# logan-pearce/olpefit

Measured on AMD Instinct MI355X. Metric: walker-steps/sec (= model evals/sec) on 64×64 2-source cutout, 1/2/4/8 GPU, higher is better.
Workload: dtype f64

## Files before the change

### include/olpe.h

```cpp
#ifndef OLPE_H
#define OLPE_H

#include <stddef.h>
#include <stdint.h>

#ifdef __cplusplus
extern "C" {
#endif

#define OLPE_OK 0
#define OLPE_EINVAL (-1)
#define OLPE_EHIP (-2)
#define OLPE_ENOMEM (-3)
#define OLPE_ESTATE (-4)
#define OLPE_ECOMM (-5)
#define OLPE_EIO (-6)

#define OLPE_DTYPE_F32 0
#define OLPE_DTYPE_F64 1

#define OLPE_EVAL_EXACT 0
#define OLPE_EVAL_FAST 1

typedef struct olpe_ctx olpe_ctx;

int olpe_version(void);
int olpe_device_count(int *count);
int olpe_device_mem(int device, long long *free_bytes, long long *total_bytes);
int olpe_device_pci_id(int device, char *buf, int len);
const char *olpe_last_error(void);

int olpe_create(const void *image, int image_dtype, const void *pois2, double readnoise2,
                const uint8_t *mask, int ny, int nx, int nsrc, int bkgd_mode, int device,
                olpe_ctx **out);
void olpe_destroy(olpe_ctx *ctx);
int olpe_set_eval_mode(olpe_ctx *ctx, int mode);

int olpe_model(olpe_ctx *ctx, const double *params, double *model_out);
int olpe_chi2_batch(olpe_ctx *ctx, const double *params, int W, double *chi2_out);
int olpe_normal_batch(olpe_ctx *ctx, const double *params , int W,
                      double *chi2 , double *grad ,
                      double *jtj );

int olpe_seed(olpe_ctx *ctx, const uint32_t *seeds, int W);
int olpe_state_set(olpe_ctx *ctx, const double *state, const double *tries,
                   const double *accepts);
int olpe_state_get(olpe_ctx *ctx, double *state, double *tries, double *accepts);
int olpe_run(olpe_ctx *ctx, long long n_iters, long long burn_in, int record_stride,
             long long accept_min, long long *nrec_out);
int olpe_chain_read(olpe_ctx *ctx, double *chain_out);
int olpe_count(olpe_ctx *ctx, long long *count);
int olpe_count_reset(olpe_ctx *ctx, long long count);
int olpe_done_at(olpe_ctx *ctx, long long *done_at);
int olpe_run_gibbs(olpe_ctx *ctx, double *state, double *tries, double *accepts, int W,
                   long long n_iters, long long burn_in, int record_stride,
                   double *chain_out);

int olpe_rng_get(olpe_ctx *ctx, uint32_t *mt_state, double *gauss_cache);
int olpe_rng_set(olpe_ctx *ctx, const uint32_t *mt_state, const double *gauss_cache);
int olpe_rng_stream(olpe_ctx *ctx, int kind, int n, void *out);

int olpe_trace_enable(olpe_ctx *ctx, int on);
int olpe_trace_read(olpe_ctx *ctx, double *out);

int olpe_sync(olpe_ctx *ctx);
int olpe_last_kernel_ms(olpe_ctx *ctx, double *ms);
int olpe_kernel_times(olpe_ctx *ctx, int n, double *ms_out);
int olpe_last_units(olpe_ctx *ctx, int *units);
int olpe_unit_stats(olpe_ctx *ctx, long long *out);

#define OLPE_LOG_WIDTH_MAX 25.0
int olpe_widths_set(olpe_ctx *ctx, const double *w);
int olpe_widths_get(olpe_ctx *ctx, double *out);

#define OLPE_TUNE_LOG 256
int olpe_tune_begin(olpe_ctx *ctx, double target, double gain);
int olpe_tune_step(olpe_ctx *ctx);
int olpe_tune_get(olpe_ctx *ctx, int *steps, long long *dT, long long *dA, double *widths);
int olpe_tune_end(olpe_ctx *ctx);

int olpe_csv_format(const double *rows, long long nrows, int ncols, int nan_row, char *out,
                    size_t cap, size_t *len_out);
int olpe_csv_write_chains(const char *const *paths, const double *chains, int nfiles,
                          long long nrows, int ncols, int nan_row, int threads);

int olpe_csv_append_chains(const char *const *paths, const double *chains, int nfiles,
                           long long rows_per_file, long long nrows, int ncols, int threads,
                           long long *sizes_out);

int olpe_csv_shape(const char *path, long long *rows, int *cols);
int olpe_csv_read_chains(const char *const *paths, int nfiles, long long nrows, int ncols,
                         long long skip, double *out, int threads);

int olpe_acceptance_format(const double *x, int n, char *out, size_t cap, size_t *len_out);
int olpe_acceptance_write(const char *const *paths, const double *accepts, const double *tries,
                          int nfiles, int np, int threads, unsigned char *done);

int olpe_comm_unique_id(uint8_t *id128);
int olpe_comm_init(olpe_ctx *ctx, const uint8_t *id128, int nranks, int rank);
int olpe_comm_timeout(olpe_ctx *ctx, double seconds);
int olpe_comm_info(olpe_ctx *ctx, int *nranks, int *rank);
int olpe_comm_allgather_state(olpe_ctx *ctx, double *out);
int olpe_comm_allgather_chain(olpe_ctx *ctx, long long w0, long long wn, double *out,
                              long long *nrec_out);
int olpe_comm_gather_limit(olpe_ctx *ctx, long long bytes);
int olpe_comm_allreduce_moments(olpe_ctx *ctx, double *out);

int olpe_moments_accumulate(olpe_ctx *ctx);
int olpe_moments_reset(olpe_ctx *ctx);
int olpe_moments_get(olpe_ctx *ctx, long long *n, double *mean, double *m2);
int olpe_moments_set(olpe_ctx *ctx, long long n, const double *mean, const double *m2);
#define OLPE_MOMENTS_LEN(ps, np) (2 + 3 * (ps) + 2 * (np))
int olpe_moments_summary(olpe_ctx *ctx, const double *centre, double *out);

typedef struct olpe_astrom olpe_astrom;
#define OLPE_ASTROM_LEN 16
#define OLPE_ASTROM_BELOW_180 0
#define OLPE_ASTROM_BELOW_0 1
#define OLPE_ASTROM_ABOVE_360 2
#define OLPE_ASTROM_ABOVE_180 3
#define OLPE_ASTROM_ABOVE_0 4
#define OLPE_ASTROM_BELOW_PER_SAMPLE 5
int olpe_astrom_create(int device, int variant, int ps, const int *pair_cols, int npairs,
                       const double *x_dist, const double *y_dist, int tab_ny, int tab_nx,
                       int xdiff, int ydiff, double pixscale, double rotation_angle,
                       double rotcorr, int use_rotcorr, long long walkers, long long row_cap,
                       olpe_astrom **out);
void olpe_astrom_destroy(olpe_astrom *a);
int olpe_astrom_fold_ctx(olpe_astrom *a, olpe_ctx *ctx);
int olpe_astrom_fold_rows(olpe_astrom *a, const double *rows, long long nrows);
int olpe_astrom_rows(olpe_astrom *a, long long *rows);
int olpe_astrom_finalize(olpe_astrom *a, double delta_r, double parantel, double *out);
int olpe_astrom_samples(olpe_astrom *a, int pair, double *out);

typedef struct olpe_corner olpe_corner;
int olpe_corner_create(int device, int ncols, const double *edges1, int nb1,
                       const double *edges2, int nb2, olpe_corner **out);
void olpe_corner_destroy(olpe_corner *h);
int olpe_corner_fold_ctx(olpe_corner *h, olpe_ctx *ctx);
int olpe_corner_fold_rows(olpe_corner *h, const double *rows, long long nsamples);
int olpe_corner_get(olpe_corner *h, unsigned long long *n, unsigned long long *h1,
                    unsigned long long *h2);
int olpe_corner_add(olpe_corner *h, unsigned long long n, const unsigned long long *h1,
                    const unsigned long long *h2);
int olpe_corner_reset(olpe_corner *h);

// ... 109 lines not shown
```

### olpefit_amd/_lib.py

```python
from __future__ import annotations

import ctypes as C
import os

HERE = os.path.dirname(os.path.abspath(__file__))
LIB_PATH = os.environ.get("OLPE_LIB", os.path.join(HERE, "libolpe.so"))

OK, EINVAL, EHIP, ENOMEM, ESTATE, ECOMM, EIO = 0, -1, -2, -3, -4, -5, -6
DTYPE_F32, DTYPE_F64 = 0, 1
EVAL_EXACT, EVAL_FAST = 0, 1
LOG_WIDTH_MAX = 25.0
TUNE_LOG = 256


class OlpeError(RuntimeError):
    def __init__(self, code: int, msg: str):
        super().__init__(f"olpe error {code}: {msg}")
        self.code = code


_P = C.c_void_p
_i = C.c_int
_ll = C.c_longlong
_d = C.c_double
# ... 41 lines not shown
    "olpe_tune_get": (_i, [_P, C.POINTER(_i), _pll, _pll, _pd]),
    "olpe_tune_end": (_i, [_P]),
    "olpe_csv_format": (_i, [_pd, _ll, _i, _i, C.c_char_p, C.c_size_t,
                             C.POINTER(C.c_size_t)]),
    "olpe_csv_write_chains": (_i, [C.POINTER(C.c_char_p), _pd, _i, _ll, _i, _i, _i]),
    "olpe_csv_append_chains": (_i, [C.POINTER(C.c_char_p), _pd, _i, _ll, _ll, _i, _i, _pll]),
    "olpe_csv_shape": (_i, [C.c_char_p, _pll, C.POINTER(_i)]),
    "olpe_csv_read_chains": (_i, [C.POINTER(C.c_char_p), _i, _ll, _i, _ll, _pd, _i]),
    "olpe_acceptance_format": (_i, [_pd, _i, C.c_char_p, C.c_size_t, C.POINTER(C.c_size_t)]),
    "olpe_acceptance_write": (_i, [C.POINTER(C.c_char_p), _pd, _pd, _i, _i, _i, _pu8]),
    "olpe_moments_accumulate": (_i, [_P]),
    "olpe_moments_reset": (_i, [_P]),
    "olpe_moments_get": (_i, [_P, _pll, _pd, _pd]),
    "olpe_moments_set": (_i, [_P, _ll, _pd, _pd]),
    "olpe_moments_summary": (_i, [_P, _pd, _pd]),
    "olpe_comm_unique_id": (_i, [_pu8]),
    "olpe_comm_init": (_i, [_P, _pu8, _i, _i]),
    "olpe_comm_timeout": (_i, [_P, _d]),
    "olpe_comm_info": (_i, [_P, C.POINTER(_i), C.POINTER(_i)]),
    "olpe_comm_allgather_state": (_i, [_P, _pd]),
    "olpe_comm_allgather_chain": (_i, [_P, _ll, _ll, _pd, _pll]),
    "olpe_comm_gather_limit": (_i, [_P, _ll]),
    "olpe_comm_allreduce_moments": (_i, [_P, _pd]),
    "olpe_astrom_create": (_i, [_i, _i, _i, C.POINTER(_i), _i, _pd, _pd, _i, _i, _i, _i,
                                _d, _d, _d, _i, _ll, _ll, C.POINTER(_P)]),
    "olpe_astrom_destroy": (None, [_P]),
    "olpe_astrom_fold_ctx": (_i, [_P, _P]),
    "olpe_astrom_fold_rows": (_i, [_P, _pd, _ll]),
    "olpe_astrom_rows": (_i, [_P, _pll]),
    "olpe_astrom_finalize": (_i, [_P, _d, _d, _pd]),
    "olpe_astrom_samples": (_i, [_P, _i, _pd]),
    "olpe_corner_create": (_i, [_i, _i, _pd, _i, _pd, _i, C.POINTER(_P)]),
    "olpe_corner_destroy": (None, [_P]),
    "olpe_corner_fold_ctx": (_i, [_P, _P]),
    "olpe_corner_fold_rows": (_i, [_P, _pd, _ll]),
    "olpe_corner_get": (_i, [_P, _pu64, _pu64, _pu64]),
    "olpe_corner_add": (_i, [_P, C.c_ulonglong, _pu64, _pu64]),
    "olpe_corner_reset": (_i, [_P]),
    "olpe_resid_create": (_i, [_P, _pd, C.POINTER(_P)]),
    "olpe_resid_destroy": (None, [_P]),
    "olpe_resid_fold_ctx": (_i, [_P, _P, _i, _i]),
    "olpe_resid_fold_rows": (_i, [_P, _pd, _ll]),
    "olpe_resid_get": (_i, [_P, _pll, _pll, _pd, _pd, _pd, _pd]),
    "olpe_resid_add": (_i, [_P, _ll, _ll, _pd, _pd, _pd, _pd]),
    "olpe_resid_reset": (_i, [_P]),
    "olpe_resid_finalize": (_i, [_P, _pd, _pd]),
    "olpe_lik_create": (_i, [_P, _pd, C.POINTER(_P)]),
    "olpe_lik_destroy": (None, [_P]),
    "olpe_lik_fold_ctx": (_i, [_P, _P, _i, _i]),
    "olpe_lik_fold_rows": (_i, [_P, _pd, _ll]),
    "olpe_lik_get": (_i, [_P, _pll, _pll, _pd, _pd, _pd, _pd, _pd, _pd]),
    "olpe_lik_add": (_i, [_P, _ll, _ll, _pd, _pd, _pd, _pd, _pd, _pd]),
    "olpe_lik_reset": (_i, [_P]),
    "olpe_lik_point": (_i, [_P, _pd, _pd]),
    "olpe_lik_finalize": (_i, [_P, _pd, _pd, _pd]),
    "olpe_acf_create": (_i, [_i, _i, _i, C.POINTER(_P)]),
    "olpe_acf_destroy": (None, [_P]),
    "olpe_acf_fold_ctx": (_i, [_P, _P]),
    "olpe_acf_fold_rows": (_i, [_P, _pd, _ll, _ll, _i]),
    "olpe_acf_get": (_i, [_P, _pu64, _pu64, _pu64, _pd]),
    "olpe_acf_add": (_i, [_P, _i, _i, C.c_ulonglong, C.c_ulonglong, C.c_ulonglong, _pd]),
    "olpe_acf_reset": (_i, [_P]),
    "olpe_phot_create": (_i, [_i, _i, _i, _d, _ll, _ll, C.POINTER(_P)]),
    "olpe_phot_destroy": (None, [_P]),
    "olpe_phot_fold_ctx": (_i, [_P, _P, _i]),
    "olpe_phot_fold_rows": (_i, [_P, _pd, _ll]),
    "olpe_phot_rows": (_i, [_P, _pll]),
    "olpe_phot_unusable": (_i, [_P, _pll]),
    "olpe_phot_finalize": (_i, [_P, _pd, _i, _pd]),
    "olpe_phot_samples": (_i, [_P, _i, _pd]),
    "olpe_phot_reset": (_i, [_P]),
    "olpe_cov_create": (_i, [_i, _i, _ll, _pd, C.POINTER(_P)]),
    "olpe_cov_destroy": (None, [_P]),
    "olpe_cov_fold_ctx": (_i, [_P, _P, _i]),
    "olpe_cov_fold_rows": (_i, [_P, _pd, _ll, _ll, _i]),
    "olpe_cov_get": (_i, [_P, _pu64, _pu64, C.POINTER(_i), _pd, _pd, _pd]),
    "olpe_cov_walkers_get": (_i, [_P, _pu64, _pd]),
    "olpe_cov_between": (_i, [_P, _pd, _pu64, _pu64, _pu64]),
    "olpe_cov_add": (_i, [_P, _i, _ll, C.c_ulonglong, C.c_ulonglong, _pd, _pd, _pd, _pu64,
                          _pd]),
    "olpe_cov_reset": (_i, [_P]),
    "olpe_moments_fault": (_i, [_P, _i]),
    "olpe_test_hold_handoff": (_i, [_P, _i]),
    "olpe_test_chain_set": (_i, [_P, _pd, _ll]),
    "olpe_test_jacobian": (_i, [_P, _pd, _pd]),
}

_lib = None


def load(path: str = LIB_PATH):
    global _lib
    if _lib is not None:
        return _lib
    if not os.path.exists(path):
        raise OSError(f"libolpe.so not found at {path}: build it with "
                      "`python -m olpefit_amd.build` (hipcc, gfx950)")
    lib = C.CDLL(path)
    for name, (res, args) in SIGNATURES.items():
        f = getattr(lib, name)
        f.restype = res
        f.argtypes = args
    _lib = lib
    return lib


def check(rc: int) -> None:
    if rc != OK:
        msg = load().olpe_last_error().decode(errors="replace")
        raise OlpeError(rc, msg)
```

### olpefit_amd/core.py

```python
from __future__ import annotations

import ctypes as C

import numpy as np

from . import _lib
from ._lib import OlpeError, check

__all__ = ["OlpeError", "Sampler", "noise_model", "param_count", "SIGMA0"]

SIGMA0 = (50 / 9.95) / 2.35


def param_count(nsrc: int) -> int:
    if nsrc not in (2, 3):
        raise ValueError("nsrc must be 2 or 3")
    return 16 if nsrc == 2 else 19


def _dptr(a):
    return a.ctypes.data_as(_lib._pd) if a is not None else None


def noise_model(image, itime, coadds, multisam, sampmode):
# ... 220 lines not shown
            if w.shape != (self.np_,):
                raise ValueError(f"widths must have {self.np_} entries")
        check(self._lib.olpe_widths_set(self._ctx, _dptr(w)))

    def get_widths(self):
        out = np.empty(self.np_)
        check(self._lib.olpe_widths_get(self._ctx, _dptr(out)))
        return out

    def tune_begin(self, target=0.44, gain=2.0):
        check(self._lib.olpe_tune_begin(self._ctx, float(target), float(gain)))

    def tune_step(self):
        check(self._lib.olpe_tune_step(self._ctx))

    def tune_history(self):
        k = C.c_int(0)
        dT = np.zeros((_lib.TUNE_LOG, self.np_), dtype=np.int64)
        dA = np.zeros((_lib.TUNE_LOG, self.np_), dtype=np.int64)
        w = np.zeros((_lib.TUNE_LOG, self.np_))
        check(self._lib.olpe_tune_get(self._ctx, C.byref(k), dT.ctypes.data_as(_lib._pll),
                                      dA.ctypes.data_as(_lib._pll), _dptr(w)))
        k = k.value
        return dT[:k].copy(), dA[:k].copy(), w[:k].copy()

    def tune_end(self):
        check(self._lib.olpe_tune_end(self._ctx))

    @staticmethod
    def device_count() -> int:
        n = C.c_int(0)
        check(_lib.load().olpe_device_count(C.byref(n)))
        return n.value

    @staticmethod
    def device_pci_id(device: int) -> str:
        buf = C.create_string_buffer(64)
        check(_lib.load().olpe_device_pci_id(int(device), buf, 64))
        return buf.value.decode()

    @staticmethod
    def comm_unique_id() -> bytes:
        buf = (C.c_uint8 * 128)()
        check(_lib.load().olpe_comm_unique_id(buf))
        return bytes(buf)

    def comm_init(self, uid: bytes, nranks: int, rank: int):
        buf = (C.c_uint8 * 128).from_buffer_copy(uid)
        check(self._lib.olpe_comm_init(self._ctx, buf, nranks, rank))
        self.nranks = nranks

    def comm_timeout(self, seconds: float):
        check(self._lib.olpe_comm_timeout(self._ctx, float(seconds)))

    def comm_info(self) -> tuple[int, int]:
        n, r = C.c_int(-1), C.c_int(-1)
        check(self._lib.olpe_comm_info(self._ctx, C.byref(n), C.byref(r)))
        return n.value, r.value

    def allgather_state(self):
        out = np.empty((self.nranks * self.W, self.ps))
        check(self._lib.olpe_comm_allgather_state(self._ctx, _dptr(out)))
        return out

    def allgather_chain(self, w0: int = 0, wn: int | None = None, out: bool = True):
        wn = self.W - w0 if wn is None else wn
        nrec = C.c_longlong(0)
        buf = np.empty((self.nranks, wn, self._nrec, self.ps)) if out else None
        check(self._lib.olpe_comm_allgather_chain(self._ctx, int(w0), int(wn), _dptr(buf),
                                                  C.byref(nrec)))
        return buf

    def gather_limit(self, nbytes: int):
        check(self._lib.olpe_comm_gather_limit(self._ctx, int(nbytes)))

    def allreduce_moments(self):
        out = np.empty(self.moments_len)
        check(self._lib.olpe_comm_allreduce_moments(self._ctx, _dptr(out)))
        return out

    def hold_handoff(self, on: bool = True):
        check(self._lib.olpe_test_hold_handoff(self._ctx, 1 if on else 0))

    def test_chain_set(self, chain):
        ch = np.ascontiguousarray(chain, dtype=np.float64)
        if ch.ndim != 3 or ch.shape[2] != self.ps or (self.W and ch.shape[0] != self.W):
            raise ValueError(f"chain must be [{self.W}, nrec, {self.ps}]")
        check(self._lib.olpe_test_chain_set(self._ctx, _dptr(ch), ch.shape[1]))
        self._nrec = int(ch.shape[1])
        self._record_stride = 1

    def moments_fault(self, where: int):
        check(self._lib.olpe_moments_fault(self._ctx, int(where)))

    @property
    def moments_len(self) -> int:
        return 2 + 3 * self.ps + 2 * self.np_

    def moments_accumulate(self):
        check(self._lib.olpe_moments_accumulate(self._ctx))

    def moments_reset(self):
        check(self._lib.olpe_moments_reset(self._ctx))

    def moments(self):
        n = C.c_longlong(0)
        mean = np.empty((self.W, self.ps))
        m2 = np.empty((self.W, self.ps))
        check(self._lib.olpe_moments_get(self._ctx, C.byref(n), _dptr(mean), _dptr(m2)))
        return int(n.value), mean, m2

    def set_moments(self, n, mean=None, m2=None):
        mean = None if mean is None else np.ascontiguousarray(mean, dtype=np.float64)
        m2 = None if m2 is None else np.ascontiguousarray(m2, dtype=np.float64)
        check(self._lib.olpe_moments_set(self._ctx, int(n), _dptr(mean), _dptr(m2)))

    def moments_summary(self, centre=None):
        out = np.empty(self.moments_len)
        c = None if centre is None else np.ascontiguousarray(centre, dtype=np.float64)
        check(self._lib.olpe_moments_summary(self._ctx, _dptr(c), _dptr(out)))
        return out
```

### olpefit_amd/csrc/olpe.hip

```cpp
#include <hip/hip_runtime.h>

#include <limits.h>
#include <math.h>
#include <stdarg.h>
#include <stdint.h>
#include <stdio.h>
#include <stdlib.h>
#include <string.h>

#include <algorithm>
#include <cmath>
#include <atomic>
#include <vector>

#include "../../include/olpe.h"
#include "../../include/olpe_test.h"
#include "olpe_device.h"
#include "olpe_internal.h"

using namespace olpe;

namespace {

__constant__ double c_widths2[16] = {0.01, 0.01, 0.3,   0.3,    0.08,  0.09,
                                     0.0025, 0.02, 0.001, 0.0008, 0.002, 0.002,
                                     0.001, 0.001, 0.008, 0.01};
__constant__ double c_widths3[19] = {0.01,  0.01,  0.3,   0.3,  0.3,   0.3,   0.08,
                                     0.09,  0.0025, 0.02, 0.02, 0.001, 0.0008, 0.002,
                                     0.002, 0.001, 0.001, 0.008, 0.01};

__device__ __forceinline__ double width_of(const double *widths, int r) {
  return ((const __attribute__((address_space(4))) double *)widths)[r];
}

__global__ void widths_default_kernel(int nsrc, double *w, double *wdef) {
  const int j = threadIdx.x;
  if (j >= (nsrc == 2 ? 16 : 19)) return;
  const double v = nsrc == 2 ? c_widths2[j] : c_widths3[j];
  w[j] = v;
  if (wdef) wdef[j] = v;
}

struct GibbsArgs {
  const double2 *DE;
  int n;
  int bkgd_mode;
  long long W;
  double *state;
  uint32_t *tries;
  uint32_t *accepts;
  uint32_t *mt;
  int *mt_pos;
  double *gauss;
  int *has_gauss;
  long long *done_at;
  long long n_iters;
  long long count0;
  long long burn_in;
  long long stride;
  long long row0;
  long long nrows;
  double *chain;
  long long accept_min;
  double *trace;
  const double *widths;
  unsigned long long *queue;
  unsigned long long qbase;
  int units;
  unsigned *uflag;
  unsigned utag;
  unsigned *uerr;
  unsigned long long wait_ticks;
  int balance;
  int stagger;
  unsigned *hold;
};

constexpr int kTraceF = 6;
constexpr int kSampHdr = kEtabBytes + 64;


template <int NP> struct WaveSlice {
  static constexpr int U32 = 2 * NP;
  static constexpr int PS = NP + 1;
  static constexpr int NSRC = NP == 16 ? 2 : 3;
  static constexpr int OT1 = PS, OT2 = PS + 5, OC1 = PS + 10, OC2 = PS + 13;
  static constexpr int OPT = PS + 16, OPC = PS + 21;
  static constexpr int OWD = PS + 24;
  static constexpr int F64 = 2 * PS + 24;
  static constexpr int OMD = ((U32 * 4 + F64 * 8 + 15) & ~15);
  static constexpr int OCC = (OMD + (int)sizeof(ModelDesc<NSRC>) + 15) & ~15;
  static constexpr int OPE = (OCC + 2 * NSRC * 4 * 8 + 15) & ~15;
  static constexpr int BYTES = OPE + NSRC * 2 * 64 * 8;
};
constexpr int kDrawTabBytes = (kDrawTab * 8 + 15) & ~15;
constexpr int kDrawTabExactBytes = (kThr * 8 + 15) & ~15;
__host__ __device__ constexpr int drawtab_extra(int nt, bool fast = true) {
  return (nt != 0 && nt <= 64) ? (fast ? kDrawTabBytes : kDrawTabExactBytes) : 0;
}
__host__ __device__ inline int vtab_bytes(int n, int nsrc) { return (n * 2 * nsrc * 8 + 15) & ~15; }
__host__ __device__ constexpr bool single_h(int nsrc, int nt, int wpb, bool fast) {
  return nsrc == 2 && nt == 64 && wpb == 16 && fast;
}
__host__ __device__ constexpr int sampler_vtab_bytes(int n, int nsrc, int nt, int wpb = 12,
                                                     bool fast = false) {
  return single_h(nsrc, nt, wpb, fast) ? 64 * 16
       : (nsrc == 3 && nt == 64) ? 2 * 64 * 16 : ((n * 2 * nsrc * 8 + 15) & ~15);
}
template <int NP> __host__ __device__ constexpr int ring_wave_bytes(int n) {
  return WaveSlice<NP>::OPE + kDrawTabBytes + 2 * n * 16;
}
__host__ __device__ constexpr bool ring_wpb(int nt, int wpb) {
  return nt == 128 && (wpb == 12 || wpb == 8);
}
static_assert((WaveSlice<16>::U32 * 4) % 8 == 0 && (WaveSlice<19>::U32 * 4) % 8 == 0, "align");
template <int NP> constexpr int parking_bytes() { return WaveSlice<NP>::BYTES - WaveSlice<NP>::OPE; }
static_assert(parking_bytes<16>() >= 64 * 4 * 8 && sampler_vtab_bytes(64, 2, 64) >= 64 * 4 * 8 &&
              parking_bytes<19>() >= 64 * 6 * 8 && parking_bytes<16>() >= 2 * 32 * 4 * 8 &&
              parking_bytes<19>() >= 2 * 32 * 6 * 8 && sampler_vtab_bytes(128, 2, 128) >= 128 * 4 * 8 &&
              sampler_vtab_bytes(128, 3, 128) >= 128 * 6 * 8 && drawtab_extra(32) && drawtab_extra(64),
              "sweep_exact_rows tables");

__device__ __forceinline__ Trig ld_trig(const double *s) { return Trig{s[0], s[1], s[2]}; }
__device__ __forceinline__ Coef ld_coef(const double *s) { return Coef{s[0], s[1], s[2]}; }
__device__ __forceinline__ void st_trig(double *s, const Trig &t) {
  s[0] = t.cost2; s[1] = t.sint2; s[2] = t.sin2t;
}
__device__ __forceinline__ void st_shape(double *s, const Trig &t, double ix, double iy) {
  st_trig(s, t);
  s[3] = ix; s[4] = iy;
}
__device__ __forceinline__ void st_coef(double *s, const Coef &k) {
  s[0] = k.a; s[1] = k.b; s[2] = k.c;
}

__device__ __forceinline__ void lds_inc(uint32_t *p) {
  const unsigned a = (unsigned)(size_t)(__attribute__((address_space(3))) uint32_t *)p;
  asm volatile("ds_add_u32 %0, %1" : : "v"(a), "v"(1u) : "memory");
}
__device__ __forceinline__ uint32_t lds_inc_rtn(uint32_t *p) {
  const unsigned a = (unsigned)(size_t)(__attribute__((address_space(3))) uint32_t *)p;
  uint32_t old;
  asm volatile("ds_add_rtn_u32 %0, %1, %2\n\ts_waitcnt lgkmcnt(0)"
               : "=v"(old) : "v"(a), "v"(1u) : "memory");
  return old;
}

typedef __attribute__((address_space(1))) unsigned gu32;
typedef __attribute__((address_space(1))) unsigned long long gu64;
__device__ __forceinline__ void st_wt(double *p, double v) {
  __hip_atomic_store((gu64 *)p, (unsigned long long)__double_as_longlong(v), __ATOMIC_RELAXED,
                     __HIP_MEMORY_SCOPE_AGENT);
}
__device__ __forceinline__ void st_wt(long long *p, long long v) {
  __hip_atomic_store((gu64 *)p, (unsigned long long)v, __ATOMIC_RELAXED, __HIP_MEMORY_SCOPE_AGENT);
}
template <class T> __device__ __forceinline__ void st_wt(T *p, T v) {
  static_assert(sizeof(T) == 4, "32-bit word");
  unsigned u;
  __builtin_memcpy(&u, &v, 4);
  __hip_atomic_store((gu32 *)p, u, __ATOMIC_RELAXED, __HIP_MEMORY_SCOPE_AGENT);
}
template <class T> __device__ __forceinline__ T ld_uniform(const T *p) {
  static_assert(sizeof(T) == 4, "32-bit word");
  const unsigned u = (unsigned)__builtin_amdgcn_readfirstlane(
      (int)__hip_atomic_load((gu32 *)p, __ATOMIC_RELAXED, __HIP_MEMORY_SCOPE_AGENT));
  T v;
  __builtin_memcpy(&v, &u, 4);
  return v;
}
__device__ __forceinline__ void unit_publish(unsigned *flag, unsigned v, int lane) {
  asm volatile("s_waitcnt vmcnt(0)" ::: "memory");
  if (lane == 0) __hip_atomic_store((gu32 *)flag, v, __ATOMIC_RELAXED, __HIP_MEMORY_SCOPE_AGENT);
}
__device__ __forceinline__ void unit_wait(unsigned *flag, unsigned want, unsigned *err,
                                          unsigned long long *stats, int lane,
                                          unsigned long long limit, unsigned *hold) {
  const unsigned long long t0 = __builtin_amdgcn_s_memrealtime();
  bool waited = false;
  for (;;) {
    const unsigned v = (unsigned)__builtin_amdgcn_readfirstlane(
        (int)__hip_atomic_load((gu32 *)flag, __ATOMIC_RELAXED, __HIP_MEMORY_SCOPE_AGENT));
    if (v == want) break;
    if (!waited && hold && lane == 0)
      __hip_atomic_store((gu32 *)hold, 1u, __ATOMIC_RELAXED, __HIP_MEMORY_SCOPE_AGENT);
    waited = true;
    if (__builtin_amdgcn_s_memrealtime() - t0 > limit) {
      __hip_atomic_store((gu32 *)err, 1u, __ATOMIC_RELAXED, __HIP_MEMORY_SCOPE_AGENT);
      break;
    }
    __builtin_amdgcn_s_sleep(4);
  }
  if (waited && lane == 0) {
    atomicAdd(stats, 1ull);
    atomicAdd(stats + 1, __builtin_amdgcn_s_memrealtime() - t0);
  }
  __builtin_amdgcn_fence(__ATOMIC_ACQUIRE, "agent");
  asm volatile("s_waitcnt vmcnt(0)" ::: "memory");
}

__device__ __forceinline__ void hold_handoff(unsigned *hold, unsigned *err, unsigned long long limit) {
  const unsigned long long t0 = __builtin_amdgcn_s_memrealtime();
  while (__builtin_amdgcn_readfirstlane((int)__hip_atomic_load((gu32 *)hold, __ATOMIC_RELAXED,
                                                               __HIP_MEMORY_SCOPE_AGENT)) == 0) {
    if (__builtin_amdgcn_s_memrealtime() - t0 > limit) {
      __hip_atomic_store((gu32 *)err, 1u, __ATOMIC_RELAXED, __HIP_MEMORY_SCOPE_AGENT);
      break;
    }
    __builtin_amdgcn_s_sleep(4);
  }
}

constexpr int kCtrlPrio = 2;
constexpr int kGlobalWavesPerEU = 3;
template <int NSRC, int NT, bool LDS_IMG, int WPB, bool FAST>
__global__ __launch_bounds__(WPB * 64, (LDS_IMG || (NT == 128 && WPB == 12)) ? 1 : kGlobalWavesPerEU)
void olpe_gibbs_kernel(GibbsArgs A) {
  using L = Layout<NSRC>;
  using WS = WaveSlice<L::NP>;
  constexpr int NP = L::NP, PS = L::PS;
  constexpr bool RING = !LDS_IMG && FAST && ring_wpb(NT, WPB);
  using Ring = LdsRing<WPB>;
  extern __shared__ __align__(16) unsigned char smem[];
  const int n = NT ? NT : A.n;
  const int npix = n * n;
  const int lane = threadIdx.x & 63;
  const int wave = __builtin_amdgcn_readfirstlane(threadIdx.x >> 6);

  double *etab = reinterpret_cast<double *>(smem);
  unsigned *s_prog = reinterpret_cast<unsigned *>(smem + kEtabBytes);
  double2 *sDE = reinterpret_cast<double2 *>(smem + kSampHdr);
  constexpr int TABX = drawtab_extra(NT, FAST);
  const int wstride = RING ? ring_wave_bytes<NP>(n)
                           : WS::BYTES + TABX + sampler_vtab_bytes(n, NSRC, NT, WPB, FAST);
  unsigned char *wb = reinterpret_cast<unsigned char *>(sDE + (LDS_IMG ? npix : 0)) +
                      (RING ? Ring::BYTES : 0) + (size_t)wave * wstride;
  uint32_t *s_tries = reinterpret_cast<uint32_t *>(wb);
  uint32_t *s_acc = s_tries + NP;
  double *st = reinterpret_cast<double *>(wb + WS::U32 * 4);
  double *vtab = reinterpret_cast<double *>(wb + (RING ? WS::OPE + kDrawTabBytes : WS::BYTES + TABX));
  double *drawtab = reinterpret_cast<double *>(wb + (TABX ? WS::BYTES : WS::OPE));
  ModelDesc<NSRC> *mdl = reinterpret_cast<ModelDesc<NSRC> *>(wb + WS::OMD);
  double *colc = reinterpret_cast<double *>(wb + WS::OCC);

  if constexpr (LDS_IMG) {
    for (int k = threadIdx.x; k < npix; k += blockDim.x) sDE[k] = A.DE[k];
  }
  if (threadIdx.x < 64) etab[threadIdx.x] = c_exp2_64[threadIdx.x];
  if (threadIdx.x == 0) s_prog[0] = 0u;
  __syncthreads();
  const double2 *DE = LDS_IMG ? sDE : A.DE;
  [[maybe_unused]] Ring ring;
  if constexpr (RING) ring.prologue(smem + kSampHdr, A.DE, wave, lane);
  unsigned my_steps = 0;
  for (int i = 0, n = (wave >> 2) * A.stagger; i < n; ++i) __builtin_amdgcn_s_sleep(8);

  auto K = []() {
    const __attribute__((address_space(4))) GibbsArgs *p =
        (const __attribute__((address_space(4))) GibbsArgs *)__builtin_amdgcn_kernarg_segment_ptr();
    asm volatile("" : "+s"(p));
    return p;
  };

  auto take = [&]() -> int {
    unsigned long long v = 0;
    if (lane == 0) v = atomicAdd(K()->queue, 1ull) - K()->qbase;
    const unsigned d = v > 0x7fffffffull ? 0x7fffffffu : (unsigned)v;
    return __builtin_amdgcn_readfirstlane((int)d);
  };

  const int niter = (int)A.n_iters;
  const int rstride = (int)A.stride;
  const int nrows = (int)A.nrows;
  int rec_it0 = -1, rec_row0 = 0;
  if (A.stride > 0) {
    const long long c1 = A.count0 + 1;
    const long long k = c1 > A.burn_in ? (c1 - A.burn_in + A.stride - 1) / A.stride : 0;
    const long long first = A.burn_in + k * A.stride - c1;
    rec_it0 = first < niter ? (int)first : -1;
    rec_row0 = (int)(k - A.row0);
  }
  auto take_batch = [&]() -> int {
    asm volatile("s_waitcnt lgkmcnt(0)\n\ts_barrier" ::: "memory");
    if (wave == 0 && lane == 0) {
      const unsigned long long v = atomicAdd(K()->queue, 1ull) - K()->qbase;
      s_prog[1] = v > 0x7fffffffull ? 0x7fffffffu : (unsigned)v;
    }
    asm volatile("s_waitcnt lgkmcnt(0)\n\ts_barrier" ::: "memory");
    return __builtin_amdgcn_readfirstlane((int)s_prog[1]);
  };
  const int total = (int)K()->W * K()->units;
  int u = RING ? 0 : A.queue ? take() : (int)blockIdx.x * WPB + wave;
  for (;;) {
    bool active = true;
    if constexpr (RING) {
      const int bt = take_batch();
      if (bt >= (total + WPB - 1) / WPB) break;
      u = bt * WPB + wave;
      active = u < total;
      if (!active) u = 0;
    } else {
      if (u >= total) break;
    }
    const int units = K()->units;
    const int Wn = (int)K()->W;
    int w = u, k = 0, it_s = 0, it_e = niter;
    if (units > 1) {
      k = u / Wn;
      w = u - k * Wn;
      const int q = niter / units, r = niter - q * units;
      it_s = q * k + (r * k) / units;
      it_e = q * (k + 1) + (r * (k + 1)) / units;
      if (k > 0 && active)
        unit_wait(K()->uflag + w, K()->utag + (unsigned)k, K()->uerr, K()->queue + 2, lane,
                  K()->wait_ticks, K()->hold);
    }
    int it_end = it_e;
    if constexpr (RING) {
      if (lane == 0) s_prog[2 + wave] = active ? (unsigned)(it_e - it_s) : 0u;
      asm volatile("s_waitcnt lgkmcnt(0)\n\ts_barrier" ::: "memory");
      unsigned mx = 0;
      for (int j = 0; j < WPB; ++j) mx = max(mx, s_prog[2 + j]);
      it_end = it_s + (int)__builtin_amdgcn_readfirstlane((int)mx);
      if (!active) it_e = it_s;
    }
    if (lane < NP) {
      s_tries[lane] = K()->tries[(size_t)w * NP + lane];
      s_acc[lane] = K()->accepts[(size_t)w * NP + lane];
    }
    if (lane < PS) st[lane] = K()->state[(size_t)w * PS + lane];
    if constexpr (FAST) {
      if (lane < NP) st[WS::OWD + lane] = K()->widths[lane];
    }
    wave_sync();
    if (lane == 0) {
      const Trig t1 = make_trig<FAST>(st[L::T1]), t2 = make_trig<FAST>(st[L::T2]);
      const double i1x = inv_var(st[L::S1X]), i1y = inv_var(st[L::S1Y]);
      const double i2x = inv_var(st[L::S2X]), i2y = inv_var(st[L::S2Y]);
      st_shape(st + WS::OT1, t1, i1x, i1y);
      st_shape(st + WS::OT2, t2, i2x, i2y);
      if constexpr (FAST) {
        st_coef(st + WS::OC1, coef_inv(t1, i1x, i1y));
        st_coef(st + WS::OC2, coef_inv(t2, i2x, i2y));
      } else {
        st_coef(st + WS::OC1, make_coef<FAST>(st[L::S1X], st[L::S1Y], t1));
        st_coef(st + WS::OC2, make_coef<FAST>(st[L::S2X], st[L::S2Y], t2));
      }
    }
    wave_sync();
    const int bg_idx = A.bkgd_mode == 0 ? L::BG_QUIRK : L::BG_FIXED;
    build_desc<NSRC, NT, FAST>(mdl, colc, [&](int k) -> double { return st[k]; },
                               ld_coef(st + WS::OC1), ld_coef(st + WS::OC2), bg_idx, lane, etab);
    wave_sync();

    MTWave mt;
    mt.key = K()->mt + (size_t)w * MT_N;
    mt.pos = ld_uniform(K()->mt_pos + w);
    mt.bstart = mt.pos;
    mt.bsize = 0;
    mt.batch = 0;
    mt.has_gauss = ld_uniform(K()->has_gauss + w);
    mt.gauss = uniform_f64(K()->gauss[w]);
    mt.tab = drawtab;
    mt.thr = FAST;

    int ndone = 0;
    long long done_at = K()->done_at[w];
    if (A.accept_min > 0) {
      for (int k = 0; k < NP; ++k) ndone += (s_tries[k] >= (uint32_t)A.accept_min);
      ndone = __builtin_amdgcn_readfirstlane(ndone);
      if (ndone == NP && done_at < 0 && it_s < it_e) done_at = A.count0 + it_s + 1;
    }

    int rec_it = rec_it0, rec_row = rec_row0;
    if (rec_it0 >= 0 && it_s > rec_it0) {
      const int j = (it_s - rec_it0 + rstride - 1) / rstride;
      rec_it += j * rstride;
      rec_row += j;
    }
    double *chain_w = K()->chain + (size_t)w * nrows * PS;

    HCache hcache;
    hcache.single = single_h(NSRC, NT, WPB, FAST);
    GuardCache gcache;
    ColCache<2 * NSRC> ccache;
    ccache.pbuf = reinterpret_cast<double *>(wb + WS::OPE);
    ccache.colc = colc;
    __builtin_amdgcn_s_setprio(kCtrlPrio);
    for (int it = it_s; it < it_end; ++it) {
      if constexpr (RING) {
        if (it >= it_e) {
          ring.idle_step();
          continue;
        }
      }
      int r0 = 0, dice_idx = 0;
      double g = 0.0;
      mt.template draw<NP>(lane, 0, 2, r0, g, dice_idx);
      const int r = __builtin_amdgcn_readfirstlane(r0);
// ... 112 lines not shown

      const double dchi = chi - st[PS - 1];
      const double la = -dchi / 2.;
      double dice = 0.0;
      if constexpr (!FAST) dice = drawtab[dice_idx];
      bool acc;
      uint32_t acc_bit;
      if constexpr (FAST) {
        const double thr = drawtab[kThr + (dice_idx == 128 ? 64 : dice_idx)];
        acc_bit = (uint32_t)(__builtin_amdgcn_ballot_w64(dchi < thr) >> 32) >> 31;
      } else {
        acc_bit = (uint32_t)(__builtin_amdgcn_ballot_w64(dice < exp(la)) >> 32) >> 31;
      }
      asm volatile("" : "+s"(acc_bit));
      acc = acc_bit != 0;
      if (acc && lane == 63) st[PS - 1] = chi;
      double chi_u = 0.0, la_u = 0.0;
      if (A.trace) {
        chi_u = lane63_f64(chi);
        la_u = lane63_f64(la);
      }
      hcache.after(acc);
      gcache.after(acc);
      if constexpr (FAST && NT != 0 && NT <= 64) {
        if (acc && gmask) colcache_accept<NSRC, NT>(ccache, *mdl, gmask, lane, etab);
        ccache.pend = 0;
      }
      if (!acc && !nan_prop) {
        Coef Cs{0.0, 0.0, 0.0};
        if (grp) Cs = ld_coef(st + (grp == 1 ? WS::OC1 : WS::OC2));
        int pl = lane;
        asm volatile("" : "+v"(pl));
        patch_desc<NSRC, NT, FAST>(mdl, colc, st, r, st[r], Cs, grp,
                                   A.bkgd_mode == 0 ? L::BG_QUIRK : L::BG_FIXED, pl, etab);
      }
      wave_sync();
      if (acc && lane == 0) {
        if constexpr (FAST) lds_inc(s_acc + r);
        else s_acc[r] = s_acc[r] + 1u;
        st[r] = nv;
        if (grp) {
          double *dt = st + (grp == 1 ? WS::OT1 : WS::OT2);
          double *dc = st + (grp == 1 ? WS::OC1 : WS::OC2);
          for (int k = 0; k < 5; ++k) dt[k] = st[WS::OPT + k];
          for (int k = 0; k < 3; ++k) dc[k] = st[WS::OPC + k];
        }
      }
      wave_sync();

      if (A.trace) {
       if (lane == 0) {
        double *t = A.trace + ((size_t)w * A.n_iters + it) * kTraceF;
        t[0] = (double)r;
        t[1] = nv;
        t[2] = chi_u;
        t[3] = FAST ? drawtab[dice_idx] : dice;
        t[4] = FAST ? (la_u == la_u ? ExpTab{etab}(la_u) : la_u) : exp(la_u);
        t[5] = acc ? 1.0 : 0.0;
       }
      }
      if (it == rec_it) {
        if (rec_row >= 0 && rec_row < nrows && lane < PS) chain_w[rec_row * PS + lane] = st[lane];
        rec_it += rstride;
        ++rec_row;
      }
    }

    wave_sync();
    if (RING && !active) continue;
    asm volatile("" : "+s"(u));
    k = K()->units > 1 ? u / (int)K()->W : 0;
    w = u - k * (int)K()->W;
    if (lane < PS) st_wt(K()->state + (size_t)w * PS + lane, st[lane]);
    if (lane < NP) {
      st_wt(K()->tries + (size_t)w * NP + lane, s_tries[lane]);
      st_wt(K()->accepts + (size_t)w * NP + lane, s_acc[lane]);
    }
    if (lane == 0) {
      st_wt(K()->mt_pos + w, mt.pos);
      st_wt(K()->has_gauss + w, mt.has_gauss);
      st_wt(K()->gauss + w, mt.gauss);
      st_wt(K()->done_at + w, done_at);
    }
    if (k < K()->units - 1) {
      if (k == 0 && K()->hold) hold_handoff(K()->hold, K()->uerr, K()->wait_ticks);
      unit_publish(K()->uflag + w, K()->utag + (unsigned)(k + 1), lane);
    }
    wave_sync();
    if constexpr (!RING) u = K()->queue ? take() : INT_MAX;
  }
  if constexpr (RING) asm volatile("s_waitcnt vmcnt(0) lgkmcnt(0)\n\ts_barrier" ::: "memory");
}

template <int NSRC, bool WRITE>
__global__ __launch_bounds__(256) void olpe_eval_kernel(const double2 *DE, int n, int bkgd_mode,
                                                        int fast, const double *params, int W,
                                                        double *out) {
  using L = Layout<NSRC>;
  constexpr int PS = L::PS;
  extern __shared__ __align__(16) unsigned char smem[];
  const int lane = threadIdx.x & 63;
  const int wave = threadIdx.x >> 6;
  double *etab = reinterpret_cast<double *>(smem);
  double *vtab =
      reinterpret_cast<double *>(smem + kEtabBytes + (size_t)wave * vtab_bytes(n, NSRC));
  if (threadIdx.x < 64) etab[threadIdx.x] = c_exp2_64[threadIdx.x];
  __syncthreads();
  const long long w = (long long)blockIdx.x * (blockDim.x / 64) + wave;
  if (w >= W) return;
  double p[PS];
#pragma unroll
  for (int k = 0; k < PS; ++k) p[k] = uniform_f64(params[w * PS + k]);
  auto q = [&](int k) -> double { return p[k]; };
  double *o = WRITE ? out + (size_t)w * n * n : nullptr;
  double part;
  if (fast) {
    const Trig T1 = make_trig<true>(p[L::T1]), T2 = make_trig<true>(p[L::T2]);
    const ModelDesc<NSRC> md = make_model<NSRC>(
        q, make_coef<true>(p[L::S1X], p[L::S1Y], T1), make_coef<true>(p[L::S2X], p[L::S2Y], T2),
        bkgd_mode);
    part = sweep<NSRC, 0, WRITE, true>(md, DE, vtab, o, n, lane, etab);
  } else {
    const Trig T1 = make_trig<false>(p[L::T1]), T2 = make_trig<false>(p[L::T2]);
    const ModelDesc<NSRC> md = make_model<NSRC>(
        q, make_coef<false>(p[L::S1X], p[L::S1Y], T1),
        make_coef<false>(p[L::S2X], p[L::S2Y], T2), bkgd_mode);
    part = sweep<NSRC, 0, WRITE, false>(md, DE, vtab, o, n, lane, etab);
  }
  if constexpr (!WRITE) {
    const double chi = wave_sum(part);
    if (lane == 0) out[w] = chi;
  }
}

__global__ void olpe_seed_kernel(const uint32_t *seeds, int W, uint32_t *mt, int *pos,
                                 int *has_gauss, double *gauss) {
  const int w = blockIdx.x * blockDim.x + threadIdx.x;
  if (w >= W) return;
  mt_seed_serial(mt + (size_t)w * MT_N, seeds[w]);
  pos[w] = MT_N;
  has_gauss[w] = 0;
  gauss[w] = 0.0;
}

template <int NP>
__global__ __launch_bounds__(64) void olpe_stream_kernel(uint32_t *mtg, int *posg,
                                                         int *hasg, double *gg, int W,
                                                         int kind, int nd, void *out) {
  const int lane = threadIdx.x;
  const int w = blockIdx.x;
  if (w >= W) return;
  __shared__ double drawtab[kDrawTab];
  MTWave mt;
  mt.tab = drawtab;
  mt.key = mtg + (size_t)w * MT_N;
  mt.pos = __builtin_amdgcn_readfirstlane(posg[w]);
  mt.bstart = mt.pos;
  mt.bsize = 0;
  mt.batch = 0;
  mt.has_gauss = __builtin_amdgcn_readfirstlane(hasg[w]);
  mt.gauss = uniform_f64(gg[w]);
  for (int i = 0; i < nd; ++i) {
    if (kind == 0) {
      const uint32_t v = mt.next(lane);
      if (lane == 0) reinterpret_cast<uint32_t *>(out)[(size_t)w * nd + i] = v;
    } else {
      int r = 0, di = 0;
      double v = 0.0;
// ... 8 lines not shown
    posg[w] = mt.pos;
    hasg[w] = mt.has_gauss;
    gg[w] = mt.gauss;
  }
}

}

namespace olpe {

thread_local char g_err[512] = "";

int set_err(int code, const char *fmt, ...) {
  va_list ap;
  va_start(ap, fmt);
  vsnprintf(g_err, sizeof(g_err), fmt, ap);
  va_end(ap);
  return code;
}

}

namespace {

template <class T> int dev_alloc(T **p, size_t count) {
  if (*p) {
    (void)hipFree(*p);
    *p = nullptr;
  }
  if (count == 0) return OLPE_OK;
  hipError_t e = hipMalloc((void **)p, count * sizeof(T));
  if (e != hipSuccess) {
    *p = nullptr;
    return set_err(OLPE_ENOMEM, "hipMalloc(%zu bytes): %s", count * sizeof(T),
                   hipGetErrorString(e));
  }
  return OLPE_OK;
}

size_t wave_lds(int n, int np, bool lds_img, bool ring = false, int wpb = 12,
                bool fast = false) {
  if (ring) return (size_t)(np == 16 ? ring_wave_bytes<16>(n) : ring_wave_bytes<19>(n));
  const int nt = lds_img && (n == 32 || n == 64) ? n : 0;
  return (size_t)(np == 16 ? WaveSlice<16>::BYTES : WaveSlice<19>::BYTES) +
         drawtab_extra(nt, fast) + sampler_vtab_bytes(n, np == 16 ? 2 : 3, nt, wpb, fast);
}

int choose_units(long long W, long long slots, long long n_iters, int override_p) {
  const int pmax = 15;
  auto ok = [&](int p) { return p <= pmax && p <= n_iters && W * p < 0x7fffffffLL; };
  if (override_p > 0) {
    int p = override_p;
    while (p > 1 && !ok(p)) --p;
    return p;
  }
  if (n_iters < 16 || slots <= 0 || W <= 0) return 1;
  const double s0 = 2.0;
  auto T = [&](int p) {
    const double rounds = (double)((W * p + slots - 1) / slots);
    return std::max(rounds * ((double)n_iters / p + s0), (double)n_iters + p * s0);
  };
  int best = 1;
  double tb = T(1);
  for (int p = 2; p <= 8; ++p) {
    if (!ok(p) || n_iters / p < 8) break;
    const double t = T(p);
    if (t < tb) {
      tb = t;
      best = p;
    }
  }
  return tb < 0.97 * T(1) ? best : 1;
}

size_t lds_bytes(const olpe_ctx *c, int wpb, bool ring = false) {
  size_t b = (size_t)wpb * wave_lds(c->n, c->np, c->lds_img, ring, wpb,
                                    c->eval_mode == OLPE_EVAL_FAST) + kSampHdr;
  if (c->lds_img) b += (size_t)c->n * c->n * sizeof(double2);
  if (ring) b += wpb >= 12 ? LdsRing<12>::BYTES : LdsRing<8>::BYTES;
  return b;
}


template <int NSRC, int NT, bool LDS, int WPB, bool FAST>
int launch_gibbs_t(olpe_ctx *c, const GibbsArgs &a) {
  constexpr bool RING = !LDS && FAST && ring_wpb(NT, WPB);
  const size_t shm = lds_bytes(c, WPB, RING);
  auto k = olpe_gibbs_kernel<NSRC, NT, LDS, WPB, FAST>;
  static std::atomic<uint64_t> attr_set{0};
  const uint64_t bit = 1ull << (c->device & 63);
  if (!(attr_set.load(std::memory_order_acquire) & bit)) {
    HIPCHK(hipFuncSetAttribute((const void *)k, hipFuncAttributeMaxDynamicSharedMemorySize,
                               160 * 1024));
    attr_set.fetch_or(bit, std::memory_order_release);
  }
  unsigned blocks = (unsigned)((a.W + WPB - 1) / WPB);
  GibbsArgs q = a;
  q.queue = nullptr;
  q.qbase = 0;
  q.units = 1;
  q.uflag = c->d_uflag;
  q.utag = 0;
  q.uerr = reinterpret_cast<unsigned *>(c->d_queue + 1);
  q.stagger = c->stagger;
  q.hold = nullptr;
  int per_cu = 0;
  HIPCHK(hipOccupancyMaxActiveBlocksPerMultiprocessor(&per_cu, k, WPB * 64, shm));
  const unsigned resident = (unsigned)std::max(1, per_cu) * (unsigned)c->n_cu;
  const int units = c->queue_on && c->d_queue && c->d_uflag && !(RING && a.W < WPB)
                        ? choose_units(a.W, (long long)resident * WPB, a.n_iters, c->units_override)
                        : 1;
  if (c->queue_on && c->d_queue && (LDS || RING || units > 1)) {
    if (blocks > resident) blocks = resident;
    q.queue = c->d_queue;
    q.qbase = c->qbase;
    q.units = units;
    c->utag += 16;
    q.utag = c->utag;
    if (c->hold_handoff && units > 1) {
      const unsigned need = (unsigned)((a.W + WPB - 1) / WPB) + 1;
      if (need > resident)
        return set_err(OLPE_EINVAL, "olpe_test_hold_handoff: %lld walkers need %u resident "
                       "workgroups, the device holds %u", a.W, need, resident);
      blocks = need;
      HIPCHK(hipMemsetAsync(c->d_queue + 4, 0, sizeof(unsigned long long), c->stream));
      q.hold = reinterpret_cast<unsigned *>(c->d_queue + 4);
    }
  }
  q.balance = c->balance >= 0 ? c->balance
            : (LDS && FAST && NSRC == 2 && WPB == 16 && q.units == 1 &&
               a.W <= (long long)resident * WPB) ? 1 : 0;
  c->last_units = q.units;
  if (q.units > 1) c->units_used = true;
  {
    const double chunk = (double)((a.n_iters + q.units - 1) / q.units);
    const double ticks = chunk * (double)a.n * (double)a.n * (2.0 * NSRC) * 0.8;
    q.wait_ticks = c->wait_ticks_override > 0
                       ? (unsigned long long)c->wait_ticks_override
                       : (unsigned long long)std::min(std::max(ticks, 3e9), 1e15);
    c->wait_limit_s = (double)q.wait_ticks * 1e-8;
  }
  hipLaunchKernelGGL(k, dim3(blocks), dim3(WPB * 64), shm, c->stream, q);
  HIPCHK(hipGetLastError());
  if (q.queue) {
    const unsigned long long tot = (unsigned long long)a.W * (unsigned long long)q.units;
    c->qbase += RING ? (tot + WPB - 1) / WPB + blocks : tot + (unsigned long long)blocks * WPB;
  }
  return OLPE_OK;
}

template <int NSRC, bool FAST> int launch_gibbs_m(olpe_ctx *c, const GibbsArgs &a) {
  if (c->lds_img) {
    switch (c->n) {
      case 32: return launch_gibbs_t<NSRC, 32, true, 12, FAST>(c, a);
      case 64: {
        const long long r16 = 16LL * c->n_cu, r12 = 12LL * c->n_cu;
        int wpb = c->wpb ? c->wpb
                : (NSRC == 2 && (!FAST || a.W >= 8 * r16 || (a.W > r12 && a.W <= r16)))
                      ? 16 : 12;
        if (wpb == 16 && lds_bytes(c, 16) > 160 * 1024) wpb = 12;
        if (wpb == 8) return launch_gibbs_t<NSRC, 64, true, 8, FAST>(c, a);
        if (wpb == 12) return launch_gibbs_t<NSRC, 64, true, 12, FAST>(c, a);
        return launch_gibbs_t<NSRC, 64, true, 16, FAST>(c, a);
      }
      default: return launch_gibbs_t<NSRC, 0, true, 16, FAST>(c, a);
    }
  }
  if (c->n == 128) {
    if constexpr (FAST) {
      if (c->ring_wpb && c->queue_on && c->d_queue && c->d_uflag) {
        return launch_gibbs_t<NSRC, 128, false, 12, FAST>(c, a);
      }
    }
    return launch_gibbs_t<NSRC, 128, false, 4, FAST>(c, a);
  }
  if (lds_bytes(c, 4) > 160 * 1024) return launch_gibbs_t<NSRC, 0, false, 1, FAST>(c, a);
  return launch_gibbs_t<NSRC, 0, false, 4, FAST>(c, a);
}

int launch_gibbs(olpe_ctx *c, const GibbsArgs &a) {
  const bool fast = c->eval_mode == OLPE_EVAL_FAST;
  if (c->nsrc == 2) return fast ? launch_gibbs_m<2, true>(c, a) : launch_gibbs_m<2, false>(c, a);
  return fast ? launch_gibbs_m<3, true>(c, a) : launch_gibbs_m<3, false>(c, a);
}

int ensure_ensemble(olpe_ctx *c, int W) {
  if (W <= 0) return set_err(OLPE_EINVAL, "W must be > 0 (got %d)", W);
  if (c->W == W && c->d_state) return OLPE_OK;
  int rc;
  if ((rc = dev_alloc(&c->d_state, (size_t)W * c->ps))) return rc;
  if ((rc = dev_alloc(&c->d_tries, (size_t)W * c->np))) return rc;
  if ((rc = dev_alloc(&c->d_acc, (size_t)W * c->np))) return rc;
  if ((rc = dev_alloc(&c->d_mt, (size_t)W * MT_N))) return rc;
  if ((rc = dev_alloc(&c->d_mtpos, (size_t)W))) return rc;
  if ((rc = dev_alloc(&c->d_gauss, (size_t)W))) return rc;
  if ((rc = dev_alloc(&c->d_hasg, (size_t)W))) return rc;
  if ((rc = dev_alloc(&c->d_done, (size_t)W))) return rc;
  if ((rc = dev_alloc(&c->d_uflag, (size_t)W))) return rc;
  HIPCHK(hipMemsetAsync(c->d_uflag, 0, (size_t)W * sizeof(unsigned), c->stream));
  HIPCHK(hipMemsetAsync(c->d_state, 0, (size_t)W * c->ps * sizeof(double), c->stream));
  HIPCHK(hipMemsetAsync(c->d_tries, 0, (size_t)W * c->np * sizeof(uint32_t), c->stream));
  HIPCHK(hipMemsetAsync(c->d_acc, 0, (size_t)W * c->np * sizeof(uint32_t), c->stream));
  HIPCHK(hipMemsetAsync(c->d_done, 0xff, (size_t)W * sizeof(long long), c->stream));
  c->W = W;
  c->seeded = false;
  c->count = 0;
  c->chain_rows = 0;
  c->mom_n = 0;
  return OLPE_OK;
}

}

int olpe_widths_defaults(olpe_ctx *c, bool with_base) {
  hipLaunchKernelGGL(widths_default_kernel, dim3(1), dim3(64), 0, c->stream, c->nsrc, c->d_widths,
                     with_base ? c->d_wdef : nullptr);
  HIPCHK(hipGetLastError());
  return OLPE_OK;
}

extern "C" {

int olpe_version(void) { return 101; }


const char *olpe_last_error(void) { return g_err; }

int olpe_device_count(int *count) {
  if (!count) return set_err(OLPE_EINVAL, "count is NULL");
  int n = 0;
  hipError_t e = hipGetDeviceCount(&n);
  *count = (e == hipSuccess) ? n : 0;
  return OLPE_OK;
}

int olpe_device_pci_id(int device, char *buf, int len) {
  if (!buf || len < 16) return set_err(OLPE_EINVAL, "buffer of at least 16 bytes needed");
  int ndev = 0;
  if (hipGetDeviceCount(&ndev) != hipSuccess || ndev == 0)
    return set_err(OLPE_EHIP, "no HIP device visible");
  if (device < 0 || device >= ndev) return set_err(OLPE_EINVAL, "bad device %d", device);
  HIPCHK(hipDeviceGetPCIBusId(buf, len, device));
  return OLPE_OK;
}

int olpe_device_mem(int device, long long *free_bytes, long long *total_bytes) {
  if (!free_bytes || !total_bytes) return set_err(OLPE_EINVAL, "NULL argument");
  int ndev = 0;
  if (hipGetDeviceCount(&ndev) != hipSuccess || ndev == 0)
    return set_err(OLPE_EHIP, "no HIP device visible");
  if (device < 0 || device >= ndev) return set_err(OLPE_EINVAL, "bad device %d", device);
  HIPCHK(hipSetDevice(device));
  size_t f = 0, t = 0;
  HIPCHK(hipMemGetInfo(&f, &t));
  *free_bytes = (long long)f;
  *total_bytes = (long long)t;
  return OLPE_OK;
}

int olpe_create(const void *image, int image_dtype, const void *pois2, double readnoise2,
                const uint8_t *mask, int ny, int nx, int nsrc, int bkgd_mode, int device,
                olpe_ctx **out) {
  if (!out) return set_err(OLPE_EINVAL, "out is NULL");
  *out = nullptr;
  if (!image || !pois2) return set_err(OLPE_EINVAL, "image/pois2 is NULL");
  if (ny <= 0 || nx <= 0) return set_err(OLPE_EINVAL, "bad shape %dx%d", ny, nx);
  if (ny != nx)
    return set_err(OLPE_EINVAL,
                   "non-square image %dx%d: the reference model is square-only "
                   "(apf_step2.py:237, :119-123)", ny, nx);
  if (nx > 4096) return set_err(OLPE_EINVAL, "image too large (%d)", nx);
  if (nsrc != 2 && nsrc != 3) return set_err(OLPE_EINVAL, "nsrc must be 2 or 3");
  {
    const size_t one = wave_lds(nx, nsrc == 2 ? 16 : 19, false) + kSampHdr;
    if (one > 160 * 1024)
      return set_err(OLPE_EINVAL, "%dx%d cutout: its row tables need %zu bytes of LDS per "
                     "wave, more than the 163840 a workgroup has (cut the frame to the stars)",
                     nx, nx, one);
  }
  if (image_dtype != OLPE_DTYPE_F32 && image_dtype != OLPE_DTYPE_F64)
    return set_err(OLPE_EINVAL, "image_dtype must be OLPE_DTYPE_F32/F64");
  if (bkgd_mode != 0 && bkgd_mode != 1) return set_err(OLPE_EINVAL, "bkgd_mode must be 0/1");
  if (device < 0) return set_err(OLPE_EINVAL, "device must be a HIP ordinal (no CPU path)");
  const int np_ = nsrc == 2 ? 16 : 19;
  const size_t npix_ = (size_t)nx * nx;
  const bool lds_img = npix_ * sizeof(double2) +
                           ((nx == 64 || nx == 32) ? 12 : 16) * wave_lds(nx, np_, true) +
                           kSampHdr <= 160 * 1024;
  int wpb = 0;
  if (const char *e = getenv("OLPE_WPB")) {
    wpb = atoi(e);
    if (wpb != 8 && wpb != 12 && wpb != 16)
      return set_err(OLPE_EINVAL, "OLPE_WPB=%s: must be 8, 12 or 16", e);
    const size_t b = (size_t)wpb * wave_lds(nx, np_, true, false, wpb, true) + kSampHdr +
                     npix_ * sizeof(double2);
    if (lds_img && nx == 64 && b > 160 * 1024)
      return set_err(OLPE_EINVAL, "OLPE_WPB=%d needs %zu bytes of LDS at %dx%d (%d sources) > 163840",
                     wpb, b, nx, nx, nsrc);
    if (!(lds_img && nx == 64)) wpb = 0;
  }
  int ndev = 0;
  if (hipGetDeviceCount(&ndev) != hipSuccess || ndev == 0)
    return set_err(OLPE_EHIP, "no HIP device visible");
  if (device >= ndev) return set_err(OLPE_EINVAL, "device %d >= device count %d", device, ndev);
  HIPCHK(hipSetDevice(device));

  olpe_ctx *c = new olpe_ctx();
  c->device = device;
  c->n = nx;
  c->nsrc = nsrc;
  c->bkgd_mode = bkgd_mode;
  c->np = nsrc == 2 ? 16 : 19;
  c->ps = c->np + 1;
  const size_t npix = (size_t)nx * nx;
  c->lds_img = lds_img;
  c->wpb = wpb;
  std::vector<double2> hDE(npix), hDW(npix);
  for (size_t i = 0; i < npix; ++i) {
    const double d = image_dtype == OLPE_DTYPE_F32 ? (double)((const float *)image)[i]
                                                   : ((const double *)image)[i];
    const double p2 = image_dtype == OLPE_DTYPE_F32 ? (double)((const float *)pois2)[i]
                                                    : ((const double *)pois2)[i];
    const double e = sqrt(readnoise2 + p2);
    if ((mask && mask[i]) || !std::isfinite(d) || !(e > 0.0)) {
      hDE[i] = make_double2(0.0, 0.0);
      hDW[i] = make_double2(0.0, 0.0);
    } else {
      hDE[i] = make_double2(d, 1.0 / e);
      hDW[i] = make_double2(d * (1.0 / e), 1.0 / e);
    }
  }
  bool any_pixel = false;
  for (size_t i = 0; i < npix && !any_pixel; ++i) any_pixel = hDE[i].y != 0.0;
  if (!any_pixel) {
    hDE[0] = make_double2(NAN, NAN);
    hDW[0] = make_double2(NAN, NAN);
  }
  int rc;
  hipError_t e1 = hipStreamCreateWithFlags(&c->stream, hipStreamNonBlocking);
  if (e1 != hipSuccess) {
    delete c;
    return set_err(OLPE_EHIP, "hipStreamCreate: %s", hipGetErrorString(e1));
  }
  for (auto &pair : c->ev)
    for (auto &ev : pair)
      if (hipEventCreate(&ev) != hipSuccess) ev = nullptr;
  if ((rc = dev_alloc(&c->d_DE, npix)) || (rc = dev_alloc(&c->d_DW, npix)) ||
      (rc = dev_alloc(&c->d_queue, 5)) || (rc = olpe_comm_setup(c))) {
    olpe_destroy(c);
    return rc;
  }
  if (hipMemset(c->d_queue, 0, 5 * sizeof(unsigned long long)) != hipSuccess ||
      hipDeviceGetAttribute(&c->n_cu, hipDeviceAttributeMultiprocessorCount, device) !=
          hipSuccess || c->n_cu <= 0) {
    olpe_destroy(c);
    return set_err(OLPE_EHIP, "walker queue setup failed");
  }
  if (const char *e = getenv("OLPE_NO_QUEUE")) c->queue_on = atoi(e) == 0;
  if (const char *e = getenv("OLPE_UNITS")) {
    const int p = atoi(e);
    if (p < 0 || p > 15) {
      olpe_destroy(c);
      return set_err(OLPE_EINVAL, "OLPE_UNITS=%s: must be 0 (automatic) .. 15", e);
    }
    c->units_override = p;
  }
  if (const char *e = getenv("OLPE_RING")) {
    const int v = atoi(e);
    if (v != 0 && v != 12) {
      olpe_destroy(c);
      return set_err(OLPE_EINVAL, "OLPE_RING=%s: must be 0 (off) or 12 (waves per workgroup)", e);
    }
    c->ring_wpb = v;
  }
  if (const char *e = getenv("OLPE_WAIT_TICKS")) c->wait_ticks_override = std::max(0.0, atof(e));
  hipError_t e2 = hipMemcpy(c->d_DE, hDE.data(), npix * sizeof(double2), hipMemcpyHostToDevice);
  if (e2 == hipSuccess)
    e2 = hipMemcpy(c->d_DW, hDW.data(), npix * sizeof(double2), hipMemcpyHostToDevice);
  if (e2 != hipSuccess) {
    olpe_destroy(c);
    return set_err(OLPE_EHIP, "hipMemcpy image: %s", hipGetErrorString(e2));
  }
  c->logmask = nsrc == 2 ? Layout<2>::LOGMASK : Layout<3>::LOGMASK;
  if ((rc = dev_alloc(&c->d_widths, (size_t)c->np)) || (rc = dev_alloc(&c->d_wdef, (size_t)c->np)) ||
      (rc = olpe_widths_defaults(c, true))) {
    olpe_destroy(c);
    return rc;
  }
  if (hipStreamSynchronize(c->stream) != hipSuccess) {
    olpe_destroy(c);
    return set_err(OLPE_EHIP, "filling in the default jump widths failed");
  }
  *out = c;
  return OLPE_OK;
}

void olpe_destroy(olpe_ctx *c) {
  if (!c) return;
  (void)hipSetDevice(c->device);
  if (c->stream) (void)hipStreamSynchronize(c->stream);
  olpe_comm_release(c);
  void *ptrs[] = {c->d_DE, c->d_DW, c->d_state, c->d_tries, c->d_acc,
                  c->d_mt, c->d_mtpos, c->d_gauss, c->d_hasg,  c->d_done,
                  c->d_chain, c->d_trace, c->d_scratch, c->d_scratch2, c->d_queue,
                  c->d_gather, c->d_uflag, c->d_mmean, c->d_mm2, c->d_mpart, c->d_check,
                  c->d_widths, c->d_wdef, c->d_tune};
  for (void *p : ptrs)
    if (p) (void)hipFree(p);
  for (auto &pair : c->ev)
    for (auto &ev : pair)
      if (ev) (void)hipEventDestroy(ev);
  if (c->stream) (void)hipStreamDestroy(c->stream);
  delete c;
}

int olpe_set_eval_mode(olpe_ctx *c, int mode) {
  if (!c) return set_err(OLPE_EINVAL, "ctx is NULL");
  if (mode != OLPE_EVAL_EXACT && mode != OLPE_EVAL_FAST)
    return set_err(OLPE_EINVAL, "unknown eval mode %d", mode);
  c->eval_mode = mode;
  return OLPE_OK;
}

static int eval_batch(olpe_ctx *c, const double *params, int W, double *out, bool write) {
  if (!c || !params || !out) return set_err(OLPE_EINVAL, "NULL argument");
  if (W <= 0) return set_err(OLPE_EINVAL, "W must be > 0");
  HIPCHK(hipSetDevice(c->device));
  const size_t pin = (size_t)W * c->ps;
  const size_t pout = write ? (size_t)W * c->n * c->n : (size_t)W;
  int rc;
  if (c->scratch_cap < pin && (rc = dev_alloc(&c->d_scratch, pin))) return rc;
  if (c->scratch_cap < pin) c->scratch_cap = pin;
  if (c->scratch2_cap < pout && (rc = dev_alloc(&c->d_scratch2, pout))) return rc;
  if (c->scratch2_cap < pout) c->scratch2_cap = pout;
  HIPCHK(hipMemcpyAsync(c->d_scratch, params, pin * 8, hipMemcpyHostToDevice, c->stream));
  int wpb = 4;
  while (wpb > 1 && (size_t)wpb * vtab_bytes(c->n, c->nsrc) + kEtabBytes > 160 * 1024) wpb /= 2;
  dim3 grid((W + wpb - 1) / wpb), block(wpb * 64);
  const size_t shm = (size_t)wpb * vtab_bytes(c->n, c->nsrc) + kEtabBytes;
  const int fast = c->eval_mode == OLPE_EVAL_FAST;
  if (shm > 160 * 1024) return set_err(OLPE_EINVAL, "image too large for the eval kernel");
  if (shm > 65536) {
    static std::atomic<uint64_t> eval_attr{0};
    const uint64_t bit = 1ull << (c->device & 63);
    if (!(eval_attr.load(std::memory_order_acquire) & bit)) {
      const void *ks[4] = {(const void *)olpe_eval_kernel<2, true>,
                           (const void *)olpe_eval_kernel<2, false>,
                           (const void *)olpe_eval_kernel<3, true>,
                           (const void *)olpe_eval_kernel<3, false>};
      for (const void *k : ks)
        HIPCHK(hipFuncSetAttribute(k, hipFuncAttributeMaxDynamicSharedMemorySize, 160 * 1024));
      eval_attr.fetch_or(bit, std::memory_order_release);
    }
  }
  if (c->nsrc == 2) {
    if (write)
      hipLaunchKernelGGL((olpe_eval_kernel<2, true>), grid, block, shm, c->stream, fast ? c->d_DW : c->d_DE,
                         c->n, c->bkgd_mode, fast, c->d_scratch, W, c->d_scratch2);
    else
      hipLaunchKernelGGL((olpe_eval_kernel<2, false>), grid, block, shm, c->stream, fast ? c->d_DW : c->d_DE,
                         c->n, c->bkgd_mode, fast, c->d_scratch, W, c->d_scratch2);
  } else {
    if (write)
      hipLaunchKernelGGL((olpe_eval_kernel<3, true>), grid, block, shm, c->stream, fast ? c->d_DW : c->d_DE,
                         c->n, c->bkgd_mode, fast, c->d_scratch, W, c->d_scratch2);
    else
      hipLaunchKernelGGL((olpe_eval_kernel<3, false>), grid, block, shm, c->stream, fast ? c->d_DW : c->d_DE,
                         c->n, c->bkgd_mode, fast, c->d_scratch, W, c->d_scratch2);
  }
  HIPCHK(hipGetLastError());
  HIPCHK(hipMemcpyAsync(out, c->d_scratch2, pout * 8, hipMemcpyDeviceToHost, c->stream));
  HIPCHK(hipStreamSynchronize(c->stream));
  return OLPE_OK;
}

int olpe_model(olpe_ctx *c, const double *params, double *model_out) {
  return eval_batch(c, params, 1, model_out, true);
}

int olpe_chi2_batch(olpe_ctx *c, const double *params, int W, double *chi2_out) {
  return eval_batch(c, params, W, chi2_out, false);
}

int olpe_seed(olpe_ctx *c, const uint32_t *seeds, int W) {
  if (!c || !seeds) return set_err(OLPE_EINVAL, "NULL argument");
  HIPCHK(hipSetDevice(c->device));
  int rc;
  if ((rc = ensure_ensemble(c, W))) return rc;
  uint32_t *ds = nullptr;
  if ((rc = dev_alloc(&ds, (size_t)W))) return rc;
  HIPCHK(hipMemcpyAsync(ds, seeds, (size_t)W * 4, hipMemcpyHostToDevice, c->stream));
  hipLaunchKernelGGL(olpe_seed_kernel, dim3((W + 255) / 256), dim3(256), 0, c->stream, ds, W,
                     c->d_mt, c->d_mtpos, c->d_hasg, c->d_gauss);
  HIPCHK(hipGetLastError());
  HIPCHK(hipStreamSynchronize(c->stream));
  (void)hipFree(ds);
  c->seeded = true;
  c->mom_n = 0;
  c->mom_folded = c->launches;
  return OLPE_OK;
}

static int check_units(olpe_ctx *c) {
  if (!c->d_queue || !c->units_used) return OLPE_OK;
  unsigned long long e = 0;
  HIPCHK(hipMemcpy(&e, c->d_queue + 1, sizeof(e), hipMemcpyDeviceToHost));
  if (e)
    return set_err(OLPE_EHIP, "sampler chunk hand-off timed out (%.0f s): results invalid",
                   c->wait_limit_s);
  return OLPE_OK;
}

static int counters_to_dev(olpe_ctx *c, const double *h, uint32_t *d) {
  const size_t m = (size_t)c->W * c->np;
  std::vector<uint32_t> t(m, 0u);
  if (h)
    for (size_t i = 0; i < m; ++i) {
      if (!(h[i] >= 0.0) || h[i] > 4294967295.0)
        return set_err(OLPE_EINVAL, "counter %zu out of range (%g)", i, h[i]);
      t[i] = (uint32_t)h[i];
    }
  HIPCHK(hipMemcpyAsync(d, t.data(), m * 4, hipMemcpyHostToDevice, c->stream));
  HIPCHK(hipStreamSynchronize(c->stream));
  return OLPE_OK;
}

static int counters_to_host(olpe_ctx *c, const uint32_t *d, double *h) {
  const size_t m = (size_t)c->W * c->np;
  std::vector<uint32_t> t(m);
  HIPCHK(hipMemcpy(t.data(), d, m * 4, hipMemcpyDeviceToHost));
  for (size_t i = 0; i < m; ++i) h[i] = (double)t[i];
  return OLPE_OK;
}

int olpe_state_set(olpe_ctx *c, const double *state, const double *tries,
                   const double *accepts) {
  if (!c || !state) return set_err(OLPE_EINVAL, "NULL argument");
  if (!c->d_state) return set_err(OLPE_ESTATE, "call olpe_seed first");
  HIPCHK(hipSetDevice(c->device));
  HIPCHK(hipStreamSynchronize(c->stream));
  HIPCHK(hipMemcpyAsync(c->d_state, state, (size_t)c->W * c->ps * 8, hipMemcpyHostToDevice,
                        c->stream));
  int rc;
  if ((rc = counters_to_dev(c, tries, c->d_tries))) return rc;
  if ((rc = counters_to_dev(c, accepts, c->d_acc))) return rc;
  HIPCHK(hipMemsetAsync(c->d_done, 0xff, (size_t)c->W * sizeof(long long), c->stream));
  HIPCHK(hipStreamSynchronize(c->stream));
  return OLPE_OK;
}

int olpe_state_get(olpe_ctx *c, double *state, double *tries, double *accepts) {
  if (!c) return set_err(OLPE_EINVAL, "NULL ctx");
  if (!c->d_state) return set_err(OLPE_ESTATE, "no ensemble");
  HIPCHK(hipSetDevice(c->device));
  HIPCHK(hipStreamSynchronize(c->stream));
  if (state)
    HIPCHK(hipMemcpy(state, c->d_state, (size_t)c->W * c->ps * 8, hipMemcpyDeviceToHost));
  int rc;
  if (tries && (rc = counters_to_host(c, c->d_tries, tries))) return rc;
  if (accepts && (rc = counters_to_host(c, c->d_acc, accepts))) return rc;
  return check_units(c);
}

int olpe_run(olpe_ctx *c, long long n_iters, long long burn_in, int record_stride,
             long long accept_min, long long *nrec_out) {
  if (!c) return set_err(OLPE_EINVAL, "NULL ctx");
  if (!c->d_state || !c->seeded) return set_err(OLPE_ESTATE, "call olpe_seed first");
  if (n_iters < 0 || burn_in < 0 || record_stride < 0 || accept_min < 0)
    return set_err(OLPE_EINVAL, "negative argument");
  if (n_iters > 0x7fffffffLL)
    return set_err(OLPE_EINVAL, "n_iters per launch must be < 2^31 (split the run)");
  HIPCHK(hipSetDevice(c->device));
  long long row0 = 0, nrows = 0;
  const long long c0 = c->count, c1 = c->count + n_iters;
  if (record_stride > 0 && c1 >= burn_in) {
    const long long s = record_stride;
    const long long lo = std::max(c0 + 1, burn_in);
    const long long first = (lo - burn_in + s - 1) / s;
    const long long last = (c1 - burn_in) / s;
    if (last >= first) {
      row0 = first;
      nrows = last - first + 1;
    }
  }
  int rc;
  const size_t chain_need = (size_t)c->W * nrows * c->ps;
  if (chain_need > c->chain_cap) {
    if ((rc = dev_alloc(&c->d_chain, chain_need))) return rc;
    c->chain_cap = chain_need;
  }
  c->chain_rows = nrows;
  const size_t trace_need = c->trace_on ? (size_t)c->W * n_iters * kTraceF : 0;
  if (trace_need > c->trace_cap) {
    if ((rc = dev_alloc(&c->d_trace, trace_need))) return rc;
    c->trace_cap = trace_need;
  }
  c->trace_iters = c->trace_on ? n_iters : 0;

  GibbsArgs a;
  a.DE = c->eval_mode == OLPE_EVAL_FAST ? c->d_DW : c->d_DE;
  a.n = c->n;
  a.bkgd_mode = c->bkgd_mode;
  a.W = c->W;
  a.state = c->d_state;
  a.tries = c->d_tries;
  a.accepts = c->d_acc;
  a.mt = c->d_mt;
  a.mt_pos = c->d_mtpos;
  a.gauss = c->d_gauss;
  a.has_gauss = c->d_hasg;
  a.done_at = c->d_done;
  a.n_iters = n_iters;
  a.count0 = c0;
  a.burn_in = burn_in;
  a.stride = nrows > 0 ? record_stride : 0;
  a.row0 = row0;
  a.nrows = nrows;
  a.chain = c->d_chain;
  a.accept_min = accept_min;
  a.trace = c->trace_on ? c->d_trace : nullptr;
  a.widths = c->d_widths;
  hipEvent_t *ev = c->ev[c->launches % olpe_ctx::kRing];
  if (!ev[0] || !ev[1]) return set_err(OLPE_EHIP, "launch events were not created");
  HIPCHK(hipEventRecord(ev[0], c->stream));
  if ((rc = launch_gibbs(c, a))) return rc;
  HIPCHK(hipEventRecord(ev[1], c->stream));
  ++c->launches;
  c->count = c1;
  if (nrec_out) *nrec_out = nrows;
  return OLPE_OK;
}

int olpe_chain_read(olpe_ctx *c, double *chain_out) {
  if (!c || !chain_out) return set_err(OLPE_EINVAL, "NULL argument");
  HIPCHK(hipSetDevice(c->device));
  HIPCHK(hipStreamSynchronize(c->stream));
  const size_t m = (size_t)c->W * c->chain_rows * c->ps;
  if (m) HIPCHK(hipMemcpy(chain_out, c->d_chain, m * 8, hipMemcpyDeviceToHost));
  return check_units(c);
}

int olpe_count(olpe_ctx *c, long long *count) {
  if (!c || !count) return set_err(OLPE_EINVAL, "NULL argument");
  *count = c->count;
  return OLPE_OK;
}

int olpe_count_reset(olpe_ctx *c, long long count) {
  if (!c || count < 0) return set_err(OLPE_EINVAL, "bad argument");
  c->count = count;
  return OLPE_OK;
}

int olpe_done_at(olpe_ctx *c, long long *done_at) {
  if (!c || !done_at) return set_err(OLPE_EINVAL, "NULL argument");
  if (!c->d_done) return set_err(OLPE_ESTATE, "no ensemble");
  HIPCHK(hipSetDevice(c->device));
  HIPCHK(hipStreamSynchronize(c->stream));
  HIPCHK(hipMemcpy(done_at, c->d_done, (size_t)c->W * 8, hipMemcpyDeviceToHost));
  return check_units(c);
}

int olpe_run_gibbs(olpe_ctx *c, double *state, double *tries, double *accepts, int W,
                   long long n_iters, long long burn_in, int record_stride,
                   double *chain_out) {
  if (!c || !state) return set_err(OLPE_EINVAL, "NULL argument");
  if (!c->seeded || c->W != W)
    return set_err(OLPE_ESTATE, "seed %d walkers with olpe_seed first", W);
  int rc;
  if ((rc = olpe_state_set(c, state, tries, accepts))) return rc;
  c->count = 0;
  if ((rc = olpe_run(c, n_iters, burn_in, record_stride, 0, nullptr))) return rc;
  if ((rc = olpe_state_get(c, state, tries, accepts))) return rc;
  if (chain_out && (rc = olpe_chain_read(c, chain_out))) return rc;
  return OLPE_OK;
}

int olpe_rng_get(olpe_ctx *c, uint32_t *mt_state, double *gauss_cache) {
  if (!c) return set_err(OLPE_EINVAL, "NULL ctx");
  if (!c->d_mt) return set_err(OLPE_ESTATE, "no ensemble");
  HIPCHK(hipSetDevice(c->device));
  HIPCHK(hipStreamSynchronize(c->stream));
  const int W = c->W;
  if (mt_state) {
    std::vector<uint32_t> key((size_t)W * MT_N);
    std::vector<int> pos(W);
    HIPCHK(hipMemcpy(key.data(), c->d_mt, key.size() * 4, hipMemcpyDeviceToHost));
    HIPCHK(hipMemcpy(pos.data(), c->d_mtpos, (size_t)W * 4, hipMemcpyDeviceToHost));
    for (int w = 0; w < W; ++w) {
      memcpy(mt_state + (size_t)w * (MT_N + 1), key.data() + (size_t)w * MT_N, MT_N * 4);
      mt_state[(size_t)w * (MT_N + 1) + MT_N] = (uint32_t)pos[w];
    }
  }
  if (gauss_cache) {
    std::vector<int> h(W);
    std::vector<double> g(W);
    HIPCHK(hipMemcpy(h.data(), c->d_hasg, (size_t)W * 4, hipMemcpyDeviceToHost));
    HIPCHK(hipMemcpy(g.data(), c->d_gauss, (size_t)W * 8, hipMemcpyDeviceToHost));
    for (int w = 0; w < W; ++w) {
      gauss_cache[2 * w] = h[w];
      gauss_cache[2 * w + 1] = g[w];
    }
  }
  return OLPE_OK;
}

int olpe_rng_set(olpe_ctx *c, const uint32_t *mt_state, const double *gauss_cache) {
  if (!c || !mt_state || !gauss_cache) return set_err(OLPE_EINVAL, "NULL argument");
  if (!c->d_mt) return set_err(OLPE_ESTATE, "no ensemble (call olpe_seed)");
  HIPCHK(hipSetDevice(c->device));
  HIPCHK(hipStreamSynchronize(c->stream));
  const int W = c->W;
  std::vector<uint32_t> key((size_t)W * MT_N);
  std::vector<int> pos(W), h(W);
  std::vector<double> g(W);
  for (int w = 0; w < W; ++w) {
    memcpy(key.data() + (size_t)w * MT_N, mt_state + (size_t)w * (MT_N + 1), MT_N * 4);
    pos[w] = (int)mt_state[(size_t)w * (MT_N + 1) + MT_N];
    if (pos[w] < 0 || pos[w] > MT_N) return set_err(OLPE_EINVAL, "bad MT position");
    h[w] = gauss_cache[2 * w] != 0.0;
    g[w] = gauss_cache[2 * w + 1];
  }
  HIPCHK(hipMemcpy(c->d_mt, key.data(), key.size() * 4, hipMemcpyHostToDevice));
  HIPCHK(hipMemcpy(c->d_mtpos, pos.data(), (size_t)W * 4, hipMemcpyHostToDevice));
  HIPCHK(hipMemcpy(c->d_hasg, h.data(), (size_t)W * 4, hipMemcpyHostToDevice));
  HIPCHK(hipMemcpy(c->d_gauss, g.data(), (size_t)W * 8, hipMemcpyHostToDevice));
  c->seeded = true;
  return OLPE_OK;
}

int olpe_rng_stream(olpe_ctx *c, int kind, int n, void *out) {
  if (!c || !out) return set_err(OLPE_EINVAL, "NULL argument");
  if (kind < 0 || kind > 3 || n <= 0) return set_err(OLPE_EINVAL, "bad kind/n");
  if (!c->seeded) return set_err(OLPE_ESTATE, "call olpe_seed first");
  HIPCHK(hipSetDevice(c->device));
  const size_t esz = kind == 0 ? 4 : 8;
  const size_t bytes = (size_t)c->W * n * esz;
  void *d = nullptr;
  HIPCHK(hipMalloc(&d, bytes));
  if (c->np == 16)
    hipLaunchKernelGGL(olpe_stream_kernel<16>, dim3(c->W), dim3(64), 0, c->stream, c->d_mt,
                       c->d_mtpos, c->d_hasg, c->d_gauss, c->W, kind, n, d);
  else
    hipLaunchKernelGGL(olpe_stream_kernel<19>, dim3(c->W), dim3(64), 0, c->stream, c->d_mt,
                       c->d_mtpos, c->d_hasg, c->d_gauss, c->W, kind, n, d);
  hipError_t e = hipGetLastError();
  if (e == hipSuccess) e = hipMemcpyAsync(out, d, bytes, hipMemcpyDeviceToHost, c->stream);
  if (e == hipSuccess) e = hipStreamSynchronize(c->stream);
  (void)hipFree(d);
  if (e != hipSuccess) return set_err(OLPE_EHIP, "rng stream: %s", hipGetErrorString(e));
  return OLPE_OK;
}

int olpe_test_hold_handoff(olpe_ctx *c, int on) {
  if (!c) return set_err(OLPE_EINVAL, "NULL ctx");
  c->hold_handoff = on != 0;
  return OLPE_OK;
}

int olpe_test_chain_set(olpe_ctx *c, const double *chain, long long nrec) {
  if (!c || nrec < 0 || (nrec > 0 && !chain)) return set_err(OLPE_EINVAL, "bad argument");
  if (!c->d_state || !c->seeded) return set_err(OLPE_ESTATE, "call olpe_seed first");
  HIPCHK(hipSetDevice(c->device));
  HIPCHK(hipStreamSynchronize(c->stream));
  int rc;
  const size_t chain_need = (size_t)c->W * nrec * c->ps;
  if (chain_need > c->chain_cap) {
    c->chain_cap = 0;
    if ((rc = dev_alloc(&c->d_chain, chain_need))) return rc;
    c->chain_cap = chain_need;
  }
  hipEvent_t *ev = c->ev[c->launches % olpe_ctx::kRing];
  if (!ev[0] || !ev[1]) return set_err(OLPE_EHIP, "launch events were not created");
  HIPCHK(hipEventRecord(ev[0], c->stream));
  if (chain_need)
    HIPCHK(hipMemcpyAsync(c->d_chain, chain, chain_need * 8, hipMemcpyHostToDevice, c->stream));
  HIPCHK(hipEventRecord(ev[1], c->stream));
  HIPCHK(hipStreamSynchronize(c->stream));
  c->chain_rows = nrec;
  ++c->launches;
  return OLPE_OK;
}

int olpe_trace_enable(olpe_ctx *c, int on) {
  if (!c) return set_err(OLPE_EINVAL, "NULL ctx");
  c->trace_on = on != 0;
  return OLPE_OK;
}

int olpe_trace_read(olpe_ctx *c, double *out) {
  if (!c || !out) return set_err(OLPE_EINVAL, "NULL argument");
  HIPCHK(hipSetDevice(c->device));
  HIPCHK(hipStreamSynchronize(c->stream));
  const size_t m = (size_t)c->W * c->trace_iters * kTraceF;
  if (m) HIPCHK(hipMemcpy(out, c->d_trace, m * 8, hipMemcpyDeviceToHost));
  return OLPE_OK;
}

int olpe_sync(olpe_ctx *c) {
  if (!c) return set_err(OLPE_EINVAL, "NULL ctx");
  HIPCHK(hipSetDevice(c->device));
  HIPCHK(hipStreamSynchronize(c->stream));
  return check_units(c);
}

int olpe_unit_stats(olpe_ctx *c, long long *out) {
  if (!c || !out) return set_err(OLPE_EINVAL, "NULL argument");
  HIPCHK(hipSetDevice(c->device));
  HIPCHK(hipStreamSynchronize(c->stream));
  unsigned long long v[2] = {0, 0};
  HIPCHK(hipMemcpy(v, c->d_queue + 2, sizeof(v), hipMemcpyDeviceToHost));
  out[0] = (long long)v[0];
  out[1] = (long long)(v[1] * 10);
  return OLPE_OK;
}

int olpe_last_units(olpe_ctx *c, int *units) {
  if (!c || !units) return set_err(OLPE_EINVAL, "NULL argument");
  *units = c->last_units;
  return OLPE_OK;
}

int olpe_kernel_times(olpe_ctx *c, int n, double *ms_out) {
  if (!c || !ms_out) return set_err(OLPE_EINVAL, "NULL argument");
  if (n < 1 || n > olpe_ctx::kRing || n > c->launches)
    return set_err(OLPE_EINVAL, "n = %d: 1..min(%d, launches so far = %lld)", n,
                   olpe_ctx::kRing, c->launches);
  HIPCHK(hipSetDevice(c->device));
  for (int i = 0; i < n; ++i) {
    hipEvent_t *ev = c->ev[(c->launches - n + i) % olpe_ctx::kRing];
    HIPCHK(hipEventSynchronize(ev[1]));
    float f = 0.f;
    HIPCHK(hipEventElapsedTime(&f, ev[0], ev[1]));
    ms_out[i] = f;
  }
  return OLPE_OK;
}

int olpe_last_kernel_ms(olpe_ctx *c, double *ms) {
  if (!c || !ms) return set_err(OLPE_EINVAL, "NULL argument");
  if (!c->launches) return set_err(OLPE_ESTATE, "no sampler launch yet");
  return olpe_kernel_times(c, 1, ms);
}

}
```

### olpefit_amd/csrc/olpe_comm.hip

```cpp
#include <hip/hip_runtime.h>
#include <rccl/rccl.h>

#include <stdarg.h>
#include <stdio.h>
#include <stdlib.h>
#include <string.h>

#include <chrono>
#include <thread>
#include <vector>

#include "../../include/olpe.h"
#include "../../include/olpe_test.h"
#include "olpe_comm_proto.h"
#include "olpe_internal.h"

using olpe::set_err;
namespace proto = olpe::proto;

namespace {

constexpr size_t kPoisonI64Off = 16, kPoisonF64Off = 32;
static_assert(proto::kCheckWords <= 16, "check words fit their slot");

double now_s() {
  return std::chrono::duration<double>(std::chrono::steady_clock::now().time_since_epoch())
      .count();
}

void dbg(const char *fmt, ...) {
  static const bool on = getenv("OLPE_COMM_DEBUG") != nullptr;
  if (!on) return;
  va_list ap;
  va_start(ap, fmt);
  fprintf(stderr, "[olpe comm %.3f] ", now_s());
  vfprintf(stderr, fmt, ap);
  fprintf(stderr, "\n");
  va_end(ap);
}

int abort_comm(olpe_ctx *c, const char *fmt, ...) {
  char msg[512];
  va_list ap;
  va_start(ap, fmt);
  vsnprintf(msg, sizeof(msg), fmt, ap);
  va_end(ap);
  dbg("abort: %s", msg);
  if (c->comm) (void)ncclCommAbort((ncclComm_t)c->comm);
  dbg("abort returned");
  c->comm = nullptr;
  c->comm_aborted = true;
  const double t0 = now_s();
  while (hipStreamQuery(c->stream) == hipErrorNotReady && now_s() - t0 < 10.0)
    std::this_thread::sleep_for(std::chrono::microseconds(200));
  (void)hipGetLastError();
  return set_err(OLPE_ECOMM, "%s", msg);
}

void poll_pause(int &spins) {
  if (++spins < 2000)
    std::this_thread::yield();
  else
    std::this_thread::sleep_for(std::chrono::microseconds(100));
}

int settle(olpe_ctx *c, ncclResult_t r, const char *what) {
  if (r == ncclSuccess) return OLPE_OK;
  if (r != ncclInProgress) {
    if (c->comm) return abort_comm(c, "%s: %s", what, ncclGetErrorString(r));
    return set_err(OLPE_ECOMM, "%s: %s", what, ncclGetErrorString(r));
  }
  const double t0 = now_s();
  int spins = 0;
  dbg("settle %s: in progress", what);
  for (;;) {
    ncclResult_t a = ncclInProgress;
    const ncclResult_t q = ncclCommGetAsyncError((ncclComm_t)c->comm, &a);
    if (spins == 0 || spins % 20000 == 0) dbg("settle %s: async state %d (%d)", what, (int)a, (int)q);
    if (q != ncclSuccess) return abort_comm(c, "%s: ncclCommGetAsyncError: %s", what,
                                            ncclGetErrorString(q));
    if (a == ncclSuccess) return OLPE_OK;
    if (a != ncclInProgress) return abort_comm(c, "%s: %s", what, ncclGetErrorString(a));
    if (c->comm_timeout_s > 0 && now_s() - t0 > c->comm_timeout_s)
      return abort_comm(c, "%s: the other ranks did not answer within %g s (olpe_comm_timeout): "
                        "communicator aborted", what, c->comm_timeout_s);
    poll_pause(spins);
  }
}

int comm_wait(olpe_ctx *c, const char *what) {
  if (!c->comm) {
    const hipError_t e = hipStreamSynchronize(c->stream);
    return e == hipSuccess ? OLPE_OK : set_err(OLPE_EHIP, "%s: %s", what, hipGetErrorString(e));
  }
  const double t0 = now_s();
  int spins = 0;
  for (;;) {
    const hipError_t e = hipStreamQuery(c->stream);
    if (e == hipSuccess) return OLPE_OK;
    if (e != hipErrorNotReady) return set_err(OLPE_EHIP, "%s: %s", what, hipGetErrorString(e));
    ncclResult_t a = ncclSuccess;
    if (ncclCommGetAsyncError((ncclComm_t)c->comm, &a) == ncclSuccess && a != ncclSuccess &&
        a != ncclInProgress)
      return abort_comm(c, "%s: RCCL reported %s", what, ncclGetErrorString(a));
    if (c->comm_timeout_s > 0 && now_s() - t0 > c->comm_timeout_s)
      return abort_comm(c, "%s: still waiting for the other ranks after %g s "
                        "(olpe_comm_timeout): communicator aborted", what, c->comm_timeout_s);
    poll_pause(spins);
  }
}

struct Rccl {
  olpe_ctx *c;
  bool has_comm() const { return c->comm != nullptr || c->comm_aborted; }
  int aborted(proto::Site s) const {
    return set_err(OLPE_ECOMM, "%s: the communicator was aborted earlier in this call",
                   proto::site_name(s));
  }
  bool forced(proto::Site s) const {
    return (c->mom_fault == 3 && s == proto::kCheckSend) ||
           (c->mom_fault == 4 && s == proto::kR1Back);
  }
  int fail(proto::Site s) const {
    return set_err(OLPE_EHIP, "%s: failure forced (olpe_moments_fault)", proto::site_name(s));
  }
  int copy(void *dst, const void *src, size_t n, hipMemcpyKind kind, proto::Site s) {
    if (forced(s)) return fail(s);
    const hipError_t e = hipMemcpyAsync(dst, src, n, kind, c->stream);
    return e == hipSuccess ? OLPE_OK
                           : set_err(OLPE_EHIP, "%s: %s", proto::site_name(s), hipGetErrorString(e));
  }
  int h2d(void *d, const void *h, size_t n, proto::Site s) {
    return copy(d, h, n, hipMemcpyHostToDevice, s);
  }
  int d2h(void *h, const void *d, size_t n, proto::Site s) {
    return copy(h, d, n, hipMemcpyDeviceToHost, s);
  }
  template <class T>
  int reduce(const T *send, T *recv, size_t n, ncclDataType_t t, ncclRedOp_t op, proto::Site s) {
    if (c->comm_aborted) return aborted(s);
    if (!c->comm) return send == recv ? OLPE_OK : copy(recv, send, n * sizeof(T),
                                                       hipMemcpyDeviceToDevice, s);
    return settle(c, ncclAllReduce(send, recv, n, t, op, (ncclComm_t)c->comm, c->stream),
                  proto::site_name(s));
  }
  int allreduce_max_i64(const long long *s, long long *r, size_t n, proto::Site site) {
    return reduce(s, r, n, ncclInt64, ncclMax, site);
  }
  int allreduce_sum_f64(const double *s, double *r, size_t n, proto::Site site) {
    return reduce(s, r, n, ncclDouble, ncclSum, site);
  }
  int allgather_f64(const double *s, double *r, size_t n, proto::Site site) {
    if (c->comm_aborted) return aborted(site);
    if (!c->comm) return copy(r, s, n * sizeof(double), hipMemcpyDeviceToDevice, site);
    return settle(c, ncclAllGather(s, r, n, ncclDouble, (ncclComm_t)c->comm, c->stream),
                  proto::site_name(site));
  }
  int wait(proto::Site s) { return comm_wait(c, proto::site_name(s)); }
  int local_summary(const double *dcen, double *d, proto::Site) {
    return olpe_moments_local(c, dcen, d);
  }
  long long *check_words() { return c->d_check; }
  const long long *poison_i64() { return c->d_check + kPoisonI64Off; }
  const double *poison_f64() { return reinterpret_cast<const double *>(c->d_check + kPoisonF64Off); }
};

}

int olpe_comm_setup(olpe_ctx *c) {
  constexpr size_t words = kPoisonF64Off + proto::kPoisonF64;
  if (hipMalloc((void **)&c->d_check, words * sizeof(long long)) != hipSuccess) {
    c->d_check = nullptr;
    (void)hipGetLastError();
    return set_err(OLPE_ENOMEM, "hipMalloc(%zu bytes) for the collectives' words", words * 8);
  }
  std::vector<long long> h(words, 0);
  h[kPoisonI64Off + proto::kLost] = 1;
  const double one = 1.0;
  memcpy(&h[kPoisonF64Off], &one, sizeof(one));
  HIPCHK(hipMemcpy(c->d_check, h.data(), words * sizeof(long long), hipMemcpyHostToDevice));
  return OLPE_OK;
}

void olpe_comm_release(olpe_ctx *c) {
  if (!c || !c->comm) return;
  ncclComm_t comm = (ncclComm_t)c->comm;
  const ncclResult_t r = ncclCommFinalize(comm);
  if (r == ncclSuccess || r == ncclInProgress) {
    const double t0 = now_s();
    ncclResult_t a = ncclInProgress;
    while (ncclCommGetAsyncError(comm, &a) == ncclSuccess && a == ncclInProgress &&
           now_s() - t0 < 30.0)
      std::this_thread::sleep_for(std::chrono::microseconds(200));
    if (a == ncclSuccess) {
      (void)ncclCommDestroy(comm);
      c->comm = nullptr;
      return;
    }
  }
  (void)ncclCommAbort(comm);
  c->comm = nullptr;
}

extern "C" {

int olpe_comm_unique_id(uint8_t *id128) {
  if (!id128) return set_err(OLPE_EINVAL, "NULL id buffer");
  static_assert(sizeof(ncclUniqueId) == 128, "ncclUniqueId must be 128 bytes");
  ncclUniqueId id;
  const ncclResult_t r = ncclGetUniqueId(&id);
  if (r != ncclSuccess) return set_err(OLPE_ECOMM, "ncclGetUniqueId: %s", ncclGetErrorString(r));
  memcpy(id128, &id, sizeof(id));
  return OLPE_OK;
}

int olpe_comm_timeout(olpe_ctx *c, double seconds) {
  if (!c || !(seconds >= 0)) return set_err(OLPE_EINVAL, "bad argument");
  c->comm_timeout_s = seconds;
  return OLPE_OK;
}

int olpe_comm_init(olpe_ctx *c, const uint8_t *id128, int nranks, int rank) {
  if (!c || !id128) return set_err(OLPE_EINVAL, "NULL argument");
  if (nranks < 1 || rank < 0 || rank >= nranks) return set_err(OLPE_EINVAL, "bad rank/nranks");
  HIPCHK(hipSetDevice(c->device));
  olpe_comm_release(c);
  c->comm_aborted = false;
  ncclUniqueId id;
  memcpy(&id, id128, sizeof(id));
  ncclConfig_t cfg = NCCL_CONFIG_INITIALIZER;
  cfg.blocking = 0;
  ncclComm_t comm = nullptr;
  dbg("ncclCommInitRankConfig %d/%d", rank, nranks);
  const ncclResult_t r = ncclCommInitRankConfig(&comm, nranks, id, rank, &cfg);
  dbg("ncclCommInitRankConfig returned %d", (int)r);
  if (r != ncclSuccess && r != ncclInProgress) {
    if (comm) (void)ncclCommAbort(comm);
    return set_err(OLPE_ECOMM, "ncclCommInitRankConfig: %s", ncclGetErrorString(r));
// ... 130 lines not shown
```

### olpefit_amd/csrc/olpe_fold.h

```cpp
#pragma once
#include <hip/hip_runtime.h>

#include <initializer_list>

#include "../../include/olpe.h"
#include "olpe_internal.h"

namespace olpe {

struct FoldBase {
  int device = 0;
  hipStream_t stream = nullptr;
  hipEvent_t ev = nullptr;
  bool ev_pending = false;
  const olpe_ctx *last_ctx = nullptr;
  long long last_launch = 0;
};

inline int open_device(int device) {
  if (device < 0) return set_err(OLPE_EINVAL, "device %d (there is no CPU path)", device);
  int ndev = 0;
  if (hipGetDeviceCount(&ndev) != hipSuccess || device >= ndev) {
    (void)hipGetLastError();
    return set_err(OLPE_EHIP, "no HIP device %d (%d visible)", device, ndev);
  }
  HIPCHK(hipSetDevice(device));
  return OLPE_OK;
}

inline int fold_open(FoldBase *b, int device) {
  b->device = device;
  if (hipStreamCreateWithFlags(&b->stream, hipStreamNonBlocking) != hipSuccess ||
      hipEventCreateWithFlags(&b->ev, hipEventDisableTiming) != hipSuccess)
    return set_err(OLPE_EHIP, "stream / event creation failed");
  return OLPE_OK;
}

inline void fold_close(FoldBase *b, std::initializer_list<void *> bufs) {
  (void)hipSetDevice(b->device);
  if (b->ev_pending) (void)hipEventSynchronize(b->ev);
  if (b->stream) (void)hipStreamSynchronize(b->stream);
  for (void *p : bufs)
    if (p) (void)hipFree(p);
  if (b->ev) (void)hipEventDestroy(b->ev);
  if (b->stream) (void)hipStreamDestroy(b->stream);
}

inline int alloc(void **p, size_t bytes, const char *what) {
  if (hipMalloc(p, bytes) != hipSuccess) {
    *p = nullptr;
    (void)hipGetLastError();
    return set_err(OLPE_ENOMEM, "hipMalloc(%zu bytes) for %s", bytes, what);
  }
  return OLPE_OK;
}

inline int grow(void **p, size_t *cap, size_t bytes, const char *what) {
  if (*cap >= bytes) return OLPE_OK;
  if (*p) (void)hipFree(*p);
  *p = nullptr;
  *cap = 0;
  int rc = alloc(p, bytes, what);
  if (!rc) *cap = bytes;
  return rc;
}

inline int wait_pending(FoldBase *b) {
  if (b->ev_pending) {
    HIPCHK(hipStreamWaitEvent(b->stream, b->ev, 0));
    b->ev_pending = false;
  }
  return OLPE_OK;
}

inline int drain(FoldBase *b) {
  if (b->ev_pending) {
    HIPCHK(hipEventSynchronize(b->ev));
    b->ev_pending = false;
  }
  HIPCHK(hipStreamSynchronize(b->stream));
  return OLPE_OK;
}

inline int fold_check(const FoldBase *b, const olpe_ctx *c) {
  if (!c->d_state || !c->launches) return set_err(OLPE_ESTATE, "no sampler launch yet");
  if (b->last_ctx == c && b->last_launch == c->launches)
    return set_err(OLPE_ESTATE, "the last launch's rows are already folded");
  return OLPE_OK;
}

inline void fold_mark(FoldBase *b, const olpe_ctx *c) {
  b->last_ctx = c;
  b->last_launch = c->launches;
}

inline int fold_enter(FoldBase *b, const olpe_ctx *c) {
  int rc;
  if ((rc = wait_pending(b))) return rc;
  HIPCHK(hipEventRecord(b->ev, b->stream));
  HIPCHK(hipStreamWaitEvent(c->stream, b->ev, 0));
  return OLPE_OK;
}

inline int fold_leave(FoldBase *b, const olpe_ctx *c) {
  HIPCHK(hipEventRecord(b->ev, c->stream));
  b->ev_pending = true;
  return OLPE_OK;
}

template <class Launch>
int fold_run(FoldBase *b, const olpe_ctx *c, bool any, Launch launch) {
  fold_mark(b, c);
  if (!any) return OLPE_OK;
  int rc;
  if ((rc = fold_enter(b, c))) return rc;
  if ((rc = launch(c->stream))) return rc;
  return fold_leave(b, c);
}

inline void fold_forget(FoldBase *b) {
  b->last_ctx = nullptr;
  b->last_launch = 0;
}

}
```

### olpefit_amd/csrc/olpe_internal.h

```cpp
#pragma once
#include <hip/hip_runtime.h>
#include <stddef.h>
#include <stdint.h>

struct olpe_ctx {
  int device = 0;
  int n = 0;
  int nsrc = 2;
  int bkgd_mode = 0;
  int np = 16, ps = 17;
  int eval_mode = 1;
  bool lds_img = true;
  int wpb = 0;
  hipStream_t stream = nullptr;
  static constexpr int kRing = 64;
  hipEvent_t ev[kRing][2] = {};
  long long launches = 0;
  double2 *d_DE = nullptr;
  double2 *d_DW = nullptr;
  int W = 0;
  bool seeded = false;
  long long count = 0;
  double *d_state = nullptr;
  uint32_t *d_tries = nullptr;
  uint32_t *d_acc = nullptr;
  uint32_t *d_mt = nullptr;
  int *d_mtpos = nullptr;
  double *d_gauss = nullptr;
  int *d_hasg = nullptr;
  long long *d_done = nullptr;
  double *d_chain = nullptr;
  size_t chain_cap = 0;
  long long chain_rows = 0;
  double *d_trace = nullptr;
  size_t trace_cap = 0;
  int trace_on = 0;
  long long trace_iters = 0;
  double *d_scratch = nullptr, *d_scratch2 = nullptr;
  size_t scratch_cap = 0, scratch2_cap = 0;
  unsigned long long *d_queue = nullptr;
  unsigned long long qbase = 0;
  bool queue_on = true;
  int n_cu = 0;
  unsigned *d_uflag = nullptr;
  unsigned utag = 0;
  int units_override = 0;
  bool hold_handoff = false;
  int last_units = 1;
  bool units_used = false;
  double wait_limit_s = 30;
  double wait_ticks_override = 0;
  int balance = -1;
  int ring_wpb = 12;
  int stagger = 0;
  double *d_widths = nullptr, *d_wdef = nullptr;
  uint32_t logmask = 0;
  void *d_tune = nullptr;
  bool tune_on = false;
  int tune_k = 0;
  double tune_target = 0, tune_gain = 0;
  double *d_mmean = nullptr, *d_mm2 = nullptr;
  size_t mom_cap = 0;
  long long mom_n = 0;
  long long mom_folded = 0;
  double *d_mpart = nullptr;
  size_t mpart_cap = 0;
  int mom_fault = 0;
  void *comm = nullptr;
  int nranks = 1, rank = 0;
  double *d_gather = nullptr;
  size_t gather_cap = 0;
  size_t gather_limit = 0;
  long long *d_check = nullptr;
  double comm_timeout_s = 600;
  bool comm_aborted = false;
};

namespace olpe {
int set_err(int code, const char *fmt, ...);
}
#define HIPCHK(expr)                                                                    \
  do {                                                                                  \
    hipError_t e_ = (expr);                                                             \
    if (e_ != hipSuccess)                                                               \
      return ::olpe::set_err(OLPE_EHIP, "%s failed: %s", #expr, hipGetErrorString(e_)); \
  } while (0)
void olpe_comm_release(olpe_ctx *c);
int olpe_widths_defaults(olpe_ctx *c, bool with_base);
int olpe_comm_setup(olpe_ctx *c);
int olpe_moments_prepare(olpe_ctx *c);
int olpe_moments_local(olpe_ctx *c, const double *d_centre, double *d_out);
```

### olpefit_amd/csrc/olpe_lik.hip

```cpp
#include <hip/hip_runtime.h>

#include <limits.h>
#include <math.h>
#include <stdint.h>
#include <stdlib.h>
#include <string.h>

#include <algorithm>
#include <type_traits>
#include <utility>
#include <vector>

#include "../../include/olpe.h"
#include "olpe_fold.h"
#include "olpe_internal.h"

namespace olpe_lik_dev {
#include "olpe_device.h"
}
namespace dev = olpe_lik_dev::olpe;

using namespace olpe;

#include "olpe_samples.h"
// ... 322 lines not shown
    hipLaunchKernelGGL((lik_pivot_kernel<2>), dim3(pixblocks), dim3(kThreads), 0, r->stream,
                       r->d_words, 1, r->d_pivot, r->d_DE, r->n, r->bkgd_mode, r->d_cimg);
  else
    hipLaunchKernelGGL((lik_pivot_kernel<3>), dim3(pixblocks), dim3(kThreads), 0, r->stream,
                       r->d_words, 1, r->d_pivot, r->d_DE, r->n, r->bkgd_mode, r->d_cimg);
  HIPCHK(hipGetLastError());
  unsigned long long one = 1;
  HIPCHK(hipMemcpyAsync(r->d_words + kWHavePivot, &one, 8, hipMemcpyHostToDevice, r->stream));
  HIPCHK(hipStreamSynchronize(r->stream));
  return OLPE_OK;
}

int read_words(olpe_lik *r, unsigned long long *w) {
  HIPCHK(hipMemcpy(w, r->d_words, kWords * 8, hipMemcpyDeviceToHost));
  return OLPE_OK;
}

int clear_sums(olpe_lik *r) {
  std::vector<double> z(4 * r->npix, 0.0);
  std::fill(z.begin() + 2 * r->npix, z.begin() + 3 * r->npix, (double)INFINITY);
  HIPCHK(hipMemcpy(r->d_sum, z.data(), 4 * r->npix * 8, hipMemcpyHostToDevice));
  return OLPE_OK;
}

int stage_vec(olpe_lik *r, const double *vec) {
  std::vector<double> v(vec, vec + r->np);
  v.push_back(0.0);
  HIPCHK(hipMemcpyAsync(r->d_vec, v.data(), (size_t)r->ps * 8, hipMemcpyHostToDevice, r->stream));
  HIPCHK(hipStreamSynchronize(r->stream));
  return OLPE_OK;
}

}

extern "C" {

int olpe_lik_create(olpe_ctx *c, const double *pivot, olpe_lik **out) {
  if (!out) return set_err(OLPE_EINVAL, "NULL out");
  *out = nullptr;
  if (!c) return set_err(OLPE_EINVAL, "NULL context");
  if (pivot && !finite_params(pivot, c->np))
    return set_err(OLPE_EINVAL, "the pivot vector has a non-finite parameter");
  int rows = 8;
  if (const char *e = getenv("OLPE_LIK_ROWS")) {
    rows = atoi(e);
    if (rows != 4 && rows != 8)
      return set_err(OLPE_EINVAL, "OLPE_LIK_ROWS=%s: 4 or 8 rows per tile", e);
  }
  const size_t npix = (size_t)c->n * c->n;
  const size_t per_block = npix * 32;
  if (per_block > kPartLimit)
    return set_err(OLPE_EINVAL, "a %dx%d frame needs %zu bytes of partial sums per block of %d "
                   "samples; the limit is %zu", c->n, c->n, per_block, kB, kPartLimit);
  const long long tiles = (long long)((c->n + 63) / 64) * ((c->n + rows - 1) / rows);
  if (tiles > 65535)
    return set_err(OLPE_EINVAL, "a %dx%d frame has %lld tiles of 64 x %d pixels; a grid "
                   "takes 65535", c->n, c->n, tiles, rows);
  HIPCHK(hipSetDevice(c->device));
  olpe_lik *r = new olpe_lik;
  r->n = c->n;
  r->nsrc = c->nsrc;
  r->np = c->np;
  r->bkgd_mode = c->bkgd_mode;
  r->ps = c->ps;
  r->rows = rows;
  r->npix = npix;
  r->piece_blocks = (int)std::min<size_t>(kMaxPieceBlocks, std::max<size_t>(1, kPartBudget / per_block));
  const size_t ks = 12 * (size_t)c->nsrc + 1, pb = (size_t)r->piece_blocks;
  const size_t finblocks = (npix + kThreads - 1) / kThreads;
  int rc = fold_open(r, c->device);
  if (!rc) rc = alloc((void **)&r->d_DE, npix * sizeof(double2), "the cutout");
  if (!rc) rc = alloc((void **)&r->d_sum, 4 * npix * 8, "the pixel state");
  if (!rc) rc = alloc((void **)&r->d_cimg, npix * 8, "the pivot's deviance");
  if (!rc) rc = alloc((void **)&r->d_pivot, (size_t)r->ps * 8, "the pivot vector");
  if (!rc) rc = alloc((void **)&r->d_best, (size_t)r->ps * 8, "the best row");
  if (!rc) rc = alloc((void **)&r->d_vec, (size_t)r->ps * 8, "the point vector");
  if (!rc) rc = alloc((void **)&r->d_words, kWords * 8, "the counters");
  if (!rc) rc = alloc(&r->d_info, pb * sizeof(BlkInfo), "the block table");
  if (!rc) rc = alloc((void **)&r->d_boff, pb * sizeof(int), "the block offsets");
  if (!rc) rc = alloc((void **)&r->d_desc, pb * kB * ks * 8, "the sample descriptors");
  if (!rc) rc = alloc((void **)&r->d_part, pb * per_block, "the partial sums");
  if (!rc) rc = alloc((void **)&r->d_planes, OLPE_LIK_PLANES * npix * 8, "the planes");
  if (!rc) rc = alloc(&r->d_fin, finblocks * sizeof(FinPart), "the finalize partials");
  if (!rc && (hipStreamSynchronize(c->stream) != hipSuccess ||
              hipMemcpy(r->d_DE, c->d_DE, npix * sizeof(double2), hipMemcpyDeviceToDevice) != hipSuccess ||
              hipMemset(r->d_cimg, 0, npix * 8) != hipSuccess ||
              hipMemset(r->d_pivot, 0, (size_t)r->ps * 8) != hipSuccess ||
              hipMemset(r->d_best, 0, (size_t)r->ps * 8) != hipSuccess ||
              hipMemset(r->d_vec, 0, (size_t)r->ps * 8) != hipSuccess ||
              hipMemset(r->d_words, 0, kWords * 8) != hipSuccess))
    rc = set_err(OLPE_EHIP, "cutout copy failed");
  if (!rc) rc = clear_sums(r);
  if (!rc && pivot) {
    std::vector<double> pv(pivot, pivot + c->np);
    pv.push_back(0.0);
    rc = set_pivot(r, pv.data());
    r->explicit_pivot = true;
  }
  if (rc) {
    olpe_lik_destroy(r);
    return rc;
  }
  *out = r;
  return OLPE_OK;
}

void olpe_lik_destroy(olpe_lik *r) {
  if (!r) return;
  fold_close(r, {r->d_DE, r->d_sum, r->d_cimg, r->d_pivot, r->d_best, r->d_vec, r->d_words,
                 r->d_info, r->d_boff, r->d_desc, r->d_part, r->d_planes, r->d_fin, r->d_stage});
  delete r;
}

int olpe_lik_fold_ctx(olpe_lik *r, olpe_ctx *c, int row_step, int walker_step) {
  if (!r || !c) return set_err(OLPE_EINVAL, "NULL argument");
  if (row_step <= 0 || walker_step <= 0)
    return set_err(OLPE_EINVAL, "row_step %d, walker_step %d: both must be > 0", row_step,
                   walker_step);
  if (c->device != r->device || c->n != r->n || c->nsrc != r->nsrc || c->bkgd_mode != r->bkgd_mode)
    return set_err(OLPE_EINVAL, "context of device %d, side %d, %d sources, bkgd_mode %d; this "
                   "object of device %d, side %d, %d sources, bkgd_mode %d", c->device, c->n,
                   c->nsrc, c->bkgd_mode, r->device, r->n, r->nsrc, r->bkgd_mode);
  int rc;
  if ((rc = fold_check(r, c))) return rc;
  HIPCHK(hipSetDevice(r->device));
  const long long nr = (c->chain_rows + row_step - 1) / row_step;
  const long long nw = ((long long)c->W + walker_step - 1) / walker_step;
  const RowMap m{c->d_chain, nr, (long long)walker_step * c->chain_rows * c->ps,
                 (long long)row_step * c->ps};
  return fold_run(r, c, nr > 0 && nw > 0,
                  [&](hipStream_t s) { return launch_fold(r, s, m, nr * nw); });
}

int olpe_lik_fold_rows(olpe_lik *r, const double *rows, long long nsamples) {
  if (!r) return set_err(OLPE_EINVAL, "NULL argument");
  if (nsamples < 0 || (nsamples > 0 && !rows))
    return set_err(OLPE_EINVAL, "%lld samples at %p", nsamples, (const void *)rows);
  if (nsamples == 0) return OLPE_OK;
  HIPCHK(hipSetDevice(r->device));
  const long long piece = (long long)r->piece_blocks * kB;
  int rc;
  if (!r->d_stage &&
      (rc = alloc((void **)&r->d_stage, (size_t)piece * r->ps * 8, "the row upload")))
    return rc;
  if ((rc = wait_pending(r))) return rc;
  for (long long s0 = 0; s0 < nsamples; s0 += piece) {
    const long long ns = std::min(piece, nsamples - s0);
    HIPCHK(hipMemcpyAsync(r->d_stage, rows + (size_t)s0 * r->ps, (size_t)ns * r->ps * 8,
                          hipMemcpyHostToDevice, r->stream));
    const RowMap m{r->d_stage, ns, 0, (long long)r->ps};
    if ((rc = launch_fold(r, r->stream, m, ns))) return rc;
    HIPCHK(hipStreamSynchronize(r->stream));
  }
  return OLPE_OK;
}

int olpe_lik_get(olpe_lik *r, long long *n, long long *n_bad, double *pivot, double *a1,
                 double *a2, double *m, double *l, double *best) {
  if (!r) return set_err(OLPE_EINVAL, "NULL argument");
  HIPCHK(hipSetDevice(r->device));
  int rc;
  if ((rc = drain(r))) return rc;
  unsigned long long w[kWords];
  if ((rc = read_words(r, w))) return rc;
  if (n) *n = (long long)w[kWUsed];
  if (n_bad) *n_bad = (long long)w[kWBad];
  if (pivot) {
// ... 170 lines not shown
```

### olpefit_amd/csrc/olpe_moments.hip

```cpp
#include <hip/hip_runtime.h>

#include <string.h>

#include <algorithm>
#include <vector>

#include "../../include/olpe.h"
#include "olpe_internal.h"
#include "olpe_reduce.h"

using olpe::block_sum;
using olpe::set_err;

namespace {

constexpr int kThreads = 256;
constexpr int kWalkersPerBlock = 256;

constexpr int kFoldRows = 8;
constexpr int kFoldWaves = 4;
constexpr int kWaveRows = 16;
constexpr long long kFoldRowsMin = 64;

__device__ __forceinline__ void chan_merge(double &m, double &q, double &n, double mb,
// ... 109 lines not shown
}

__global__ __launch_bounds__(kThreads) void summary_stage1(
    const double *__restrict__ mean, const double *__restrict__ m2,
    const double *__restrict__ centre, const uint32_t *__restrict__ tries,
    const uint32_t *__restrict__ acc, long long W, int ps, int np, int nblk,
    double *__restrict__ part) {
  __shared__ double red[kThreads];
  __shared__ unsigned long long cnt[2 * 32];
  const int b = blockIdx.x;
  const long long w0 = (long long)b * kWalkersPerBlock;
  const long long w1 = w0 + kWalkersPerBlock < W ? w0 + kWalkersPerBlock : W;
  for (int k = 0; k < ps; ++k) {
    const double *mk = mean + (size_t)k * W, *qk = m2 + (size_t)k * W;
    const double ck = centre ? centre[k] : 0.0;
    double a = 0.0, q = 0.0, d2 = 0.0;
    for (long long w = w0 + threadIdx.x; w < w1; w += kThreads) {
      const double m = mk[w];
      a += m;
      q += qk[w];
      const double d = m - ck;
      d2 = fma(d, d, d2);
    }
    a = block_sum<kThreads>(a, red);
    q = block_sum<kThreads>(q, red);
    d2 = block_sum<kThreads>(d2, red);
    if (threadIdx.x == 0) {
      part[((size_t)0 * ps + k) * nblk + b] = a;
      part[((size_t)1 * ps + k) * nblk + b] = q;
      part[((size_t)2 * ps + k) * nblk + b] = centre ? d2 : 0.0;
    }
  }
  for (int i = threadIdx.x; i < 2 * np; i += kThreads) cnt[i] = 0;
  __syncthreads();
  const size_t e0 = (size_t)w0 * np, e1 = (size_t)w1 * np;
  for (size_t e = e0 + threadIdx.x; e < e1; e += kThreads) {
    const int k = (int)(e % (size_t)np);
    atomicAdd(&cnt[k], (unsigned long long)tries[e]);
    atomicAdd(&cnt[np + k], (unsigned long long)acc[e]);
  }
  __syncthreads();
  double *pc = part + (size_t)3 * ps * nblk;
  for (int i = threadIdx.x; i < 2 * np; i += kThreads) pc[(size_t)i * nblk + b] = (double)cnt[i];
}

int ensure_moments(olpe_ctx *c) {
  const size_t need = (size_t)c->W * c->ps;
  if (c->d_mmean && c->mom_cap >= need) return OLPE_OK;
  if (c->d_mmean) (void)hipFree(c->d_mmean);
  if (c->d_mm2) (void)hipFree(c->d_mm2);
  c->d_mmean = c->d_mm2 = nullptr;
  c->mom_cap = 0;
  if (hipMalloc((void **)&c->d_mmean, need * sizeof(double)) != hipSuccess ||
      hipMalloc((void **)&c->d_mm2, need * sizeof(double)) != hipSuccess) {
    if (c->d_mmean) (void)hipFree(c->d_mmean);
    c->d_mmean = nullptr;
    return set_err(OLPE_ENOMEM, "hipMalloc(%zu bytes) for the walker moments", 2 * need * 8);
  }
  c->mom_cap = need;
  return OLPE_OK;
}

}

int olpe_moments_prepare(olpe_ctx *c) {
  if (c->mom_fault == 1)
    return set_err(OLPE_ENOMEM, "moment partials: allocation failure forced (olpe_moments_fault)");
  const int nblk = (int)((c->W + kWalkersPerBlock - 1) / kWalkersPerBlock);
  const size_t need = ((size_t)3 * c->ps + 2 * c->np) * nblk;
  if (need > c->mpart_cap) {
    if (c->d_mpart) (void)hipFree(c->d_mpart);
    c->d_mpart = nullptr;
    c->mpart_cap = 0;
    if (hipMalloc((void **)&c->d_mpart, need * sizeof(double)) != hipSuccess) {
      c->d_mpart = nullptr;
      (void)hipGetLastError();
      return set_err(OLPE_ENOMEM, "hipMalloc(%zu bytes) for the moment partials", need * 8);
    }
    c->mpart_cap = need;
  }
  int rc;
  if ((rc = ensure_moments(c))) return rc;
  if (c->mom_n == 0) {
    HIPCHK(hipMemsetAsync(c->d_mmean, 0, (size_t)c->W * c->ps * 8, c->stream));
    HIPCHK(hipMemsetAsync(c->d_mm2, 0, (size_t)c->W * c->ps * 8, c->stream));
  }
  return OLPE_OK;
}

int olpe_moments_local(olpe_ctx *c, const double *d_centre, double *d_out) {
  if (c->mom_fault == 2)
    return set_err(OLPE_EHIP, "moments summary launch: failure forced (olpe_moments_fault)");
  const int nblk = (int)((c->W + kWalkersPerBlock - 1) / kWalkersPerBlock);
  const size_t cols = (size_t)3 * c->ps + 2 * c->np;
  if (!c->d_mpart || c->mpart_cap < cols * nblk || !c->d_mmean)
    return set_err(OLPE_ESTATE, "moments summary before its buffers were prepared");
  hipLaunchKernelGGL(summary_stage1, dim3(nblk), dim3(kThreads), 0, c->stream, c->d_mmean,
                     c->d_mm2, d_centre, c->d_tries, c->d_acc, (long long)c->W, c->ps, c->np,
                     nblk, c->d_mpart);
  HIPCHK(hipGetLastError());
  hipLaunchKernelGGL(olpe::reduce_stage2_kernel<kThreads>, dim3((unsigned)cols), dim3(kThreads),
                     0, c->stream, c->d_mpart, nblk, d_out + 2);
  HIPCHK(hipGetLastError());
  return OLPE_OK;
}

extern "C" {

int olpe_moments_fault(olpe_ctx *c, int where) {
  if (!c || where < 0 || where > 4) return set_err(OLPE_EINVAL, "bad argument");
  c->mom_fault = where;
  return OLPE_OK;
}

int olpe_moments_accumulate(olpe_ctx *c) {
  if (!c) return set_err(OLPE_EINVAL, "NULL ctx");
  if (!c->d_state || !c->launches) return set_err(OLPE_ESTATE, "no sampler launch yet");
  if (c->mom_folded == c->launches)
    return set_err(OLPE_ESTATE, "the last launch's rows are already in the moments");
  HIPCHK(hipSetDevice(c->device));
  int rc;
  if ((rc = ensure_moments(c))) return rc;
  c->mom_folded = c->launches;
  const long long nrec = c->chain_rows;
  if (nrec == 0) return OLPE_OK;
  if (nrec >= kFoldRowsMin && c->ps <= 64) {
    hipLaunchKernelGGL(fold_rows_kernel, dim3((unsigned)((c->W + kFoldWaves - 1) / kFoldWaves)),
                       dim3(64 * kFoldWaves), 0, c->stream, c->d_chain, (long long)c->W, c->ps,
                       nrec, (double)c->mom_n, c->d_mmean, c->d_mm2);
  } else {
    const long long total = (long long)c->W * c->ps;
    hipLaunchKernelGGL(fold_cols_kernel, dim3((unsigned)((total + kThreads - 1) / kThreads)),
                       dim3(kThreads), 0, c->stream, c->d_chain, (long long)c->W, c->ps, nrec,
                       (double)c->mom_n, c->d_mmean, c->d_mm2);
  }
  HIPCHK(hipGetLastError());
  c->mom_n += nrec;
  return OLPE_OK;
}

int olpe_moments_reset(olpe_ctx *c) {
  if (!c) return set_err(OLPE_EINVAL, "NULL ctx");
  c->mom_n = 0;
  c->mom_folded = c->launches;
  return OLPE_OK;
}

int olpe_moments_get(olpe_ctx *c, long long *n, double *mean, double *m2) {
  if (!c || !n) return set_err(OLPE_EINVAL, "NULL argument");
  if (!c->d_state) return set_err(OLPE_ESTATE, "no ensemble");
  HIPCHK(hipSetDevice(c->device));
  HIPCHK(hipStreamSynchronize(c->stream));
  *n = c->mom_n;
  const size_t m = (size_t)c->W * c->ps;
  std::vector<double> t(m, 0.0);
  double *outs[2] = {mean, m2};
  double *devs[2] = {c->d_mmean, c->d_mm2};
  for (int i = 0; i < 2; ++i) {
    if (!outs[i]) continue;
    if (c->mom_n && devs[i]) {
      HIPCHK(hipMemcpy(t.data(), devs[i], m * 8, hipMemcpyDeviceToHost));
    } else {
      std::fill(t.begin(), t.end(), 0.0);
    }
    for (int w = 0; w < c->W; ++w)
      for (int k = 0; k < c->ps; ++k) outs[i][(size_t)w * c->ps + k] = t[(size_t)k * c->W + w];
  }
  return OLPE_OK;
}

int olpe_moments_set(olpe_ctx *c, long long n, const double *mean, const double *m2) {
  if (!c || n < 0 || (n > 0 && (!mean || !m2))) return set_err(OLPE_EINVAL, "bad argument");
  if (!c->d_state) return set_err(OLPE_ESTATE, "call olpe_seed first");
  HIPCHK(hipSetDevice(c->device));
  HIPCHK(hipStreamSynchronize(c->stream));
  int rc;
  if ((rc = ensure_moments(c))) return rc;
  const size_t m = (size_t)c->W * c->ps;
  if (n > 0) {
    std::vector<double> t(m);
    const double *ins[2] = {mean, m2};
    double *devs[2] = {c->d_mmean, c->d_mm2};
    for (int i = 0; i < 2; ++i) {
      for (int w = 0; w < c->W; ++w)
        for (int k = 0; k < c->ps; ++k) t[(size_t)k * c->W + w] = ins[i][(size_t)w * c->ps + k];
      HIPCHK(hipMemcpy(devs[i], t.data(), m * 8, hipMemcpyHostToDevice));
    }
  }
  c->mom_n = n;
  c->mom_folded = c->launches;
  return OLPE_OK;
}

int olpe_moments_summary(olpe_ctx *c, const double *centre, double *out) {
  if (!c || !out) return set_err(OLPE_EINVAL, "NULL argument");
  if (!c->d_state) return set_err(OLPE_ESTATE, "no ensemble");
  HIPCHK(hipSetDevice(c->device));
  const size_t len = (size_t)OLPE_MOMENTS_LEN(c->ps, c->np);
  double *d = nullptr;
  HIPCHK(hipMalloc((void **)&d, (len + c->ps) * sizeof(double)));
  double *dc = nullptr;
  hipError_t e = hipSuccess;
  if (centre) {
    dc = d + len;
    e = hipMemcpyAsync(dc, centre, c->ps * sizeof(double), hipMemcpyHostToDevice, c->stream);
  }
  int rc = e == hipSuccess ? olpe_moments_prepare(c) : OLPE_OK;
  if (e == hipSuccess && rc == OLPE_OK) rc = olpe_moments_local(c, dc, d);
  if (e == hipSuccess && rc == OLPE_OK)
    e = hipMemcpyAsync(out, d, len * sizeof(double), hipMemcpyDeviceToHost, c->stream);
  if (e == hipSuccess && rc == OLPE_OK) e = hipStreamSynchronize(c->stream);
  (void)hipFree(d);
  if (rc) return rc;
  if (e != hipSuccess) return set_err(OLPE_EHIP, "moments summary: %s", hipGetErrorString(e));
  out[0] = (double)c->mom_n;
  out[1] = (double)c->W;
  return OLPE_OK;
}

}
```

### olpefit_amd/csrc/olpe_normal.hip

```cpp
#include <hip/hip_runtime.h>

#include <math.h>
#include <stdint.h>
#include <stdlib.h>
#include <string.h>

#include "../../include/olpe.h"
#include "../../include/olpe_test.h"
#include "olpe_fold.h"
#include "olpe_internal.h"

namespace olpe_normal_dev {
#include "olpe_device.h"
}
namespace dev = olpe_normal_dev::olpe;

using namespace olpe;

#include "olpe_samples.h"

namespace {

constexpr int kWaves = 4;
typedef double v4d __attribute__((ext_vector_type(4)));
// ... 195 lines not shown
  }
  const int col = lane & 15;
#pragma unroll
  for (int q = 0; q < 4; ++q) {
    const int rowi = (lane >> 4) + 4 * q;
    const double v = nanout ? nanv : acc[q];
    if (rowi <= col) {
      oj[rowi * P + col] = v;
      oj[col * P + rowi] = v;
    }
    if constexpr (HI > 0) {
      const double vh = nanout ? nanv : acch[q];
      if (col < HI) {
        oj[rowi * P + 16 + col] = vh;
        oj[(16 + col) * P + rowi] = vh;
      }
      if constexpr (CM) {
        const double vc = nanout ? nanv : accc[q];
        if (rowi <= col && col < HI) {
          oj[(16 + rowi) * P + 16 + col] = vc;
          oj[(16 + col) * P + 16 + rowi] = vc;
        }
      }
    }
  }
}

template <int NSRC>
__global__ __launch_bounds__(kThreads) void jacobian_kernel(const double *__restrict__ vec, int n,
                                                            int bkgd_mode,
                                                            double *__restrict__ planes) {
  using L = dev::Layout<NSRC>;
  const int pix = blockIdx.x * kThreads + threadIdx.x;
  const int npix = n * n;
  if (pix >= npix) return;
  double p[L::NP], d[12 * NSRC + 1], J[L::NP];
#pragma unroll
  for (int k = 0; k < L::NP; ++k) p[k] = vec[k];
  make_desc<NSRC>(p, bkgd_mode, d);
  const Chain<NSRC> ch = make_chain<NSRC>(p);
  const int i = pix / n, j = pix - i * n;
  (void)pixel_jac<NSRC>(d, ch, bkgd_mode, (double)j, (double)i, J);
#pragma unroll
  for (int k = 0; k < L::NP; ++k) planes[(size_t)k * npix + pix] = J[k];
}

int reserve(olpe_ctx *c, size_t pin, size_t pout) {
  int rc;
  if (c->scratch_cap < pin) {
    if (c->d_scratch) (void)hipFree(c->d_scratch);
    c->d_scratch = nullptr;
    c->scratch_cap = 0;
    if ((rc = alloc((void **)&c->d_scratch, pin * 8, "the parameter vectors"))) return rc;
    c->scratch_cap = pin;
  }
  if (c->scratch2_cap < pout) {
    if (c->d_scratch2) (void)hipFree(c->d_scratch2);
    c->d_scratch2 = nullptr;
    c->scratch2_cap = 0;
    if ((rc = alloc((void **)&c->d_scratch2, pout * 8, "the normal equations"))) return rc;
    c->scratch2_cap = pout;
  }
  return OLPE_OK;
}

}

extern "C" {

int olpe_normal_batch(olpe_ctx *c, const double *params, int W, double *chi2, double *grad,
                      double *jtj) {
  if (!c || !params || !chi2 || !grad || !jtj) return set_err(OLPE_EINVAL, "NULL argument");
  if (W <= 0) return set_err(OLPE_EINVAL, "W must be > 0");
  bool corner_mfma = false;
  if (const char *e = getenv("OLPE_NORMAL_CORNER")) {
    if (strcmp(e, "mfma") && strcmp(e, "valu"))
      return set_err(OLPE_EINVAL, "OLPE_NORMAL_CORNER=%s: mfma or valu", e);
    corner_mfma = !strcmp(e, "mfma");
  }
  HIPCHK(hipSetDevice(c->device));
  const size_t P = (size_t)c->np, nw = (size_t)W;
  const size_t pin = nw * c->ps, pout = nw * (1 + P + P * P);
  int rc;
  HIPCHK(hipStreamSynchronize(c->stream));
  if ((rc = reserve(c, pin, pout))) return rc;
  HIPCHK(hipMemcpyAsync(c->d_scratch, params, pin * 8, hipMemcpyHostToDevice, c->stream));
  double *d_chi = c->d_scratch2, *d_grad = d_chi + nw, *d_jtj = d_grad + nw * P;
  const dim3 grid((unsigned)((nw + kWaves - 1) / kWaves)), block(kWaves * 64);
  if (c->nsrc == 2)
    hipLaunchKernelGGL((normal_kernel<2>), grid, block, 0, c->stream, c->d_DE, c->n,
                       c->bkgd_mode, c->d_scratch, W, d_chi, d_grad, d_jtj);
  else if (corner_mfma)
    hipLaunchKernelGGL((normal_kernel<3, true>), grid, block, 0, c->stream, c->d_DE, c->n,
                       c->bkgd_mode, c->d_scratch, W, d_chi, d_grad, d_jtj);
  else
    hipLaunchKernelGGL((normal_kernel<3>), grid, block, 0, c->stream, c->d_DE, c->n,
                       c->bkgd_mode, c->d_scratch, W, d_chi, d_grad, d_jtj);
  HIPCHK(hipGetLastError());
  HIPCHK(hipMemcpyAsync(chi2, d_chi, nw * 8, hipMemcpyDeviceToHost, c->stream));
  HIPCHK(hipMemcpyAsync(grad, d_grad, nw * P * 8, hipMemcpyDeviceToHost, c->stream));
  HIPCHK(hipMemcpyAsync(jtj, d_jtj, nw * P * P * 8, hipMemcpyDeviceToHost, c->stream));
  HIPCHK(hipStreamSynchronize(c->stream));
  return OLPE_OK;
}

int olpe_test_jacobian(olpe_ctx *c, const double *vec, double *planes) {
  if (!c || !vec || !planes) return set_err(OLPE_EINVAL, "NULL argument");
  HIPCHK(hipSetDevice(c->device));
  const size_t npix = (size_t)c->n * c->n, pout = (size_t)c->np * npix;
  int rc;
  HIPCHK(hipStreamSynchronize(c->stream));
  if ((rc = reserve(c, (size_t)c->ps, pout))) return rc;
  HIPCHK(hipMemcpyAsync(c->d_scratch, vec, (size_t)c->ps * 8, hipMemcpyHostToDevice, c->stream));
  const dim3 grid((unsigned)((npix + kThreads - 1) / kThreads)), block(kThreads);
  if (c->nsrc == 2)
    hipLaunchKernelGGL((jacobian_kernel<2>), grid, block, 0, c->stream, c->d_scratch, c->n,
                       c->bkgd_mode, c->d_scratch2);
  else
    hipLaunchKernelGGL((jacobian_kernel<3>), grid, block, 0, c->stream, c->d_scratch, c->n,
                       c->bkgd_mode, c->d_scratch2);
  HIPCHK(hipGetLastError());
  HIPCHK(hipMemcpyAsync(planes, c->d_scratch2, pout * 8, hipMemcpyDeviceToHost, c->stream));
  HIPCHK(hipStreamSynchronize(c->stream));
  return OLPE_OK;
}

}
```

### olpefit_amd/csrc/olpe_resid.hip

```cpp
#include <hip/hip_runtime.h>

#include <limits.h>
#include <math.h>
#include <stdint.h>
#include <stdlib.h>
#include <string.h>

#include <algorithm>
#include <type_traits>
#include <utility>
#include <vector>

#include "../../include/olpe.h"
#include "olpe_fold.h"
#include "olpe_internal.h"

namespace olpe_resid_dev {
#include "olpe_device.h"
}
namespace dev = olpe_resid_dev::olpe;

using namespace olpe;

#include "olpe_samples.h"
// ... 232 lines not shown
}

int launch_fold(olpe_resid *r, hipStream_t st, const RowMap &m, long long count) {
  const long long piece = (long long)r->piece_blocks * kB;
  for (long long s0 = 0; s0 < count; s0 += piece) {
    const int ns = (int)std::min(piece, count - s0);
    const int rc = r->nsrc == 2 ? launch_piece_t<2>(r, st, m, s0, ns)
                                : launch_piece_t<3>(r, st, m, s0, ns);
    if (rc) return rc;
  }
  return OLPE_OK;
}

int set_pivot(olpe_resid *r, const double *pivot) {
  HIPCHK(hipMemcpyAsync(r->d_pivot, pivot, (size_t)r->ps * 8, hipMemcpyHostToDevice, r->stream));
  const unsigned pixblocks = (unsigned)((r->npix + kThreads - 1) / kThreads);
  if (r->nsrc == 2)
    hipLaunchKernelGGL((resid_pivot_kernel<2>), dim3(pixblocks), dim3(kThreads), 0, r->stream,
                       r->d_words, 1, r->d_pivot, r->n, r->bkgd_mode, r->d_pivimg);
  else
    hipLaunchKernelGGL((resid_pivot_kernel<3>), dim3(pixblocks), dim3(kThreads), 0, r->stream,
                       r->d_words, 1, r->d_pivot, r->n, r->bkgd_mode, r->d_pivimg);
  HIPCHK(hipGetLastError());
  unsigned long long one = 1;
  HIPCHK(hipMemcpyAsync(r->d_words + kWHavePivot, &one, 8, hipMemcpyHostToDevice, r->stream));
  HIPCHK(hipStreamSynchronize(r->stream));
  return OLPE_OK;
}

int read_words(olpe_resid *r, unsigned long long *w) {
  HIPCHK(hipMemcpy(w, r->d_words, kWords * 8, hipMemcpyDeviceToHost));
  return OLPE_OK;
}

}

extern "C" {

int olpe_resid_create(olpe_ctx *c, const double *pivot, olpe_resid **out) {
  if (!out) return set_err(OLPE_EINVAL, "NULL out");
  *out = nullptr;
  if (!c) return set_err(OLPE_EINVAL, "NULL context");
  if (pivot && !finite_params(pivot, c->np))
    return set_err(OLPE_EINVAL, "the pivot vector has a non-finite parameter");
  int rows = 16;
  if (const char *e = getenv("OLPE_RESID_ROWS")) {
    rows = atoi(e);
    if (rows != 8 && rows != 16)
      return set_err(OLPE_EINVAL, "OLPE_RESID_ROWS=%s: 8 or 16 rows per tile", e);
  }
  const size_t npix = (size_t)c->n * c->n;
  const size_t per_block = npix * 16;
  if (per_block > kPartLimit)
    return set_err(OLPE_EINVAL, "a %dx%d frame needs %zu bytes of partial sums per block of %d "
                   "samples; the limit is %zu", c->n, c->n, per_block, kB, kPartLimit);
  const long long tiles = (long long)((c->n + 63) / 64) * ((c->n + rows - 1) / rows);
  if (tiles > 65535)
    return set_err(OLPE_EINVAL, "a %dx%d frame has %lld tiles of 64 x %d pixels; a grid "
                   "takes 65535", c->n, c->n, tiles, rows);
  HIPCHK(hipSetDevice(c->device));
  olpe_resid *r = new olpe_resid;
  r->n = c->n;
  r->nsrc = c->nsrc;
  r->bkgd_mode = c->bkgd_mode;
  r->ps = c->ps;
  r->rows = rows;
  r->npix = npix;
  r->piece_blocks = (int)std::min<size_t>(kMaxPieceBlocks, std::max<size_t>(1, kPartBudget / per_block));
  const size_t ks = 12 * (size_t)c->nsrc + 1, pb = (size_t)r->piece_blocks;
  const size_t finblocks = (npix + kThreads - 1) / kThreads;
  int rc = fold_open(r, c->device);
  if (!rc) rc = alloc((void **)&r->d_DE, npix * sizeof(double2), "the cutout");
  if (!rc) rc = alloc((void **)&r->d_sum, 2 * npix * 8, "the shifted sums");
  if (!rc) rc = alloc((void **)&r->d_pivimg, npix * 8, "the pivot image");
  if (!rc) rc = alloc((void **)&r->d_pivot, (size_t)r->ps * 8, "the pivot vector");
  if (!rc) rc = alloc((void **)&r->d_best, (size_t)r->ps * 8, "the best row");
  if (!rc) rc = alloc((void **)&r->d_words, kWords * 8, "the counters");
  if (!rc) rc = alloc(&r->d_info, pb * sizeof(BlkInfo), "the block table");
  if (!rc) rc = alloc((void **)&r->d_boff, pb * sizeof(int), "the block offsets");
  if (!rc) rc = alloc((void **)&r->d_desc, pb * kB * ks * 8, "the sample descriptors");
  if (!rc) rc = alloc((void **)&r->d_part, pb * per_block, "the partial sums");
  if (!rc) rc = alloc((void **)&r->d_planes, OLPE_RESID_PLANES * npix * 8, "the planes");
  if (!rc) rc = alloc(&r->d_fin, finblocks * sizeof(FinPart), "the finalize partials");
  if (!rc && (hipStreamSynchronize(c->stream) != hipSuccess ||
              hipMemcpy(r->d_DE, c->d_DE, npix * sizeof(double2), hipMemcpyDeviceToDevice) != hipSuccess ||
              hipMemset(r->d_sum, 0, 2 * npix * 8) != hipSuccess ||
              hipMemset(r->d_pivimg, 0, npix * 8) != hipSuccess ||
              hipMemset(r->d_pivot, 0, (size_t)r->ps * 8) != hipSuccess ||
              hipMemset(r->d_best, 0, (size_t)r->ps * 8) != hipSuccess ||
              hipMemset(r->d_words, 0, kWords * 8) != hipSuccess))
    rc = set_err(OLPE_EHIP, "cutout copy failed");
  if (!rc && pivot) {
    std::vector<double> pv(pivot, pivot + c->np);
    pv.push_back(0.0);
    rc = set_pivot(r, pv.data());
    r->explicit_pivot = true;
  }
  if (rc) {
    olpe_resid_destroy(r);
    return rc;
  }
  *out = r;
  return OLPE_OK;
}

void olpe_resid_destroy(olpe_resid *r) {
  if (!r) return;
  fold_close(r, {r->d_DE, r->d_sum, r->d_pivimg, r->d_pivot, r->d_best, r->d_words, r->d_info,
                 r->d_boff, r->d_desc, r->d_part, r->d_planes, r->d_fin, r->d_stage});
  delete r;
}

int olpe_resid_fold_ctx(olpe_resid *r, olpe_ctx *c, int row_step, int walker_step) {
  if (!r || !c) return set_err(OLPE_EINVAL, "NULL argument");
  if (row_step <= 0 || walker_step <= 0)
    return set_err(OLPE_EINVAL, "row_step %d, walker_step %d: both must be > 0", row_step,
                   walker_step);
  if (c->device != r->device || c->n != r->n || c->nsrc != r->nsrc || c->bkgd_mode != r->bkgd_mode)
    return set_err(OLPE_EINVAL, "context of device %d, side %d, %d sources, bkgd_mode %d; this "
                   "object of device %d, side %d, %d sources, bkgd_mode %d", c->device, c->n,
                   c->nsrc, c->bkgd_mode, r->device, r->n, r->nsrc, r->bkgd_mode);
  int rc;
  if ((rc = fold_check(r, c))) return rc;
  HIPCHK(hipSetDevice(r->device));
  const long long nr = (c->chain_rows + row_step - 1) / row_step;
  const long long nw = ((long long)c->W + walker_step - 1) / walker_step;
  const RowMap m{c->d_chain, nr, (long long)walker_step * c->chain_rows * c->ps,
                 (long long)row_step * c->ps};
  return fold_run(r, c, nr > 0 && nw > 0,
                  [&](hipStream_t s) { return launch_fold(r, s, m, nr * nw); });
}

int olpe_resid_fold_rows(olpe_resid *r, const double *rows, long long nsamples) {
  if (!r) return set_err(OLPE_EINVAL, "NULL argument");
  if (nsamples < 0 || (nsamples > 0 && !rows))
    return set_err(OLPE_EINVAL, "%lld samples at %p", nsamples, (const void *)rows);
  if (nsamples == 0) return OLPE_OK;
  HIPCHK(hipSetDevice(r->device));
  const long long piece = (long long)r->piece_blocks * kB;
  int rc;
  if (!r->d_stage &&
      (rc = alloc((void **)&r->d_stage, (size_t)piece * r->ps * 8, "the row upload")))
    return rc;
  if ((rc = wait_pending(r))) return rc;
  for (long long s0 = 0; s0 < nsamples; s0 += piece) {
    const long long ns = std::min(piece, nsamples - s0);
    HIPCHK(hipMemcpyAsync(r->d_stage, rows + (size_t)s0 * r->ps, (size_t)ns * r->ps * 8,
                          hipMemcpyHostToDevice, r->stream));
    const RowMap m{r->d_stage, ns, 0, (long long)r->ps};
    if ((rc = launch_fold(r, r->stream, m, ns))) return rc;
    HIPCHK(hipStreamSynchronize(r->stream));
  }
  return OLPE_OK;
}

int olpe_resid_get(olpe_resid *r, long long *n, long long *n_bad, double *pivot, double *s1,
                   double *s2, double *best) {
  if (!r) return set_err(OLPE_EINVAL, "NULL argument");
  HIPCHK(hipSetDevice(r->device));
  int rc;
  if ((rc = drain(r))) return rc;
  unsigned long long w[kWords];
  if ((rc = read_words(r, w))) return rc;
  if (n) *n = (long long)w[kWUsed];
  if (n_bad) *n_bad = (long long)w[kWBad];
  if (pivot) {
    if (w[kWHavePivot]) HIPCHK(hipMemcpy(pivot, r->d_pivot, (size_t)r->ps * 8, hipMemcpyDeviceToHost));
// ... 126 lines not shown
```

### olpefit_amd/csrc/olpe_tune.hip

```cpp
#include <hip/hip_runtime.h>

#include <math.h>

#include <algorithm>
#include <vector>

#include "../../include/olpe.h"
#include "olpe_internal.h"
#include "olpe_reduce.h"

using namespace olpe;

namespace {

constexpr int kP = 19;
constexpr int kThreads = 256;
constexpr int kMaxBlocks = 64;
constexpr int kTuneLog = OLPE_TUNE_LOG;

struct TuneRec {
  long long dT[kP], dA[kP];
  double w[kP];
};
struct TuneBuf {
  unsigned long long now[2 * kP];
  long long prev[2 * kP];
  TuneRec log[kTuneLog];
};

struct WidthsArg {
  double w[kP];
};

__global__ void widths_set_kernel(int np, WidthsArg a, double *w) {
  const int j = threadIdx.x;
  if (j < np) w[j] = a.w[j];
}

template <int NP>
__global__ __launch_bounds__(kThreads) void tune_sum_kernel(const uint32_t *__restrict__ tries,
                                                            const uint32_t *__restrict__ acc,
                                                            long long W, unsigned long long *now) {
  __shared__ unsigned long long red[kThreads];
  unsigned long long t[NP], a[NP];
#pragma unroll
  for (int j = 0; j < NP; ++j) t[j] = a[j] = 0ull;
  const long long step = (long long)gridDim.x * kThreads;
  for (long long w = (long long)blockIdx.x * kThreads + threadIdx.x; w < W; w += step) {
    const uint32_t *tr = tries + (size_t)w * NP, *ac = acc + (size_t)w * NP;
#pragma unroll
    for (int j = 0; j < NP; ++j) {
      t[j] += tr[j];
      a[j] += ac[j];
    }
  }
#pragma unroll
  for (int j = 0; j < NP; ++j) {
    const unsigned long long st = block_word<kThreads, WordSum>(t[j], red);
    const unsigned long long sa = block_word<kThreads, WordSum>(a[j], red);
    if (threadIdx.x == 0) {
      atomicAdd(now + j, st);
      atomicAdd(now + kP + j, sa);
    }
  }
}

__global__ void tune_update_kernel(int np, TuneBuf *b, double *w, const double *wdef, double g,
                                   double target, TuneRec *rec) {
  const int j = threadIdx.x;
  if (j >= np) return;
  const long long T = (long long)b->now[j], A = (long long)b->now[kP + j];
  if (rec) {
    const long long dT = T - b->prev[j], dA = A - b->prev[kP + j];
    double wj = w[j];
    if (dT > 0) {
      const double a = (double)dA / (double)dT;
      const double f = 1.0 + g * (a - target);
      double v = wj * f;
      const double lo = wdef[j] / 1024.0, hi = wdef[j] * 64.0;
      v = v < lo ? lo : v;
      v = v > hi ? hi : v;
      wj = v;
      w[j] = wj;
    }
    rec->dT[j] = dT;
    rec->dA[j] = dA;
    rec->w[j] = wj;
  }
  b->prev[j] = T;
  b->prev[kP + j] = A;
}

int enqueue_sums(olpe_ctx *c, TuneBuf *b) {
  HIPCHK(hipMemsetAsync(b->now, 0, sizeof(b->now), c->stream));
  const unsigned blocks =
      (unsigned)std::min<long long>(((long long)c->W + kThreads - 1) / kThreads, kMaxBlocks);
  if (c->np == 16)
    hipLaunchKernelGGL(tune_sum_kernel<16>, dim3(blocks), dim3(kThreads), 0, c->stream, c->d_tries,
                       c->d_acc, (long long)c->W, b->now);
  else
    hipLaunchKernelGGL(tune_sum_kernel<19>, dim3(blocks), dim3(kThreads), 0, c->stream, c->d_tries,
                       c->d_acc, (long long)c->W, b->now);
  HIPCHK(hipGetLastError());
  return OLPE_OK;
}

}

extern "C" {

int olpe_widths_set(olpe_ctx *c, const double *w) {
  if (!c) return set_err(OLPE_EINVAL, "NULL ctx");
  HIPCHK(hipSetDevice(c->device));
  if (!w) return olpe_widths_defaults(c, false);
  for (int j = 0; j < c->np; ++j) {
    if (!std::isfinite(w[j]) || !(w[j] > 0.0))
      return set_err(OLPE_EINVAL, "width %d is %g: widths are finite and > 0", j, w[j]);
    if (((c->logmask >> j) & 1u) && w[j] > OLPE_LOG_WIDTH_MAX)
      return set_err(OLPE_EINVAL, "width %d is %g dex: a log-proposed parameter takes at most %g",
                     j, w[j], (double)OLPE_LOG_WIDTH_MAX);
  }
  WidthsArg a = {};
  for (int j = 0; j < c->np; ++j) a.w[j] = w[j];
  hipLaunchKernelGGL(widths_set_kernel, dim3(1), dim3(64), 0, c->stream, c->np, a, c->d_widths);
  HIPCHK(hipGetLastError());
  return OLPE_OK;
}

int olpe_widths_get(olpe_ctx *c, double *out) {
  if (!c || !out) return set_err(OLPE_EINVAL, "NULL argument");
  HIPCHK(hipSetDevice(c->device));
  HIPCHK(hipMemcpyAsync(out, c->d_widths, (size_t)c->np * 8, hipMemcpyDeviceToHost, c->stream));
  HIPCHK(hipStreamSynchronize(c->stream));
  return OLPE_OK;
}

int olpe_tune_begin(olpe_ctx *c, double target, double gain) {
  if (!c) return set_err(OLPE_EINVAL, "NULL ctx");
  if (!(target > 0.0 && target < 1.0) || !(gain > 0.0) || !std::isfinite(gain) ||
      !(gain * target < 1.0))
    return set_err(OLPE_EINVAL, "tuner: 0 < target < 1, gain > 0 and gain * target < 1 "
                   "(got target %g, gain %g)", target, gain);
  if (!c->d_tries || !c->d_acc) return set_err(OLPE_ESTATE, "call olpe_seed first");
  HIPCHK(hipSetDevice(c->device));
  if (!c->d_tune) {
    if (hipMalloc(&c->d_tune, sizeof(TuneBuf)) != hipSuccess) {
      c->d_tune = nullptr;
      (void)hipGetLastError();
      return set_err(OLPE_ENOMEM, "hipMalloc(%zu bytes) for the tuner", sizeof(TuneBuf));
    }
  }
  TuneBuf *b = static_cast<TuneBuf *>(c->d_tune);
  c->tune_on = false;
  int rc;
  if ((rc = enqueue_sums(c, b))) return rc;
  hipLaunchKernelGGL(tune_update_kernel, dim3(1), dim3(64), 0, c->stream, c->np, b, c->d_widths,
                     c->d_wdef, 0.0, target, (TuneRec *)nullptr);
  HIPCHK(hipGetLastError());
  c->tune_on = true;
  c->tune_k = 0;
  c->tune_target = target;
  c->tune_gain = gain;
  return OLPE_OK;
}

int olpe_tune_step(olpe_ctx *c) {
  if (!c) return set_err(OLPE_EINVAL, "NULL ctx");
  if (!c->tune_on) return set_err(OLPE_ESTATE, "call olpe_tune_begin first");
  if (c->tune_k >= kTuneLog)
    return set_err(OLPE_ESTATE, "the tuner's log holds %d steps: end the session", kTuneLog);
  if (!c->d_tries || !c->d_acc) return set_err(OLPE_ESTATE, "no ensemble");
  HIPCHK(hipSetDevice(c->device));
  TuneBuf *b = static_cast<TuneBuf *>(c->d_tune);
  int rc;
  if ((rc = enqueue_sums(c, b))) return rc;
  const int k = c->tune_k + 1;
  const double g = c->tune_gain / sqrt((double)k);
  hipLaunchKernelGGL(tune_update_kernel, dim3(1), dim3(64), 0, c->stream, c->np, b, c->d_widths,
                     c->d_wdef, g, c->tune_target, b->log + (k - 1));
  HIPCHK(hipGetLastError());
  c->tune_k = k;
  return OLPE_OK;
}

int olpe_tune_get(olpe_ctx *c, int *steps, long long *dT, long long *dA, double *widths) {
  if (!c || !steps) return set_err(OLPE_EINVAL, "NULL argument");
  if (!c->d_tune) return set_err(OLPE_ESTATE, "no tuning session yet");
  HIPCHK(hipSetDevice(c->device));
  HIPCHK(hipStreamSynchronize(c->stream));
  const int k = c->tune_k;
  *steps = k;
  if (!k || (!dT && !dA && !widths)) return OLPE_OK;
  std::vector<TuneRec> h((size_t)k);
  HIPCHK(hipMemcpy(h.data(), static_cast<TuneBuf *>(c->d_tune)->log, (size_t)k * sizeof(TuneRec),
                   hipMemcpyDeviceToHost));
  for (int i = 0; i < k; ++i)
    for (int j = 0; j < c->np; ++j) {
      if (dT) dT[(size_t)i * c->np + j] = h[i].dT[j];
      if (dA) dA[(size_t)i * c->np + j] = h[i].dA[j];
      if (widths) widths[(size_t)i * c->np + j] = h[i].w[j];
    }
  return OLPE_OK;
}

int olpe_tune_end(olpe_ctx *c) {
  if (!c) return set_err(OLPE_EINVAL, "NULL ctx");
  if (!c->tune_on) return set_err(OLPE_ESTATE, "no tuning session to end");
  c->tune_on = false;
  return OLPE_OK;
}

}
```

Baseline: 563.7 million.

## Overlap consecutive Gibbs launches across two streams with per-walker tag handoff

Launches Gibbs kernels alternately on two side streams with separate queue counters, chain buffers and events. A new launch can start before the previous one finishes: a gate kernel waits on the prior queue, and each walker waits on its previous-launch tag before its first unit. Other work routes through a main stream that joins the side streams first. The aim is to hide kernel launch gaps and tail idleness between chunks, at the cost of more synchronisation complexity and risk of deadlock or ordering bugs.

New measurement: 573.5 million, median of 6. +1.7%, better.

```diff
diff --git a/include/olpe.h b/include/olpe.h
--- a/include/olpe.h
+++ b/include/olpe.h
@@ -62,6 +62,7 @@
 
 int olpe_trace_enable(olpe_ctx *ctx, int on);
 int olpe_trace_read(olpe_ctx *ctx, double *out);
+
 
 int olpe_sync(olpe_ctx *ctx);
 int olpe_last_kernel_ms(olpe_ctx *ctx, double *ms);
diff --git a/olpefit_amd/_lib.py b/olpefit_amd/_lib.py
--- a/olpefit_amd/_lib.py
+++ b/olpefit_amd/_lib.py
@@ -147,6 +147,7 @@
     "olpe_cov_reset": (_i, [_P]),
     "olpe_moments_fault": (_i, [_P, _i]),
     "olpe_test_hold_handoff": (_i, [_P, _i]),
+    "olpe_test_overlaps": (_i, [_P, _pll]),
     "olpe_test_chain_set": (_i, [_P, _pd, _ll]),
     "olpe_test_jacobian": (_i, [_P, _pd, _pd]),
 }
diff --git a/olpefit_amd/core.py b/olpefit_amd/core.py
--- a/olpefit_amd/core.py
+++ b/olpefit_amd/core.py
@@ -326,6 +326,11 @@
     def hold_handoff(self, on: bool = True):
         check(self._lib.olpe_test_hold_handoff(self._ctx, 1 if on else 0))
 
+    def overlaps(self) -> int:
+        n = C.c_longlong(0)
+        check(self._lib.olpe_test_overlaps(self._ctx, C.byref(n)))
+        return int(n.value)
+
     def test_chain_set(self, chain):
         ch = np.ascontiguousarray(chain, dtype=np.float64)
         if ch.ndim != 3 or ch.shape[2] != self.ps or (self.W and ch.shape[0] != self.W):
diff --git a/olpefit_amd/csrc/olpe.hip b/olpefit_amd/csrc/olpe.hip
--- a/olpefit_amd/csrc/olpe.hip
+++ b/olpefit_amd/csrc/olpe.hip
@@ -69,6 +69,8 @@
   int units;
   unsigned *uflag;
   unsigned utag;
+  unsigned ptag;
+  unsigned long long *ustats;
   unsigned *uerr;
   unsigned long long wait_ticks;
   int balance;
@@ -211,6 +213,21 @@
   }
 }
 
+__global__ __launch_bounds__(64) void olpe_overlap_gate_kernel(unsigned long long *queue,
+                                                               unsigned long long base,
+                                                               unsigned *err,
+                                                               unsigned long long limit) {
+  if (threadIdx.x != 0) return;
+  const unsigned long long t0 = __builtin_amdgcn_s_memrealtime();
+  while (__hip_atomic_load((gu64 *)queue, __ATOMIC_RELAXED, __HIP_MEMORY_SCOPE_AGENT) <= base) {
+    if (__builtin_amdgcn_s_memrealtime() - t0 > limit) {
+      __hip_atomic_store((gu32 *)err, 1u, __ATOMIC_RELAXED, __HIP_MEMORY_SCOPE_AGENT);
+      break;
+    }
+    __builtin_amdgcn_s_sleep(16);
+  }
+}
+
 constexpr int kCtrlPrio = 2;
 constexpr int kGlobalWavesPerEU = 3;
 template <int NSRC, int NT, bool LDS_IMG, int WPB, bool FAST>
@@ -312,9 +329,12 @@
       it_s = q * k + (r * k) / units;
       it_e = q * (k + 1) + (r * (k + 1)) / units;
       if (k > 0 && active)
-        unit_wait(K()->uflag + w, K()->utag + (unsigned)k, K()->uerr, K()->queue + 2, lane,
+        unit_wait(K()->uflag + w, K()->utag + (unsigned)k, K()->uerr, K()->ustats, lane,
                   K()->wait_ticks, K()->hold);
     }
+    if (k == 0 && K()->ptag && active)
+      unit_wait(K()->uflag + w, K()->ptag, K()->uerr, K()->ustats, lane, K()->wait_ticks,
+                K()->hold);
     int it_end = it_e;
     if constexpr (RING) {
       if (lane == 0) s_prog[2 + wave] = active ? (unsigned)(it_e - it_s) : 0u;
@@ -593,8 +613,9 @@
       st_wt(K()->gauss + w, mt.gauss);
       st_wt(K()->done_at + w, done_at);
     }
-    if (k < K()->units - 1) {
-      if (k == 0 && K()->hold) hold_handoff(K()->hold, K()->uerr, K()->wait_ticks);
+    if (K()->queue) {
+      if (k == 0 && k < K()->units - 1 && K()->hold)
+        hold_handoff(K()->hold, K()->uerr, K()->wait_ticks);
       unit_publish(K()->uflag + w, K()->utag + (unsigned)(k + 1), lane);
     }
     wave_sync();
@@ -769,8 +790,13 @@
 }
 
 
+struct LaunchSlot {
+  int slot;
+  bool serial;
+};
+
 template <int NSRC, int NT, bool LDS, int WPB, bool FAST>
-int launch_gibbs_t(olpe_ctx *c, const GibbsArgs &a) {
+int launch_gibbs_t(olpe_ctx *c, const GibbsArgs &a, const LaunchSlot &l) {
   constexpr bool RING = !LDS && FAST && ring_wpb(NT, WPB);
   const size_t shm = lds_bytes(c, WPB, RING);
   auto k = olpe_gibbs_kernel<NSRC, NT, LDS, WPB, FAST>;
@@ -782,12 +808,16 @@
     attr_set.fetch_or(bit, std::memory_order_release);
   }
   unsigned blocks = (unsigned)((a.W + WPB - 1) / WPB);
+  const int p = c->par;
+  const hipStream_t s = c->sstream[p];
   GibbsArgs q = a;
   q.queue = nullptr;
   q.qbase = 0;
   q.units = 1;
   q.uflag = c->d_uflag;
   q.utag = 0;
+  q.ptag = 0;
+  q.ustats = c->d_queue + 2;
   q.uerr = reinterpret_cast<unsigned *>(c->d_queue + 1);
   q.stagger = c->stagger;
   q.hold = nullptr;
@@ -799,8 +829,8 @@
                         : 1;
   if (c->queue_on && c->d_queue && (LDS || RING || units > 1)) {
     if (blocks > resident) blocks = resident;
-    q.queue = c->d_queue;
-    q.qbase = c->qbase;
+    q.queue = c->d_queue + (p ? 5 : 0);
+    q.qbase = c->qbase2[p];
     q.units = units;
     c->utag += 16;
     q.utag = c->utag;
@@ -810,15 +840,22 @@
         return set_err(OLPE_EINVAL, "olpe_test_hold_handoff: %lld walkers need %u resident "
                        "workgroups, the device holds %u", a.W, need, resident);
       blocks = need;
-      HIPCHK(hipMemsetAsync(c->d_queue + 4, 0, sizeof(unsigned long long), c->stream));
-      q.hold = reinterpret_cast<unsigned *>(c->d_queue + 4);
-    }
-  }
+      q.hold = reinterpret_cast<unsigned *>(c->d_queue + (p ? 6 : 4));
+    }
+  }
+  const bool overlap = c->overlap_on && q.queue && c->prev_queue && c->prev_W == a.W &&
+                       !l.serial && !a.trace && c->prev_slot >= 0;
+  if (overlap) {
+    q.ptag = c->prev_tag;
+  } else if (c->prev_slot >= 0) {
+    HIPCHK(hipStreamWaitEvent(s, c->ev[c->prev_slot][1], 0));
+  }
+  if (q.hold) HIPCHK(hipMemsetAsync(q.hold, 0, sizeof(unsigned long long), s));
   q.balance = c->balance >= 0 ? c->balance
             : (LDS && FAST && NSRC == 2 && WPB == 16 && q.units == 1 &&
                a.W <= (long long)resident * WPB) ? 1 : 0;
   c->last_units = q.units;
-  if (q.units > 1) c->units_used = true;
+  if (q.units > 1 || overlap) c->units_used = true;
   {
     const double chunk = (double)((a.n_iters + q.units - 1) / q.units);
     const double ticks = chunk * (double)a.n * (double)a.n * (2.0 * NSRC) * 0.8;
@@ -827,48 +864,65 @@
                        : (unsigned long long)std::min(std::max(ticks, 3e9), 1e15);
     c->wait_limit_s = (double)q.wait_ticks * 1e-8;
   }
-  hipLaunchKernelGGL(k, dim3(blocks), dim3(WPB * 64), shm, c->stream, q);
+  if (overlap) {
+    hipLaunchKernelGGL(olpe_overlap_gate_kernel, dim3(1), dim3(64), 0, s, c->prev_qptr,
+                       c->prev_qbase, q.uerr, q.wait_ticks);
+    HIPCHK(hipGetLastError());
+  }
+  HIPCHK(hipEventRecord(c->ev[l.slot][0], s));
+  hipLaunchKernelGGL(k, dim3(blocks), dim3(WPB * 64), shm, s, q);
   HIPCHK(hipGetLastError());
+  c->prev_qptr = q.queue;
+  c->prev_qbase = q.qbase;
+  HIPCHK(hipEventRecord(c->ev[l.slot][1], s));
+  HIPCHK(hipEventRecord(c->ev_tail[p], s));
+  c->pend = true;
+  c->ev_ovl[l.slot] = overlap;
+  c->overlaps += overlap ? 1 : 0;
   if (q.queue) {
     const unsigned long long tot = (unsigned long long)a.W * (unsigned long long)q.units;
-    c->qbase += RING ? (tot + WPB - 1) / WPB + blocks : tot + (unsigned long long)blocks * WPB;
-  }
-  return OLPE_OK;
-}
-
-template <int NSRC, bool FAST> int launch_gibbs_m(olpe_ctx *c, const GibbsArgs &a) {
+    c->qbase2[p] += RING ? (tot + WPB - 1) / WPB + blocks : tot + (unsigned long long)blocks * WPB;
+  }
+  c->prev_queue = q.queue != nullptr;
+  c->prev_W = a.W;
+  c->prev_tag = q.utag + (unsigned)q.units;
+  c->prev_slot = l.slot;
+  return OLPE_OK;
+}
+
+template <int NSRC, bool FAST> int launch_gibbs_m(olpe_ctx *c, const GibbsArgs &a, const LaunchSlot &l) {
   if (c->lds_img) {
     switch (c->n) {
-      case 32: return launch_gibbs_t<NSRC, 32, true, 12, FAST>(c, a);
+      case 32: return launch_gibbs_t<NSRC, 32, true, 12, FAST>(c, a, l);
       case 64: {
         const long long r16 = 16LL * c->n_cu, r12 = 12LL * c->n_cu;
         int wpb = c->wpb ? c->wpb
                 : (NSRC == 2 && (!FAST || a.W >= 8 * r16 || (a.W > r12 && a.W <= r16)))
                       ? 16 : 12;
         if (wpb == 16 && lds_bytes(c, 16) > 160 * 1024) wpb = 12;
-        if (wpb == 8) return launch_gibbs_t<NSRC, 64, true, 8, FAST>(c, a);
-        if (wpb == 12) return launch_gibbs_t<NSRC, 64, true, 12, FAST>(c, a);
-        return launch_gibbs_t<NSRC, 64, true, 16, FAST>(c, a);
+        if (wpb == 8) return launch_gibbs_t<NSRC, 64, true, 8, FAST>(c, a, l);
+        if (wpb == 12) return launch_gibbs_t<NSRC, 64, true, 12, FAST>(c, a, l);
+        return launch_gibbs_t<NSRC, 64, true, 16, FAST>(c, a, l);
       }
-      default: return launch_gibbs_t<NSRC, 0, true, 16, FAST>(c, a);
+      default: return launch_gibbs_t<NSRC, 0, true, 16, FAST>(c, a, l);
     }
   }
   if (c->n == 128) {
     if constexpr (FAST) {
       if (c->ring_wpb && c->queue_on && c->d_queue && c->d_uflag) {
-        return launch_gibbs_t<NSRC, 128, false, 12, FAST>(c, a);
+        return launch_gibbs_t<NSRC, 128, false, 12, FAST>(c, a, l);
       }
     }
-    return launch_gibbs_t<NSRC, 128, false, 4, FAST>(c, a);
-  }
-  if (lds_bytes(c, 4) > 160 * 1024) return launch_gibbs_t<NSRC, 0, false, 1, FAST>(c, a);
-  return launch_gibbs_t<NSRC, 0, false, 4, FAST>(c, a);
-}
-
-int launch_gibbs(olpe_ctx *c, const GibbsArgs &a) {
+    return launch_gibbs_t<NSRC, 128, false, 4, FAST>(c, a, l);
+  }
+  if (lds_bytes(c, 4) > 160 * 1024) return launch_gibbs_t<NSRC, 0, false, 1, FAST>(c, a, l);
+  return launch_gibbs_t<NSRC, 0, false, 4, FAST>(c, a, l);
+}
+
+int launch_gibbs(olpe_ctx *c, const GibbsArgs &a, const LaunchSlot &l) {
   const bool fast = c->eval_mode == OLPE_EVAL_FAST;
-  if (c->nsrc == 2) return fast ? launch_gibbs_m<2, true>(c, a) : launch_gibbs_m<2, false>(c, a);
-  return fast ? launch_gibbs_m<3, true>(c, a) : launch_gibbs_m<3, false>(c, a);
+  if (c->nsrc == 2) return fast ? launch_gibbs_m<2, true>(c, a, l) : launch_gibbs_m<2, false>(c, a, l);
+  return fast ? launch_gibbs_m<3, true>(c, a, l) : launch_gibbs_m<3, false>(c, a, l);
 }
 
 int ensure_ensemble(olpe_ctx *c, int W) {
@@ -884,11 +938,11 @@
   if ((rc = dev_alloc(&c->d_hasg, (size_t)W))) return rc;
   if ((rc = dev_alloc(&c->d_done, (size_t)W))) return rc;
   if ((rc = dev_alloc(&c->d_uflag, (size_t)W))) return rc;
-  HIPCHK(hipMemsetAsync(c->d_uflag, 0, (size_t)W * sizeof(unsigned), c->stream));
-  HIPCHK(hipMemsetAsync(c->d_state, 0, (size_t)W * c->ps * sizeof(double), c->stream));
-  HIPCHK(hipMemsetAsync(c->d_tries, 0, (size_t)W * c->np * sizeof(uint32_t), c->stream));
-  HIPCHK(hipMemsetAsync(c->d_acc, 0, (size_t)W * c->np * sizeof(uint32_t), c->stream));
-  HIPCHK(hipMemsetAsync(c->d_done, 0xff, (size_t)W * sizeof(long long), c->stream));
+  HIPCHK(hipMemsetAsync(c->d_uflag, 0, (size_t)W * sizeof(unsigned), olpe_main(c)));
+  HIPCHK(hipMemsetAsync(c->d_state, 0, (size_t)W * c->ps * sizeof(double), olpe_main(c)));
+  HIPCHK(hipMemsetAsync(c->d_tries, 0, (size_t)W * c->np * sizeof(uint32_t), olpe_main(c)));
+  HIPCHK(hipMemsetAsync(c->d_acc, 0, (size_t)W * c->np * sizeof(uint32_t), olpe_main(c)));
+  HIPCHK(hipMemsetAsync(c->d_done, 0xff, (size_t)W * sizeof(long long), olpe_main(c)));
   c->W = W;
   c->seeded = false;
   c->count = 0;
@@ -899,8 +953,41 @@
 
 }
 
+hipStream_t olpe_main(olpe_ctx *c) {
+  if (c->pend) {
+    for (hipEvent_t e : c->ev_tail)
+      if (e) (void)hipStreamWaitEvent(c->stream, e, 0);
+    c->pend = false;
+  }
+  c->main_dirty = true;
+  return c->stream;
+}
+
+static int follow_main(olpe_ctx *c, hipStream_t s) {
+  if (!c->main_dirty) return OLPE_OK;
+  HIPCHK(hipEventRecord(c->ev_main, c->stream));
+  HIPCHK(hipStreamWaitEvent(s, c->ev_main, 0));
+  return OLPE_OK;
+}
+
+int olpe_fold_stream(olpe_ctx *c, hipStream_t *s) {
+  *s = c->sstream[c->par];
+  int rc;
+  if ((rc = follow_main(c, *s))) return rc;
+  HIPCHK(hipStreamWaitEvent(*s, c->ev_fold, 0));
+  return OLPE_OK;
+}
+
+int olpe_fold_done(olpe_ctx *c) {
+  const hipStream_t s = c->sstream[c->par];
+  HIPCHK(hipEventRecord(c->ev_fold, s));
+  HIPCHK(hipEventRecord(c->ev_tail[c->par], s));
+  c->pend = true;
+  return OLPE_OK;
+}
+
 int olpe_widths_defaults(olpe_ctx *c, bool with_base) {
-  hipLaunchKernelGGL(widths_default_kernel, dim3(1), dim3(64), 0, c->stream, c->nsrc, c->d_widths,
+  hipLaunchKernelGGL(widths_default_kernel, dim3(1), dim3(64), 0, olpe_main(c), c->nsrc, c->d_widths,
                      with_base ? c->d_wdef : nullptr);
   HIPCHK(hipGetLastError());
   return OLPE_OK;
@@ -1025,19 +1112,24 @@
   }
   int rc;
   hipError_t e1 = hipStreamCreateWithFlags(&c->stream, hipStreamNonBlocking);
+  for (auto &s : c->sstream)
+    if (e1 == hipSuccess) e1 = hipStreamCreateWithFlags(&s, hipStreamNonBlocking);
+  hipEvent_t *order[] = {&c->ev_tail[0], &c->ev_tail[1], &c->ev_fold, &c->ev_main};
+  for (hipEvent_t *e : order)
+    if (e1 == hipSuccess) e1 = hipEventCreateWithFlags(e, hipEventDisableTiming);
   if (e1 != hipSuccess) {
-    delete c;
-    return set_err(OLPE_EHIP, "hipStreamCreate: %s", hipGetErrorString(e1));
+    olpe_destroy(c);
+    return set_err(OLPE_EHIP, "stream / event creation: %s", hipGetErrorString(e1));
   }
   for (auto &pair : c->ev)
     for (auto &ev : pair)
       if (hipEventCreate(&ev) != hipSuccess) ev = nullptr;
   if ((rc = dev_alloc(&c->d_DE, npix)) || (rc = dev_alloc(&c->d_DW, npix)) ||
-      (rc = dev_alloc(&c->d_queue, 5)) || (rc = olpe_comm_setup(c))) {
+      (rc = dev_alloc(&c->d_queue, 7)) || (rc = olpe_comm_setup(c))) {
     olpe_destroy(c);
     return rc;
   }
-  if (hipMemset(c->d_queue, 0, 5 * sizeof(unsigned long long)) != hipSuccess ||
+  if (hipMemset(c->d_queue, 0, 7 * sizeof(unsigned long long)) != hipSuccess ||
       hipDeviceGetAttribute(&c->n_cu, hipDeviceAttributeMultiprocessorCount, device) !=
           hipSuccess || c->n_cu <= 0) {
     olpe_destroy(c);
@@ -1052,6 +1144,7 @@
     }
     c->units_override = p;
   }
+  if (const char *e = getenv("OLPE_OVERLAP")) c->overlap_on = atoi(e) != 0;
   if (const char *e = getenv("OLPE_RING")) {
     const int v = atoi(e);
     if (v != 0 && v != 12) {
@@ -1074,7 +1167,7 @@
     olpe_destroy(c);
     return rc;
   }
-  if (hipStreamSynchronize(c->stream) != hipSuccess) {
+  if (hipStreamSynchronize(olpe_main(c)) != hipSuccess) {
     olpe_destroy(c);
     return set_err(OLPE_EHIP, "filling in the default jump widths failed");
   }
@@ -1085,11 +1178,13 @@
 void olpe_destroy(olpe_ctx *c) {
   if (!c) return;
   (void)hipSetDevice(c->device);
+  for (hipStream_t s : c->sstream)
+    if (s) (void)hipStreamSynchronize(s);
   if (c->stream) (void)hipStreamSynchronize(c->stream);
   olpe_comm_release(c);
   void *ptrs[] = {c->d_DE, c->d_DW, c->d_state, c->d_tries, c->d_acc,
                   c->d_mt, c->d_mtpos, c->d_gauss, c->d_hasg,  c->d_done,
-                  c->d_chain, c->d_trace, c->d_scratch, c->d_scratch2, c->d_queue,
+                  c->d_chain2[0], c->d_chain2[1], c->d_trace, c->d_scratch, c->d_scratch2, c->d_queue,
                   c->d_gather, c->d_uflag, c->d_mmean, c->d_mm2, c->d_mpart, c->d_check,
                   c->d_widths, c->d_wdef, c->d_tune};
   for (void *p : ptrs)
@@ -1097,6 +1192,10 @@
   for (auto &pair : c->ev)
     for (auto &ev : pair)
       if (ev) (void)hipEventDestroy(ev);
+  for (hipEvent_t e : {c->ev_tail[0], c->ev_tail[1], c->ev_fold, c->ev_main})
+    if (e) (void)hipEventDestroy(e);
+  for (hipStream_t s : c->sstream)
+    if (s) (void)hipStreamDestroy(s);
   if (c->stream) (void)hipStreamDestroy(c->stream);
   delete c;
 }
@@ -1120,7 +1219,7 @@
   if (c->scratch_cap < pin) c->scratch_cap = pin;
   if (c->scratch2_cap < pout && (rc = dev_alloc(&c->d_scratch2, pout))) return rc;
   if (c->scratch2_cap < pout) c->scratch2_cap = pout;
-  HIPCHK(hipMemcpyAsync(c->d_scratch, params, pin * 8, hipMemcpyHostToDevice, c->stream));
+  HIPCHK(hipMemcpyAsync(c->d_scratch, params, pin * 8, hipMemcpyHostToDevice, olpe_main(c)));
   int wpb = 4;
   while (wpb > 1 && (size_t)wpb * vtab_bytes(c->n, c->nsrc) + kEtabBytes > 160 * 1024) wpb /= 2;
   dim3 grid((W + wpb - 1) / wpb), block(wpb * 64);
@@ -1142,22 +1241,22 @@
   }
   if (c->nsrc == 2) {
     if (write)
-      hipLaunchKernelGGL((olpe_eval_kernel<2, true>), grid, block, shm, c->stream, fast ? c->d_DW : c->d_DE,
+      hipLaunchKernelGGL((olpe_eval_kernel<2, true>), grid, block, shm, olpe_main(c), fast ? c->d_DW : c->d_DE,
                          c->n, c->bkgd_mode, fast, c->d_scratch, W, c->d_scratch2);
     else
-      hipLaunchKernelGGL((olpe_eval_kernel<2, false>), grid, block, shm, c->stream, fast ? c->d_DW : c->d_DE,
+      hipLaunchKernelGGL((olpe_eval_kernel<2, false>), grid, block, shm, olpe_main(c), fast ? c->d_DW : c->d_DE,
                          c->n, c->bkgd_mode, fast, c->d_scratch, W, c->d_scratch2);
   } else {
     if (write)
-      hipLaunchKernelGGL((olpe_eval_kernel<3, true>), grid, block, shm, c->stream, fast ? c->d_DW : c->d_DE,
+      hipLaunchKernelGGL((olpe_eval_kernel<3, true>), grid, block, shm, olpe_main(c), fast ? c->d_DW : c->d_DE,
                          c->n, c->bkgd_mode, fast, c->d_scratch, W, c->d_scratch2);
     else
-      hipLaunchKernelGGL((olpe_eval_kernel<3, false>), grid, block, shm, c->stream, fast ? c->d_DW : c->d_DE,
+      hipLaunchKernelGGL((olpe_eval_kernel<3, false>), grid, block, shm, olpe_main(c), fast ? c->d_DW : c->d_DE,
                          c->n, c->bkgd_mode, fast, c->d_scratch, W, c->d_scratch2);
   }
   HIPCHK(hipGetLastError());
-  HIPCHK(hipMemcpyAsync(out, c->d_scratch2, pout * 8, hipMemcpyDeviceToHost, c->stream));
-  HIPCHK(hipStreamSynchronize(c->stream));
+  HIPCHK(hipMemcpyAsync(out, c->d_scratch2, pout * 8, hipMemcpyDeviceToHost, olpe_main(c)));
+  HIPCHK(hipStreamSynchronize(olpe_main(c)));
   return OLPE_OK;
 }
 
@@ -1176,11 +1275,11 @@
   if ((rc = ensure_ensemble(c, W))) return rc;
   uint32_t *ds = nullptr;
   if ((rc = dev_alloc(&ds, (size_t)W))) return rc;
-  HIPCHK(hipMemcpyAsync(ds, seeds, (size_t)W * 4, hipMemcpyHostToDevice, c->stream));
-  hipLaunchKernelGGL(olpe_seed_kernel, dim3((W + 255) / 256), dim3(256), 0, c->stream, ds, W,
+  HIPCHK(hipMemcpyAsync(ds, seeds, (size_t)W * 4, hipMemcpyHostToDevice, olpe_main(c)));
+  hipLaunchKernelGGL(olpe_seed_kernel, dim3((W + 255) / 256), dim3(256), 0, olpe_main(c), ds, W,
                      c->d_mt, c->d_mtpos, c->d_hasg, c->d_gauss);
   HIPCHK(hipGetLastError());
-  HIPCHK(hipStreamSynchronize(c->stream));
+  HIPCHK(hipStreamSynchronize(olpe_main(c)));
   (void)hipFree(ds);
   c->seeded = true;
   c->mom_n = 0;
@@ -1207,8 +1306,8 @@
         return set_err(OLPE_EINVAL, "counter %zu out of range (%g)", i, h[i]);
       t[i] = (uint32_t)h[i];
     }
-  HIPCHK(hipMemcpyAsync(d, t.data(), m * 4, hipMemcpyHostToDevice, c->stream));
-  HIPCHK(hipStreamSynchronize(c->stream));
+  HIPCHK(hipMemcpyAsync(d, t.data(), m * 4, hipMemcpyHostToDevice, olpe_main(c)));
+  HIPCHK(hipStreamSynchronize(olpe_main(c)));
   return OLPE_OK;
 }
 
@@ -1225,14 +1324,14 @@
   if (!c || !state) return set_err(OLPE_EINVAL, "NULL argument");
   if (!c->d_state) return set_err(OLPE_ESTATE, "call olpe_seed first");
   HIPCHK(hipSetDevice(c->device));
-  HIPCHK(hipStreamSynchronize(c->stream));
+  HIPCHK(hipStreamSynchronize(olpe_main(c)));
   HIPCHK(hipMemcpyAsync(c->d_state, state, (size_t)c->W * c->ps * 8, hipMemcpyHostToDevice,
-                        c->stream));
+                        olpe_main(c)));
   int rc;
   if ((rc = counters_to_dev(c, tries, c->d_tries))) return rc;
   if ((rc = counters_to_dev(c, accepts, c->d_acc))) return rc;
-  HIPCHK(hipMemsetAsync(c->d_done, 0xff, (size_t)c->W * sizeof(long long), c->stream));
-  HIPCHK(hipStreamSynchronize(c->stream));
+  HIPCHK(hipMemsetAsync(c->d_done, 0xff, (size_t)c->W * sizeof(long long), olpe_main(c)));
+  HIPCHK(hipStreamSynchronize(olpe_main(c)));
   return OLPE_OK;
 }
 
@@ -1240,7 +1339,7 @@
   if (!c) return set_err(OLPE_EINVAL, "NULL ctx");
   if (!c->d_state) return set_err(OLPE_ESTATE, "no ensemble");
   HIPCHK(hipSetDevice(c->device));
-  HIPCHK(hipStreamSynchronize(c->stream));
+  HIPCHK(hipStreamSynchronize(olpe_main(c)));
   if (state)
     HIPCHK(hipMemcpy(state, c->d_state, (size_t)c->W * c->ps * 8, hipMemcpyDeviceToHost));
   int rc;
@@ -1271,12 +1370,13 @@
     }
   }
   int rc;
+  const int p = c->par ^ 1;
   const size_t chain_need = (size_t)c->W * nrows * c->ps;
-  if (chain_need > c->chain_cap) {
-    if ((rc = dev_alloc(&c->d_chain, chain_need))) return rc;
-    c->chain_cap = chain_need;
-  }
-  c->chain_rows = nrows;
+  if (chain_need > c->chain_cap2[p]) {
+    c->chain_cap2[p] = 0;
+    if ((rc = dev_alloc(&c->d_chain2[p], chain_need))) return rc;
+    c->chain_cap2[p] = chain_need;
+  }
   const size_t trace_need = c->trace_on ? (size_t)c->W * n_iters * kTraceF : 0;
   if (trace_need > c->trace_cap) {
     if ((rc = dev_alloc(&c->d_trace, trace_need))) return rc;
@@ -1303,15 +1403,23 @@
   a.stride = nrows > 0 ? record_stride : 0;
   a.row0 = row0;
   a.nrows = nrows;
-  a.chain = c->d_chain;
+  a.chain = c->d_chain2[p];
   a.accept_min = accept_min;
   a.trace = c->trace_on ? c->d_trace : nullptr;
   a.widths = c->d_widths;
-  hipEvent_t *ev = c->ev[c->launches % olpe_ctx::kRing];
-  if (!ev[0] || !ev[1]) return set_err(OLPE_EHIP, "launch events were not created");
-  HIPCHK(hipEventRecord(ev[0], c->stream));
-  if ((rc = launch_gibbs(c, a))) return rc;
-  HIPCHK(hipEventRecord(ev[1], c->stream));
+  const LaunchSlot l{(int)(c->launches % olpe_ctx::kSlots), c->main_dirty};
+  if (!c->ev[l.slot][0] || !c->ev[l.slot][1])
+    return set_err(OLPE_EHIP, "launch events were not created");
+  if ((rc = follow_main(c, c->sstream[p]))) return rc;
+  c->par = p;
+  if ((rc = launch_gibbs(c, a, l))) {
+    c->par = p ^ 1;
+    return rc;
+  }
+  c->main_dirty = false;
+  c->d_chain = c->d_chain2[p];
+  c->chain_cap = c->chain_cap2[p];
+  c->chain_rows = nrows;
   ++c->launches;
   c->count = c1;
   if (nrec_out) *nrec_out = nrows;
@@ -1321,7 +1429,7 @@
 int olpe_chain_read(olpe_ctx *c, double *chain_out) {
   if (!c || !chain_out) return set_err(OLPE_EINVAL, "NULL argument");
   HIPCHK(hipSetDevice(c->device));
-  HIPCHK(hipStreamSynchronize(c->stream));
+  HIPCHK(hipStreamSynchronize(olpe_main(c)));
   const size_t m = (size_t)c->W * c->chain_rows * c->ps;
   if (m) HIPCHK(hipMemcpy(chain_out, c->d_chain, m * 8, hipMemcpyDeviceToHost));
   return check_units(c);
@@ -1343,7 +1451,7 @@
   if (!c || !done_at) return set_err(OLPE_EINVAL, "NULL argument");
   if (!c->d_done) return set_err(OLPE_ESTATE, "no ensemble");
   HIPCHK(hipSetDevice(c->device));
-  HIPCHK(hipStreamSynchronize(c->stream));
+  HIPCHK(hipStreamSynchronize(olpe_main(c)));
   HIPCHK(hipMemcpy(done_at, c->d_done, (size_t)c->W * 8, hipMemcpyDeviceToHost));
   return check_units(c);
 }
@@ -1367,7 +1475,7 @@
   if (!c) return set_err(OLPE_EINVAL, "NULL ctx");
   if (!c->d_mt) return set_err(OLPE_ESTATE, "no ensemble");
   HIPCHK(hipSetDevice(c->device));
-  HIPCHK(hipStreamSynchronize(c->stream));
+  HIPCHK(hipStreamSynchronize(olpe_main(c)));
   const int W = c->W;
   if (mt_state) {
     std::vector<uint32_t> key((size_t)W * MT_N);
@@ -1396,7 +1504,7 @@
   if (!c || !mt_state || !gauss_cache) return set_err(OLPE_EINVAL, "NULL argument");
   if (!c->d_mt) return set_err(OLPE_ESTATE, "no ensemble (call olpe_seed)");
   HIPCHK(hipSetDevice(c->device));
-  HIPCHK(hipStreamSynchronize(c->stream));
+  HIPCHK(hipStreamSynchronize(olpe_main(c)));
   const int W = c->W;
   std::vector<uint32_t> key((size_t)W * MT_N);
   std::vector<int> pos(W), h(W);
@@ -1426,14 +1534,14 @@
   void *d = nullptr;
   HIPCHK(hipMalloc(&d, bytes));
   if (c->np == 16)
-    hipLaunchKernelGGL(olpe_stream_kernel<16>, dim3(c->W), dim3(64), 0, c->stream, c->d_mt,
+    hipLaunchKernelGGL(olpe_stream_kernel<16>, dim3(c->W), dim3(64), 0, olpe_main(c), c->d_mt,
                        c->d_mtpos, c->d_hasg, c->d_gauss, c->W, kind, n, d);
   else
-    hipLaunchKernelGGL(olpe_stream_kernel<19>, dim3(c->W), dim3(64), 0, c->stream, c->d_mt,
+    hipLaunchKernelGGL(olpe_stream_kernel<19>, dim3(c->W), dim3(64), 0, olpe_main(c), c->d_mt,
                        c->d_mtpos, c->d_hasg, c->d_gauss, c->W, kind, n, d);
   hipError_t e = hipGetLastError();
-  if (e == hipSuccess) e = hipMemcpyAsync(out, d, bytes, hipMemcpyDeviceToHost, c->stream);
-  if (e == hipSuccess) e = hipStreamSynchronize(c->stream);
+  if (e == hipSuccess) e = hipMemcpyAsync(out, d, bytes, hipMemcpyDeviceToHost, olpe_main(c));
+  if (e == hipSuccess) e = hipStreamSynchronize(olpe_main(c));
   (void)hipFree(d);
   if (e != hipSuccess) return set_err(OLPE_EHIP, "rng stream: %s", hipGetErrorString(e));
   return OLPE_OK;
@@ -1442,6 +1550,12 @@
 int olpe_test_hold_handoff(olpe_ctx *c, int on) {
   if (!c) return set_err(OLPE_EINVAL, "NULL ctx");
   c->hold_handoff = on != 0;
+  return OLPE_OK;
+}
+
+int olpe_test_overlaps(olpe_ctx *c, long long *count) {
+  if (!c || !count) return set_err(OLPE_EINVAL, "NULL argument");
+  *count = c->overlaps;
   return OLPE_OK;
 }
 
@@ -1449,21 +1563,31 @@
   if (!c || nrec < 0 || (nrec > 0 && !chain)) return set_err(OLPE_EINVAL, "bad argument");
   if (!c->d_state || !c->seeded) return set_err(OLPE_ESTATE, "call olpe_seed first");
   HIPCHK(hipSetDevice(c->device));
-  HIPCHK(hipStreamSynchronize(c->stream));
+  HIPCHK(hipStreamSynchronize(olpe_main(c)));
   int rc;
   const size_t chain_need = (size_t)c->W * nrec * c->ps;
-  if (chain_need > c->chain_cap) {
+  const int p = c->par;
+  if (chain_need > c->chain_cap2[p]) {
+    c->chain_cap2[p] = 0;
+    c->d_chain = nullptr;
     c->chain_cap = 0;
-    if ((rc = dev_alloc(&c->d_chain, chain_need))) return rc;
-    c->chain_cap = chain_need;
-  }
-  hipEvent_t *ev = c->ev[c->launches % olpe_ctx::kRing];
+    c->chain_rows = 0;
+    if ((rc = dev_alloc(&c->d_chain2[p], chain_need))) return rc;
+    c->chain_cap2[p] = chain_need;
+  }
+  c->d_chain = c->d_chain2[p];
+  c->chain_cap = c->chain_cap2[p];
+  const int slot = (int)(c->launches % olpe_ctx::kSlots);
+  hipEvent_t *ev = c->ev[slot];
   if (!ev[0] || !ev[1]) return set_err(OLPE_EHIP, "launch events were not created");
-  HIPCHK(hipEventRecord(ev[0], c->stream));
+  c->ev_ovl[slot] = false;
+  c->prev_slot = slot;
+  c->prev_queue = false;
+  HIPCHK(hipEventRecord(ev[0], olpe_main(c)));
   if (chain_need)
-    HIPCHK(hipMemcpyAsync(c->d_chain, chain, chain_need * 8, hipMemcpyHostToDevice, c->stream));
-  HIPCHK(hipEventRecord(ev[1], c->stream));
-  HIPCHK(hipStreamSynchronize(c->stream));
+    HIPCHK(hipMemcpyAsync(c->d_chain, chain, chain_need * 8, hipMemcpyHostToDevice, olpe_main(c)));
+  HIPCHK(hipEventRecord(ev[1], olpe_main(c)));
+  HIPCHK(hipStreamSynchronize(olpe_main(c)));
   c->chain_rows = nrec;
   ++c->launches;
   return OLPE_OK;
@@ -1478,7 +1602,7 @@
 int olpe_trace_read(olpe_ctx *c, double *out) {
   if (!c || !out) return set_err(OLPE_EINVAL, "NULL argument");
   HIPCHK(hipSetDevice(c->device));
-  HIPCHK(hipStreamSynchronize(c->stream));
+  HIPCHK(hipStreamSynchronize(olpe_main(c)));
   const size_t m = (size_t)c->W * c->trace_iters * kTraceF;
   if (m) HIPCHK(hipMemcpy(out, c->d_trace, m * 8, hipMemcpyDeviceToHost));
   return OLPE_OK;
@@ -1487,14 +1611,14 @@
 int olpe_sync(olpe_ctx *c) {
   if (!c) return set_err(OLPE_EINVAL, "NULL ctx");
   HIPCHK(hipSetDevice(c->device));
-  HIPCHK(hipStreamSynchronize(c->stream));
+  HIPCHK(hipStreamSynchronize(olpe_main(c)));
   return check_units(c);
 }
 
 int olpe_unit_stats(olpe_ctx *c, long long *out) {
   if (!c || !out) return set_err(OLPE_EINVAL, "NULL argument");
   HIPCHK(hipSetDevice(c->device));
-  HIPCHK(hipStreamSynchronize(c->stream));
+  HIPCHK(hipStreamSynchronize(olpe_main(c)));
   unsigned long long v[2] = {0, 0};
   HIPCHK(hipMemcpy(v, c->d_queue + 2, sizeof(v), hipMemcpyDeviceToHost));
   out[0] = (long long)v[0];
@@ -1515,10 +1639,17 @@
                    olpe_ctx::kRing, c->launches);
   HIPCHK(hipSetDevice(c->device));
   for (int i = 0; i < n; ++i) {
-    hipEvent_t *ev = c->ev[(c->launches - n + i) % olpe_ctx::kRing];
+    const long long j = c->launches - n + i;
+    const int slot = (int)(j % olpe_ctx::kSlots);
+    hipEvent_t *ev = c->ev[slot];
     HIPCHK(hipEventSynchronize(ev[1]));
     float f = 0.f;
     HIPCHK(hipEventElapsedTime(&f, ev[0], ev[1]));
+    if (c->ev_ovl[slot] && j > 0) {
+      float g = 0.f;
+      HIPCHK(hipEventElapsedTime(&g, c->ev[(j - 1) % olpe_ctx::kSlots][1], ev[1]));
+      if (g > 0.f && g < f) f = g;
+    }
     ms_out[i] = f;
   }
   return OLPE_OK;
diff --git a/olpefit_amd/csrc/olpe_comm.hip b/olpefit_amd/csrc/olpe_comm.hip
--- a/olpefit_amd/csrc/olpe_comm.hip
+++ b/olpefit_amd/csrc/olpe_comm.hip
@@ -51,7 +51,7 @@
   c->comm = nullptr;
   c->comm_aborted = true;
   const double t0 = now_s();
-  while (hipStreamQuery(c->stream) == hipErrorNotReady && now_s() - t0 < 10.0)
+  while (hipStreamQuery(olpe_main(c)) == hipErrorNotReady && now_s() - t0 < 10.0)
     std::this_thread::sleep_for(std::chrono::microseconds(200));
   (void)hipGetLastError();
   return set_err(OLPE_ECOMM, "%s", msg);
@@ -90,13 +90,13 @@
 
 int comm_wait(olpe_ctx *c, const char *what) {
   if (!c->comm) {
-    const hipError_t e = hipStreamSynchronize(c->stream);
+    const hipError_t e = hipStreamSynchronize(olpe_main(c));
     return e == hipSuccess ? OLPE_OK : set_err(OLPE_EHIP, "%s: %s", what, hipGetErrorString(e));
   }
   const double t0 = now_s();
   int spins = 0;
   for (;;) {
-    const hipError_t e = hipStreamQuery(c->stream);
+    const hipError_t e = hipStreamQuery(olpe_main(c));
     if (e == hipSuccess) return OLPE_OK;
     if (e != hipErrorNotReady) return set_err(OLPE_EHIP, "%s: %s", what, hipGetErrorString(e));
     ncclResult_t a = ncclSuccess;
@@ -126,7 +126,7 @@
   }
   int copy(void *dst, const void *src, size_t n, hipMemcpyKind kind, proto::Site s) {
     if (forced(s)) return fail(s);
-    const hipError_t e = hipMemcpyAsync(dst, src, n, kind, c->stream);
+    const hipError_t e = hipMemcpyAsync(dst, src, n, kind, olpe_main(c));
     return e == hipSuccess ? OLPE_OK
                            : set_err(OLPE_EHIP, "%s: %s", proto::site_name(s), hipGetErrorString(e));
   }
@@ -141,7 +141,7 @@
     if (c->comm_aborted) return aborted(s);
     if (!c->comm) return send == recv ? OLPE_OK : copy(recv, send, n * sizeof(T),
                                                        hipMemcpyDeviceToDevice, s);
-    return settle(c, ncclAllReduce(send, recv, n, t, op, (ncclComm_t)c->comm, c->stream),
+    return settle(c, ncclAllReduce(send, recv, n, t, op, (ncclComm_t)c->comm, olpe_main(c)),
                   proto::site_name(s));
   }
   int allreduce_max_i64(const long long *s, long long *r, size_t n, proto::Site site) {
@@ -153,7 +153,7 @@
   int allgather_f64(const double *s, double *r, size_t n, proto::Site site) {
     if (c->comm_aborted) return aborted(site);
     if (!c->comm) return copy(r, s, n * sizeof(double), hipMemcpyDeviceToDevice, site);
-    return settle(c, ncclAllGather(s, r, n, ncclDouble, (ncclComm_t)c->comm, c->stream),
+    return settle(c, ncclAllGather(s, r, n, ncclDouble, (ncclComm_t)c->comm, olpe_main(c)),
                   proto::site_name(site));
   }
   int wait(proto::Site s) { return comm_wait(c, proto::site_name(s)); }
diff --git a/olpefit_amd/csrc/olpe_fold.h b/olpefit_amd/csrc/olpe_fold.h
--- a/olpefit_amd/csrc/olpe_fold.h
+++ b/olpefit_amd/csrc/olpe_fold.h
@@ -94,16 +94,18 @@
   b->last_launch = c->launches;
 }
 
+inline hipStream_t main_stream(const olpe_ctx *c) { return olpe_main(const_cast<olpe_ctx *>(c)); }
+
 inline int fold_enter(FoldBase *b, const olpe_ctx *c) {
   int rc;
   if ((rc = wait_pending(b))) return rc;
   HIPCHK(hipEventRecord(b->ev, b->stream));
-  HIPCHK(hipStreamWaitEvent(c->stream, b->ev, 0));
+  HIPCHK(hipStreamWaitEvent(main_stream(c), b->ev, 0));
   return OLPE_OK;
 }
 
 inline int fold_leave(FoldBase *b, const olpe_ctx *c) {
-  HIPCHK(hipEventRecord(b->ev, c->stream));
+  HIPCHK(hipEventRecord(b->ev, main_stream(c)));
   b->ev_pending = true;
   return OLPE_OK;
 }
@@ -114,7 +116,7 @@
   if (!any) return OLPE_OK;
   int rc;
   if ((rc = fold_enter(b, c))) return rc;
-  if ((rc = launch(c->stream))) return rc;
+  if ((rc = launch(main_stream(c)))) return rc;
   return fold_leave(b, c);
 }
 
diff --git a/olpefit_amd/csrc/olpe_internal.h b/olpefit_amd/csrc/olpe_internal.h
--- a/olpefit_amd/csrc/olpe_internal.h
+++ b/olpefit_amd/csrc/olpe_internal.h
@@ -13,8 +13,28 @@
   bool lds_img = true;
   int wpb = 0;
   hipStream_t stream = nullptr;
+  hipStream_t sstream[2] = {nullptr, nullptr};
+  int par = 0;
+  hipEvent_t ev_tail[2] = {};
+  hipEvent_t ev_fold = nullptr;
+  hipEvent_t ev_main = nullptr;
+  bool pend = false;
+  bool main_dirty = false;
+  bool overlap_on = true;
+  bool prev_queue = false;
+  long long prev_W = 0;
+  unsigned prev_tag = 0;
+  unsigned long long *prev_qptr = nullptr;
+  unsigned long long prev_qbase = 0;
+  int prev_slot = -1;
+  long long overlaps = 0;
+  unsigned long long qbase2[2] = {0, 0};
+  double *d_chain2[2] = {nullptr, nullptr};
+  size_t chain_cap2[2] = {0, 0};
   static constexpr int kRing = 64;
-  hipEvent_t ev[kRing][2] = {};
+  static constexpr int kSlots = kRing + 1;
+  hipEvent_t ev[kSlots][2] = {};
+  bool ev_ovl[kSlots] = {};
   long long launches = 0;
   double2 *d_DE = nullptr;
   double2 *d_DW = nullptr;
@@ -39,7 +59,6 @@
   double *d_scratch = nullptr, *d_scratch2 = nullptr;
   size_t scratch_cap = 0, scratch2_cap = 0;
   unsigned long long *d_queue = nullptr;
-  unsigned long long qbase = 0;
   bool queue_on = true;
   int n_cu = 0;
   unsigned *d_uflag = nullptr;
@@ -85,6 +104,9 @@
     if (e_ != hipSuccess)                                                               \
       return ::olpe::set_err(OLPE_EHIP, "%s failed: %s", #expr, hipGetErrorString(e_)); \
   } while (0)
+hipStream_t olpe_main(olpe_ctx *c);
+int olpe_fold_stream(olpe_ctx *c, hipStream_t *s);
+int olpe_fold_done(olpe_ctx *c);
 void olpe_comm_release(olpe_ctx *c);
 int olpe_widths_defaults(olpe_ctx *c, bool with_base);
 int olpe_comm_setup(olpe_ctx *c);
diff --git a/olpefit_amd/csrc/olpe_lik.hip b/olpefit_amd/csrc/olpe_lik.hip
--- a/olpefit_amd/csrc/olpe_lik.hip
+++ b/olpefit_amd/csrc/olpe_lik.hip
@@ -428,7 +428,7 @@
   if (!rc) rc = alloc((void **)&r->d_part, pb * per_block, "the partial sums");
   if (!rc) rc = alloc((void **)&r->d_planes, OLPE_LIK_PLANES * npix * 8, "the planes");
   if (!rc) rc = alloc(&r->d_fin, finblocks * sizeof(FinPart), "the finalize partials");
-  if (!rc && (hipStreamSynchronize(c->stream) != hipSuccess ||
+  if (!rc && (hipStreamSynchronize(olpe_main(c)) != hipSuccess ||
               hipMemcpy(r->d_DE, c->d_DE, npix * sizeof(double2), hipMemcpyDeviceToDevice) != hipSuccess ||
               hipMemset(r->d_cimg, 0, npix * 8) != hipSuccess ||
               hipMemset(r->d_pivot, 0, (size_t)r->ps * 8) != hipSuccess ||
diff --git a/olpefit_amd/csrc/olpe_moments.hip b/olpefit_amd/csrc/olpe_moments.hip
--- a/olpefit_amd/csrc/olpe_moments.hip
+++ b/olpefit_amd/csrc/olpe_moments.hip
@@ -215,8 +215,8 @@
   int rc;
   if ((rc = ensure_moments(c))) return rc;
   if (c->mom_n == 0) {
-    HIPCHK(hipMemsetAsync(c->d_mmean, 0, (size_t)c->W * c->ps * 8, c->stream));
-    HIPCHK(hipMemsetAsync(c->d_mm2, 0, (size_t)c->W * c->ps * 8, c->stream));
+    HIPCHK(hipMemsetAsync(c->d_mmean, 0, (size_t)c->W * c->ps * 8, olpe_main(c)));
+    HIPCHK(hipMemsetAsync(c->d_mm2, 0, (size_t)c->W * c->ps * 8, olpe_main(c)));
   }
   return OLPE_OK;
 }
@@ -228,12 +228,12 @@
   const size_t cols = (size_t)3 * c->ps + 2 * c->np;
   if (!c->d_mpart || c->mpart_cap < cols * nblk || !c->d_mmean)
     return set_err(OLPE_ESTATE, "moments summary before its buffers were prepared");
-  hipLaunchKernelGGL(summary_stage1, dim3(nblk), dim3(kThreads), 0, c->stream, c->d_mmean,
+  hipLaunchKernelGGL(summary_stage1, dim3(nblk), dim3(kThreads), 0, olpe_main(c), c->d_mmean,
                      c->d_mm2, d_centre, c->d_tries, c->d_acc, (long long)c->W, c->ps, c->np,
                      nblk, c->d_mpart);
   HIPCHK(hipGetLastError());
   hipLaunchKernelGGL(olpe::reduce_stage2_kernel<kThreads>, dim3((unsigned)cols), dim3(kThreads),
-                     0, c->stream, c->d_mpart, nblk, d_out + 2);
+                     0, olpe_main(c), c->d_mpart, nblk, d_out + 2);
   HIPCHK(hipGetLastError());
   return OLPE_OK;
 }
@@ -257,17 +257,20 @@
   c->mom_folded = c->launches;
   const long long nrec = c->chain_rows;
   if (nrec == 0) return OLPE_OK;
+  hipStream_t s = nullptr;
+  if ((rc = olpe_fold_stream(c, &s))) return rc;
   if (nrec >= kFoldRowsMin && c->ps <= 64) {
     hipLaunchKernelGGL(fold_rows_kernel, dim3((unsigned)((c->W + kFoldWaves - 1) / kFoldWaves)),
-                       dim3(64 * kFoldWaves), 0, c->stream, c->d_chain, (long long)c->W, c->ps,
+                       dim3(64 * kFoldWaves), 0, s, c->d_chain, (long long)c->W, c->ps,
                        nrec, (double)c->mom_n, c->d_mmean, c->d_mm2);
   } else {
     const long long total = (long long)c->W * c->ps;
     hipLaunchKernelGGL(fold_cols_kernel, dim3((unsigned)((total + kThreads - 1) / kThreads)),
-                       dim3(kThreads), 0, c->stream, c->d_chain, (long long)c->W, c->ps, nrec,
+                       dim3(kThreads), 0, s, c->d_chain, (long long)c->W, c->ps, nrec,
                        (double)c->mom_n, c->d_mmean, c->d_mm2);
   }
   HIPCHK(hipGetLastError());
+  if ((rc = olpe_fold_done(c))) return rc;
   c->mom_n += nrec;
   return OLPE_OK;
 }
@@ -283,7 +286,7 @@
   if (!c || !n) return set_err(OLPE_EINVAL, "NULL argument");
   if (!c->d_state) return set_err(OLPE_ESTATE, "no ensemble");
   HIPCHK(hipSetDevice(c->device));
-  HIPCHK(hipStreamSynchronize(c->stream));
+  HIPCHK(hipStreamSynchronize(olpe_main(c)));
   *n = c->mom_n;
   const size_t m = (size_t)c->W * c->ps;
   std::vector<double> t(m, 0.0);
@@ -306,7 +309,7 @@
   if (!c || n < 0 || (n > 0 && (!mean || !m2))) return set_err(OLPE_EINVAL, "bad argument");
   if (!c->d_state) return set_err(OLPE_ESTATE, "call olpe_seed first");
   HIPCHK(hipSetDevice(c->device));
-  HIPCHK(hipStreamSynchronize(c->stream));
+  HIPCHK(hipStreamSynchronize(olpe_main(c)));
   int rc;
   if ((rc = ensure_moments(c))) return rc;
   const size_t m = (size_t)c->W * c->ps;
@@ -336,13 +339,13 @@
   hipError_t e = hipSuccess;
   if (centre) {
     dc = d + len;
-    e = hipMemcpyAsync(dc, centre, c->ps * sizeof(double), hipMemcpyHostToDevice, c->stream);
+    e = hipMemcpyAsync(dc, centre, c->ps * sizeof(double), hipMemcpyHostToDevice, olpe_main(c));
   }
   int rc = e == hipSuccess ? olpe_moments_prepare(c) : OLPE_OK;
   if (e == hipSuccess && rc == OLPE_OK) rc = olpe_moments_local(c, dc, d);
   if (e == hipSuccess && rc == OLPE_OK)
-    e = hipMemcpyAsync(out, d, len * sizeof(double), hipMemcpyDeviceToHost, c->stream);
-  if (e == hipSuccess && rc == OLPE_OK) e = hipStreamSynchronize(c->stream);
+    e = hipMemcpyAsync(out, d, len * sizeof(double), hipMemcpyDeviceToHost, olpe_main(c));
+  if (e == hipSuccess && rc == OLPE_OK) e = hipStreamSynchronize(olpe_main(c));
   (void)hipFree(d);
   if (rc) return rc;
   if (e != hipSuccess) return set_err(OLPE_EHIP, "moments summary: %s", hipGetErrorString(e));
diff --git a/olpefit_amd/csrc/olpe_normal.hip b/olpefit_amd/csrc/olpe_normal.hip
--- a/olpefit_amd/csrc/olpe_normal.hip
+++ b/olpefit_amd/csrc/olpe_normal.hip
@@ -301,25 +301,25 @@
   const size_t P = (size_t)c->np, nw = (size_t)W;
   const size_t pin = nw * c->ps, pout = nw * (1 + P + P * P);
   int rc;
-  HIPCHK(hipStreamSynchronize(c->stream));
+  HIPCHK(hipStreamSynchronize(olpe_main(c)));
   if ((rc = reserve(c, pin, pout))) return rc;
-  HIPCHK(hipMemcpyAsync(c->d_scratch, params, pin * 8, hipMemcpyHostToDevice, c->stream));
+  HIPCHK(hipMemcpyAsync(c->d_scratch, params, pin * 8, hipMemcpyHostToDevice, olpe_main(c)));
   double *d_chi = c->d_scratch2, *d_grad = d_chi + nw, *d_jtj = d_grad + nw * P;
   const dim3 grid((unsigned)((nw + kWaves - 1) / kWaves)), block(kWaves * 64);
   if (c->nsrc == 2)
-    hipLaunchKernelGGL((normal_kernel<2>), grid, block, 0, c->stream, c->d_DE, c->n,
+    hipLaunchKernelGGL((normal_kernel<2>), grid, block, 0, olpe_main(c), c->d_DE, c->n,
                        c->bkgd_mode, c->d_scratch, W, d_chi, d_grad, d_jtj);
   else if (corner_mfma)
-    hipLaunchKernelGGL((normal_kernel<3, true>), grid, block, 0, c->stream, c->d_DE, c->n,
+    hipLaunchKernelGGL((normal_kernel<3, true>), grid, block, 0, olpe_main(c), c->d_DE, c->n,
                        c->bkgd_mode, c->d_scratch, W, d_chi, d_grad, d_jtj);
   else
-    hipLaunchKernelGGL((normal_kernel<3>), grid, block, 0, c->stream, c->d_DE, c->n,
+    hipLaunchKernelGGL((normal_kernel<3>), grid, block, 0, olpe_main(c), c->d_DE, c->n,
                        c->bkgd_mode, c->d_scratch, W, d_chi, d_grad, d_jtj);
   HIPCHK(hipGetLastError());
-  HIPCHK(hipMemcpyAsync(chi2, d_chi, nw * 8, hipMemcpyDeviceToHost, c->stream));
-  HIPCHK(hipMemcpyAsync(grad, d_grad, nw * P * 8, hipMemcpyDeviceToHost, c->stream));
-  HIPCHK(hipMemcpyAsync(jtj, d_jtj, nw * P * P * 8, hipMemcpyDeviceToHost, c->stream));
-  HIPCHK(hipStreamSynchronize(c->stream));
+  HIPCHK(hipMemcpyAsync(chi2, d_chi, nw * 8, hipMemcpyDeviceToHost, olpe_main(c)));
+  HIPCHK(hipMemcpyAsync(grad, d_grad, nw * P * 8, hipMemcpyDeviceToHost, olpe_main(c)));
+  HIPCHK(hipMemcpyAsync(jtj, d_jtj, nw * P * P * 8, hipMemcpyDeviceToHost, olpe_main(c)));
+  HIPCHK(hipStreamSynchronize(olpe_main(c)));
   return OLPE_OK;
 }
 
@@ -328,19 +328,19 @@
   HIPCHK(hipSetDevice(c->device));
   const size_t npix = (size_t)c->n * c->n, pout = (size_t)c->np * npix;
   int rc;
-  HIPCHK(hipStreamSynchronize(c->stream));
+  HIPCHK(hipStreamSynchronize(olpe_main(c)));
   if ((rc = reserve(c, (size_t)c->ps, pout))) return rc;
-  HIPCHK(hipMemcpyAsync(c->d_scratch, vec, (size_t)c->ps * 8, hipMemcpyHostToDevice, c->stream));
+  HIPCHK(hipMemcpyAsync(c->d_scratch, vec, (size_t)c->ps * 8, hipMemcpyHostToDevice, olpe_main(c)));
   const dim3 grid((unsigned)((npix + kThreads - 1) / kThreads)), block(kThreads);
   if (c->nsrc == 2)
-    hipLaunchKernelGGL((jacobian_kernel<2>), grid, block, 0, c->stream, c->d_scratch, c->n,
+    hipLaunchKernelGGL((jacobian_kernel<2>), grid, block, 0, olpe_main(c), c->d_scratch, c->n,
                        c->bkgd_mode, c->d_scratch2);
   else
-    hipLaunchKernelGGL((jacobian_kernel<3>), grid, block, 0, c->stream, c->d_scratch, c->n,
+    hipLaunchKernelGGL((jacobian_kernel<3>), grid, block, 0, olpe_main(c), c->d_scratch, c->n,
                        c->bkgd_mode, c->d_scratch2);
   HIPCHK(hipGetLastError());
-  HIPCHK(hipMemcpyAsync(planes, c->d_scratch2, pout * 8, hipMemcpyDeviceToHost, c->stream));
-  HIPCHK(hipStreamSynchronize(c->stream));
+  HIPCHK(hipMemcpyAsync(planes, c->d_scratch2, pout * 8, hipMemcpyDeviceToHost, olpe_main(c)));
+  HIPCHK(hipStreamSynchronize(olpe_main(c)));
   return OLPE_OK;
 }
 
diff --git a/olpefit_amd/csrc/olpe_resid.hip b/olpefit_amd/csrc/olpe_resid.hip
--- a/olpefit_amd/csrc/olpe_resid.hip
+++ b/olpefit_amd/csrc/olpe_resid.hip
@@ -338,7 +338,7 @@
   if (!rc) rc = alloc((void **)&r->d_part, pb * per_block, "the partial sums");
   if (!rc) rc = alloc((void **)&r->d_planes, OLPE_RESID_PLANES * npix * 8, "the planes");
   if (!rc) rc = alloc(&r->d_fin, finblocks * sizeof(FinPart), "the finalize partials");
-  if (!rc && (hipStreamSynchronize(c->stream) != hipSuccess ||
+  if (!rc && (hipStreamSynchronize(olpe_main(c)) != hipSuccess ||
               hipMemcpy(r->d_DE, c->d_DE, npix * sizeof(double2), hipMemcpyDeviceToDevice) != hipSuccess ||
               hipMemset(r->d_sum, 0, 2 * npix * 8) != hipSuccess ||
               hipMemset(r->d_pivimg, 0, npix * 8) != hipSuccess ||
diff --git a/olpefit_amd/csrc/olpe_tune.hip b/olpefit_amd/csrc/olpe_tune.hip
--- a/olpefit_amd/csrc/olpe_tune.hip
+++ b/olpefit_amd/csrc/olpe_tune.hip
@@ -92,14 +92,14 @@
 }
 
 int enqueue_sums(olpe_ctx *c, TuneBuf *b) {
-  HIPCHK(hipMemsetAsync(b->now, 0, sizeof(b->now), c->stream));
+  HIPCHK(hipMemsetAsync(b->now, 0, sizeof(b->now), olpe_main(c)));
   const unsigned blocks =
       (unsigned)std::min<long long>(((long long)c->W + kThreads - 1) / kThreads, kMaxBlocks);
   if (c->np == 16)
-    hipLaunchKernelGGL(tune_sum_kernel<16>, dim3(blocks), dim3(kThreads), 0, c->stream, c->d_tries,
+    hipLaunchKernelGGL(tune_sum_kernel<16>, dim3(blocks), dim3(kThreads), 0, olpe_main(c), c->d_tries,
                        c->d_acc, (long long)c->W, b->now);
   else
-    hipLaunchKernelGGL(tune_sum_kernel<19>, dim3(blocks), dim3(kThreads), 0, c->stream, c->d_tries,
+    hipLaunchKernelGGL(tune_sum_kernel<19>, dim3(blocks), dim3(kThreads), 0, olpe_main(c), c->d_tries,
                        c->d_acc, (long long)c->W, b->now);
   HIPCHK(hipGetLastError());
   return OLPE_OK;
@@ -122,7 +122,7 @@
   }
   WidthsArg a = {};
   for (int j = 0; j < c->np; ++j) a.w[j] = w[j];
-  hipLaunchKernelGGL(widths_set_kernel, dim3(1), dim3(64), 0, c->stream, c->np, a, c->d_widths);
+  hipLaunchKernelGGL(widths_set_kernel, dim3(1), dim3(64), 0, olpe_main(c), c->np, a, c->d_widths);
   HIPCHK(hipGetLastError());
   return OLPE_OK;
 }
@@ -130,8 +130,8 @@
 int olpe_widths_get(olpe_ctx *c, double *out) {
   if (!c || !out) return set_err(OLPE_EINVAL, "NULL argument");
   HIPCHK(hipSetDevice(c->device));
-  HIPCHK(hipMemcpyAsync(out, c->d_widths, (size_t)c->np * 8, hipMemcpyDeviceToHost, c->stream));
-  HIPCHK(hipStreamSynchronize(c->stream));
+  HIPCHK(hipMemcpyAsync(out, c->d_widths, (size_t)c->np * 8, hipMemcpyDeviceToHost, olpe_main(c)));
+  HIPCHK(hipStreamSynchronize(olpe_main(c)));
   return OLPE_OK;
 }
 
@@ -154,7 +154,7 @@
   c->tune_on = false;
   int rc;
   if ((rc = enqueue_sums(c, b))) return rc;
-  hipLaunchKernelGGL(tune_update_kernel, dim3(1), dim3(64), 0, c->stream, c->np, b, c->d_widths,
+  hipLaunchKernelGGL(tune_update_kernel, dim3(1), dim3(64), 0, olpe_main(c), c->np, b, c->d_widths,
                      c->d_wdef, 0.0, target, (TuneRec *)nullptr);
   HIPCHK(hipGetLastError());
   c->tune_on = true;
@@ -176,7 +176,7 @@
   if ((rc = enqueue_sums(c, b))) return rc;
   const int k = c->tune_k + 1;
   const double g = c->tune_gain / sqrt((double)k);
-  hipLaunchKernelGGL(tune_update_kernel, dim3(1), dim3(64), 0, c->stream, c->np, b, c->d_widths,
+  hipLaunchKernelGGL(tune_update_kernel, dim3(1), dim3(64), 0, olpe_main(c), c->np, b, c->d_widths,
                      c->d_wdef, g, c->tune_target, b->log + (k - 1));
   HIPCHK(hipGetLastError());
   c->tune_k = k;
@@ -187,7 +187,7 @@
   if (!c || !steps) return set_err(OLPE_EINVAL, "NULL argument");
   if (!c->d_tune) return set_err(OLPE_ESTATE, "no tuning session yet");
   HIPCHK(hipSetDevice(c->device));
-  HIPCHK(hipStreamSynchronize(c->stream));
+  HIPCHK(hipStreamSynchronize(olpe_main(c)));
   const int k = c->tune_k;
   *steps = k;
   if (!k || (!dT && !dA && !widths)) return OLPE_OK;
```
